# zhvng/open-musiclm

Measured on AMD Instinct MI355X. Metric: train steps/sec + AR tokens/sec, coarse-stage musiclm_small, higher is better.
Workload: dtype fp16ff; 1 GPU; musiclm_small coarse-stage train step (fwd+bwd+allreduce+clip+AdamW), N=1116 (3 start + 13 clap + 200 semantic + 900 coarse), forgetful mask 0.15, ff_dropout 0.1; global_batch=32, per_gpu_batch=32, grad_accum=1, seq_len=1116, parallelism=dp1, precision=fp16ff, hip_graph=True, exchange=none (single GPU)

## Files before the change

include/omlm.h:

```cpp
#ifndef OMLM_H
#define OMLM_H
#include <stdint.h>
#ifdef __cplusplus
extern "C" {
#endif

int         omlm_version(void);
const char* omlm_last_error(void);
void        omlm_set_error(const char* msg);

int omlm_gemm(const void* A, const void* B, void* C, const float* Cin,
              const int* a_map, const int* b_map, const int* c_map, long long a_rows, long long b_rows,
              int M, int N, int K, int lda, int ldb, int ldc, int ldcin,
              int a_kmajor, int b_kmajor, int in_dtype, int out_dtype, float alpha,
              void* workspace, long long workspace_bytes, void* stream);
long long omlm_gemm_tail_workspace_bytes(int M, int N);

int omlm_layernorm_fwd(const float* x, const float* gamma, void* y, void* xcast, float* mean, float* rstd,
                       int M, int D, int ldy, float eps, int out_dtype, void* stream);
int omlm_layernorm_fwd_planes(const float* x, const float* gamma, void* y, void* y_lo, float* mean, float* rstd,
                              int M, int D, int ldy, float eps, int out_dtype, void* stream);
int omlm_layernorm_fwd_seg(const float* x, const float* gamma, void* y, void* xcast, float* mean, float* rstd, float* xc,
                           int M, int D, int ldy, float eps, int out_dtype, int n_full, int p0, int n_live, void* stream);
int omlm_layernorm_fwd_planes_seg(const float* x, const float* gamma, void* y, void* y_lo, float* mean, float* rstd, float* xc,
                                  int M, int D, int ldy, float eps, int out_dtype, int n_full, int p0, int n_live, void* stream);
int omlm_layernorm_bwd2_seg(const void* dy, const float* x, const float* gamma, const float* mean, const float* rstd,
                            const float* dres, const void* dres2, float* dx, void* dxcast, float* dgamma, float* workspace, int M, int D,
                            float dx_scale, int cast_dtype, int dy_dtype, int n_full, int p0, int n_live, void* stream);
long long omlm_layernorm_bwd_workspace_bytes(int D);
int omlm_layernorm_bwd2(const void* dy, const float* x, const float* gamma, const float* mean, const float* rstd,
                        const float* dres, const void* dres2, float* dx, void* dxcast, float* dgamma, float* workspace, int M, int D,
                        float dx_scale, int cast_dtype, int dy_dtype, void* stream);

int omlm_qk_norm_fwd(const float* q_raw, const float* kv_raw, const float* q_scale, const float* k_scale,
                     void* q, void* k, void* v, int M, int H, int out_dtype, void* stream);
int omlm_qk_norm_bwd(const float* dq, const float* dk, const float* dv, const float* q_raw, const float* kv_raw,
                     const float* q_scale, const float* k_scale, void* dq_raw, void* dkv_raw,
                     float* dq_scale, float* dk_scale, int M, int H, int out_dtype, void* stream);

int omlm_gemm_qknorm(const void* A, const void* B, void* C, void* C2, int c2_col0, int ldc2, const float* scale, float* norm_out,
                     int ldnorm, int groups, long long a_rows, long long b_rows, int M, int N, int K, int lda, int ldb, int ldc,
                     int dtype, void* stream);
int omlm_qk_norm_bwd2(const float* dq, const float* dk, const float* dv, const void* q, const void* k, const float* qn, const float* kn,
                      const float* q_scale, const float* k_scale, void* dq_raw, void* dkv_raw, float* dq_scale, float* dk_scale,
                      int M, int H, int dtype, void* stream);

int omlm_mqa_attn_fwd(const void* q, const void* k, const void* v, const float* bias, const float* biasT, const unsigned char* keymask,
                      void* out, float* lse, int B, int N, int H, float scale, int bias_ld, int dtype, int P, float p,
                      unsigned long long seed, const unsigned long long* seed_dev, void* stream);
long long omlm_attn_bias_table_floats(int N, int H, int P);
int omlm_attn_bias_prepare(const float* bias, float* biasT, int N, int H, int bias_ld, const float* q_scale,
                           const float* k_scale, float qk_bound, float scale, int p_max_log2, void* stream);
int omlm_attn_bias_prepare_group(const float* bias, float* const* biasT, int layers, int N, int H, int bias_ld,
                                 const float* const* q_scale, const float* const* k_scale, float qk_bound, float scale,
                                 int p_max_log2, int P, void* stream);
int omlm_attn_max_positions(int dtype, int P);
long long omlm_mqa_attn_bwd_workspace_bytes(int B, int N, int H);
int omlm_mqa_attn_bwd(const void* q, const void* k, const void* v, const float* bias, const float* biasT, const unsigned char* keymask,
                      const void* out, const void* dout, const float* lse, float* delta, float* dq, float* dk, float* dv, float* dbias,
                      float* dbias_ws, int B, int N, int H, float scale, int bias_ld, int dtype, int P, float p, unsigned long long seed,
                      const unsigned long long* seed_dev, void* stream);
int omlm_attn_dropout_keep(unsigned char* keep, int B, int N, int H, float p, unsigned long long seed,
                           const unsigned long long* seed_dev, void* stream);
int omlm_dropout_residual_fwd(const float* x, const float* y, float* x1, long long M, int D, float p, unsigned long long seed,
                              const unsigned long long* seed_dev, void* stream);
int omlm_dropout_residual_bwd(const float* dx1, void* dy, long long M, int D, float p, unsigned long long seed,
                              const unsigned long long* seed_dev, int out_dtype, void* stream);

int omlm_ffmid_fwd(const void* h1, const void* convw, const void* gamma, void* h2, float* mean, float* rstd,
                   int M, int nseq, int F, int Fp, float eps, float p, unsigned long long seed,
                   const unsigned long long* seed_dev, unsigned char* drop_bits, void* gh, int dtype, void* stream);
int omlm_ffmid_fwd_planes(const void* h1, const void* h1_lo, const void* convw, const void* convw_lo, const void* gamma, const void* gamma_lo,
                          void* h2, void* h2_lo, float* mean, float* rstd, int M, int nseq, int F, int Fp, float eps, float p,
                          unsigned long long seed, const unsigned long long* seed_dev, unsigned char* drop_bits, void* gh, int dtype, void* stream);
int omlm_ffmid_fwd_seg(const void* h1, const void* convw, const void* gamma, void* h2, float* mean, float* rstd,
                       int M, int nseq, int F, int Fp, float eps, float p, unsigned long long seed,
                       const unsigned long long* seed_dev, unsigned char* drop_bits, void* gh, int dtype, int n_full, int p0, void* stream);
int omlm_ffmid_fwd_planes_seg(const void* h1, const void* h1_lo, const void* convw, const void* convw_lo, const void* gamma, const void* gamma_lo,
                              void* h2, void* h2_lo, float* mean, float* rstd, int M, int nseq, int F, int Fp, float eps, float p,
                              unsigned long long seed, const unsigned long long* seed_dev, unsigned char* drop_bits, void* gh, int dtype,
                              int n_full, int p0, void* stream);
long long omlm_ffmid_bwd_workspace_bytes(int F, int Fp);
int omlm_ffmid_bwd(const void* dh2, const void* h1, const void* convw, const void* gamma, const float* mean,
                   const float* rstd, void* du_tmp, void* dh1, float* dgamma, float* dconv, float* workspace,
                   int M, int nseq, int F, int Fp, float p, unsigned long long seed,
                   const unsigned long long* seed_dev, const unsigned char* drop_bits, const void* gh, int dtype, void* stream);
int omlm_colsum_accumulate(const float* part, float* out, int P, int C, int ldp, void* stream);
typedef struct omlm_colsum_desc { const float* part; float* out; int P, C, ldp; } omlm_colsum_desc;
int omlm_colsum_group(const omlm_colsum_desc* problems, int count, void* stream);
int omlm_ffmid_set_impl(int impl);

int omlm_embed_gather_fwd(const int* ids, const int* seg, const int* posidx,
                          const float* const* tables, const float* const* starts, const float* const* pos,
                          int nseq, float* out, int B, int N, int D,
                          const long long* table_rows, const long long* pos_rows, int* err_flag, void* stream);
int omlm_embed_gather_bwd(const int* ids, const int* seg, const int* posidx,
                          float* const* dtables, float* const* dstarts, float* const* dpos,
                          int nseq, const float* dx, int B, int N, int D, float alpha,
                          const long long* table_rows, const long long* pos_rows, int* err_flag, void* stream);

int omlm_prepare_train_batch(const long long* const* ids, int* const* labels, const int* len, const int* eos, const int* Q,
                             const int* codebook, int nseq, int B, int pad_id, const float* scores, int n_drop,
                             int* ids32, unsigned char* keymask, int N, const float* null_u, float null_p, void* stream);

int omlm_cross_entropy_fwd(const float* logits, const int* labels, float* row_lse, float* nll_sum,
                           int R, int V, int ld, int* err_flag, void* stream);
int omlm_cross_entropy_bwd(const float* logits, const int* labels, const float* row_lse, const float* gscale,
                           float coef, void* dlogits, int R, int V, int ld, int ldd, int out_dtype, void* stream);
int omlm_cross_entropy_fwd_reg(const float* logits, const int* labels, float* row_lse, float* sums,
                               int R, int V, int ld, int* err_flag, void* stream);
int omlm_cross_entropy_bwd_reg(const float* logits, const int* labels, const float* row_lse, const float* gscale,
                               float coef, void* dlogits, int R, int V, int ld, int ldd, int out_dtype,
                               float label_smoothing, float z_loss, void* stream);

int omlm_sumsq_accumulate(const float* g, long long n, float* out, float* partials, void* stream);
int omlm_adamw_clip_step(float* p, float* g, float* m, float* v, void* p16, long long n,
                         float lr, float beta1, float beta2, float eps, float wd, int step,
                         float gscale, const float* gnorm_sq, float max_norm, int decoupled, int zero_grad, int p16_dtype,
                         const float* ls_state, void* stream);
int omlm_adamw_clip_step_ema(float* p, float* g, float* m, float* v, void* p16, long long n,
                             float lr, float beta1, float beta2, float eps, float wd, int step,
                             float gscale, const float* gnorm_sq, float max_norm, int decoupled, int zero_grad, int p16_dtype,
                             const float* ls_state, float* e, float ema_decay, int ema_update_after_step, int ema_warmup, void* stream);
int omlm_loss_scale_update(float* ls_state, const float* gnorm_sq, float growth, float backoff, int interval,
                           float scale_min, float scale_max, void* stream);

int omlm_cast_pad(const float* src, void* dst, long long R, int C, int ld_src, int ld_dst, int out_dtype, void* stream);
typedef struct omlm_cast_pad_desc { const float* src; void* dst; int R, C, ld_src, ld_dst, transpose, lo; } omlm_cast_pad_desc;
int omlm_cast_pad_group(const omlm_cast_pad_desc* problems, int count, int out_dtype, void* stream);

int omlm_gemm_planes(const void* A, long long a_plane_bytes, const void* B, long long b_plane_bytes, void* C, const float* Cin,
                     const int* a_map, const int* b_map, const int* c_map, long long a_rows, long long b_rows,
                     int M, int N, int K, int lda, int ldb, int ldc, int ldcin,
                     int a_kmajor, int b_kmajor, int out_dtype, float alpha, void* workspace, long long workspace_bytes, void* stream);
int omlm_split_planes(const float* x, void* planes, long long n, long long plane_elems, void* stream);
int omlm_gemm_planes16(const void* A, const void* A_lo, const void* B, const void* B_lo, void* C, void* C_lo, const float* Cin,
                       const int* a_map, const int* c_map, long long a_rows, long long b_rows, int M, int N, int K,
                       int lda, int ldb, int ldc, int ldcin, int dtype, void* workspace, long long workspace_bytes, void* stream);
int omlm_gemm_mx16(const void* A, const void* A8, long long a8_stride, const unsigned char* a_scale,
                   const void* B, const void* B8, long long b8_stride, const unsigned char* b_scale,
                   void* C, void* C_lo, int c_lo_bf8, const float* Cin, long long a_rows, long long b_rows,
                   int M, int N, int K, int lda, int ldb, int ldc, int ldcin,
                   void* workspace, long long workspace_bytes, void* stream);
long long omlm_gemm_mx16_workspace_bytes(int M, int N, int K);
int omlm_layernorm_fwd_mx(const float* x, const float* gamma, void* y, void* y8, long long y8_stride, unsigned char* scale8,
                          float* mean, float* rstd, int M, int D, int ldy, float eps, void* stream);
int omlm_ffmid_fwd_mx(const void* h1, const void* h1_lo, const void* convw, const void* convw_lo, const void* gamma, const void* gamma_lo,
                      void* h2, void* h2_8, long long h2_8_stride, unsigned char* scale8, float* mean, float* rstd, int M, int nseq, int F, int Fp,
                      float eps, float p, unsigned long long seed, const unsigned long long* seed_dev, unsigned char* drop_bits, void* gh, void* stream);
int omlm_layernorm_fwd_mx_seg(const float* x, const float* gamma, void* y, void* y8, long long y8_stride, unsigned char* scale8,
                              float* mean, float* rstd, float* xc, int M, int D, int ldy, float eps, int n_full, int p0, int n_live, void* stream);
int omlm_ffmid_fwd_mx_seg(const void* h1, const void* h1_lo, const void* convw, const void* convw_lo, const void* gamma, const void* gamma_lo,
                          void* h2, void* h2_8, long long h2_8_stride, unsigned char* scale8, float* mean, float* rstd, int M, int nseq, int F, int Fp,
                          float eps, float p, unsigned long long seed, const unsigned long long* seed_dev, unsigned char* drop_bits, void* gh,
                          int n_full, int p0, void* stream);
typedef struct omlm_quant_rows_desc { const float* src; unsigned char* dst8; long long lo_stride; unsigned char* scale8; int R, C, ld_src, ld8; } omlm_quant_rows_desc;
int omlm_quant_rows_mx(const omlm_quant_rows_desc* problems, int count, void* stream);
typedef struct omlm_gemm_wgrad_desc {
    const void* A; const void* B; float* C; const int* c_map;
    int M, N, K, lda, ldb, ldc;
} omlm_gemm_wgrad_desc;
int omlm_gemm_wgrad_group(const omlm_gemm_wgrad_desc* problems, int count, int splits, int dtype, void* stream);

int omlm_relpos_first_fwd(const float* w0, const float* b0, float* pre, float* z, int n, int Hd, int x0, void* stream);
int omlm_relpos_first_bwd(const float* ds, float* dw0, int n, int Hd, int x0, void* stream);
int omlm_bias_silu_fwd(const float* a, const float* b, float* pre, float* z, long long R, int C, void* stream);
int omlm_silu_bwd(const float* dz, const float* pre, float* ds, long long total, void* stream);
int omlm_bias_add(const float* a, const float* b, float* out, int R, int C, int ld, void* stream);
int omlm_relpos_mlp_fwd(const float* w0, const float* b0, const float* W1, const float* b1, const float* W2, const float* b2,
                        const float* W3, const float* b3, float* pre0, float* z0, float* pre1, float* z1, float* pre2, float* z2,
                        float* table, int n, int Hd, int H, int ldb, int x0, void* stream);
int omlm_relpos_mlp_bwd(const float* dtable, const float* W1, const float* W2, const float* W3, const float* pre0, const float* z0,
                        const float* pre1, const float* z1, const float* pre2, const float* z2, float* scratch, float* gw0, float* gb0,
                        float* gW1, float* gb1, float* gW2, float* gb2, float* gW3, float* gb3, int n, int Hd, int H, int ldb, int x0,
                        void* stream);

int omlm_rvq_encode(const float* x, const float* codebooks_T, int* indices, float* residual_out,
                    int n, int D, int C, int nstage, int idx_stride, void* stream);
int omlm_nearest_centroid(const float* x, const float* centroids_T, int* indices, int n, int D, int C, void* stream);
int omlm_vq_accumulate(const float* x, const int* indices, int idx_stride, float* counts, float* sums, int n, int D, int K, void* stream);
int omlm_vq_kmeans_update(float* means, float* means_T, const float* counts, const float* sums, int K, int D, void* stream);
int omlm_vq_ema_update(float* cluster_size, float* embed_avg, float* embed, float* embed_T, const float* counts, const float* sums,
                       float* total_scratch, int K, int D, float decay, float eps, void* stream);

long long omlm_kmeans_pp_workspace_bytes(int m, int trials);
int omlm_kmeans_pp_pick(const float* rows, float* closest, const float* uniforms, int* pick_counter, float* centres, float* centres_T,
                        int* chosen, double* pots, void* workspace, long long workspace_bytes, int m, int D, int K, int trials,
                        void* stream);
int omlm_kmeans_pp_seed(const float* rows, float* closest, const float* uniforms, int* pick_counter, float* centres, float* centres_T,
                        int* chosen, double* pots, void* workspace, long long workspace_bytes, int m, int D, int K, int trials,
                        void* stream);
int omlm_kmeans_minibatch_step(const float* x, const int* idx, float* centres, float* centres_T, float* counts, float* bcounts,
                               float* sums, float* rowmin, double* move_partial, double* state, int n, int B, int D, int K,
                               double alpha, double tol_abs, int max_no_improvement, void* stream);
int omlm_kmeans_inertia(const float* x, const float* centres_T, double* out, int* labels, int n, int D, int K, void* stream);

int omlm_sample_topk_gumbel(const float* logits, const float* uniform, long long* out, int B, int V, int ld,
                            int k, float temperature, int forbid_last, void* stream);

int omlm_sample_topk_gumbel_at(const float* logits, const float* uniform_base, const int* step_dev, long long* out,
                               long long* hist, int B, int V, int ld, int k, float temperature, int forbid_last, void* stream);

int omlm_sample_embed_at(const float* logits, const float* uniform_base, const int* step_dev, long long* out, long long* hist,
                         int B, int V, int ld, int k, float temperature, int forbid_last,
                         const float* emb_table, long long emb_row_offset, long long emb_rows, float* x, int D, void* stream);

int omlm_sample_topk_gumbel_rng(const float* logits, unsigned seed_lo, unsigned seed_hi, int step, int row0, long long* out,
                                int B, int V, int ld, int k, float temperature, int forbid_last, void* stream);
int omlm_sample_topk_gumbel_at_rng(const float* logits, unsigned seed_lo, unsigned seed_hi, const int* step_dev, int row0,
                                   long long* out, long long* hist, int B, int V, int ld, int k, float temperature, int forbid_last,
                                   void* stream);
int omlm_sample_embed_at_rng(const float* logits, unsigned seed_lo, unsigned seed_hi, const int* step_dev, int row0, long long* out,
                             long long* hist, int B, int V, int ld, int k, float temperature, int forbid_last,
                             const float* emb_table, long long emb_row_offset, long long emb_rows, float* x, int D, void* stream);

typedef struct omlm_sample_args {
    const float* logits;
    int B, V, ld;
    const float* uniform;
    unsigned seed_lo, seed_hi;
    int step, row0;
    const int* step_dev;
    long long* out;
    long long* hist;
    int k;
    float temperature, top_p;
    int forbid_last;
    const float* emb_table;
    long long emb_row_offset, emb_rows;
    float* x;
    int D;
} omlm_sample_args;
int omlm_sample(const omlm_sample_args* args, void* stream);

int omlm_sample_lp(const omlm_sample_args* args, float* lp_model, float* lp_sampled, void* stream);

typedef struct omlm_sample_row_params {
    const int*   k;
    const float* temperature;
// ... 49 lines not shown
```

open_musiclm_amd/csrc/ffmid.hip:

```cpp
#include "common.h"
#include "ffmid_plan.h"
#include <initializer_list>
#include <stdlib.h>

namespace OMLM_NS {
using namespace omlm_plan;

template <typename T> struct vec8;
template <> struct vec8<float> {
    float v[8];
    __device__ __forceinline__ void load(const float* p) {
        const float4 a = ((const float4*)p)[0], b = ((const float4*)p)[1];
        v[0] = a.x; v[1] = a.y; v[2] = a.z; v[3] = a.w; v[4] = b.x; v[5] = b.y; v[6] = b.z; v[7] = b.w;
    }
    __device__ __forceinline__ void store(float* p) const {
        ((float4*)p)[0] = make_float4(v[0], v[1], v[2], v[3]);
        ((float4*)p)[1] = make_float4(v[4], v[5], v[6], v[7]);
    }
};
template <> struct vec8<h16_t> {
    float v[8];
    __device__ __forceinline__ void load(const h16_t* p) {
        const u32x4 a = *(const u32x4*)p;
#pragma unroll
// ... 421 lines not shown
        for (int i = 0; i < 8; ++i) {
            o.v[i] = w[i][2] * da.v[i] + w[i][1] * (m1 * db.v[i]) + w[i][0] * (m2 * dc.v[i]);
            dw[i][0] += da.v[i] * (p2 * xa.v[i]);
            dw[i][1] += da.v[i] * (p1 * xb.v[i]);
            dw[i][2] += da.v[i] * xc.v[i];
        }
        o.store(dh1 + (size_t)row * ld + col);
    }
#pragma unroll
    for (int i = 0; i < 8; ++i) {
        if (chreal + i < F) {
#pragma unroll
            for (int k = 0; k < 3; ++k)
                part_dconv[((size_t)blockIdx.y * 2 * F + wch + i) * 3 + k] = dw[i][k];
        }
    }
}

__global__ void colsum_kernel(const float* __restrict__ part, float* __restrict__ out, int P, int C, int ldp) {
    const int c = blockIdx.x * blockDim.x + threadIdx.x;
    if (c >= C) return;
    const int per = (P + gridDim.y - 1) / gridDim.y;
    const int p0 = blockIdx.y * per, p1 = min(P, p0 + per);
    float s = 0.f;
    for (int p = p0; p < p1; ++p) s += part[(size_t)p * ldp + c];
    if (p1 > p0) unsafeAtomicAdd(out + c, s);
}

struct omlm_colsum_desc { const float* part; float* out; int P, C, ldp; };
#define OMLM_COLSUM_MAX 32
struct ColsumGroupArgs { int n; omlm_colsum_desc p[OMLM_COLSUM_MAX]; };
__global__ void colsum_group_kernel(ColsumGroupArgs ga) {
    const omlm_colsum_desc& q = ga.p[blockIdx.z];
    const int c = blockIdx.x * blockDim.x + threadIdx.x;
    if (c >= q.C) return;
    const int per = (q.P + gridDim.y - 1) / gridDim.y;
    const int p0 = blockIdx.y * per, p1 = min(q.P, p0 + per);
    float s = 0.f;
    for (int p = p0; p < p1; ++p) s += q.part[(size_t)p * q.ldp + c];
    if (p1 > p0) unsafeAtomicAdd(q.out + c, s);
}

#if OMLM_FP16
extern "C" int omlm_colsum_accumulate(const float* part, float* out, int P, int C, int ldp, void* stream);
extern "C" int omlm_colsum_group(const omlm_colsum_desc* d, int count, void* stream);
#else
extern "C" int omlm_colsum_group(const omlm_colsum_desc* d, int count, void* stream) {
    if (count <= 0) return OMLM_OK;
    OMLM_CHECK_ARG(d, "colsum_group: null descriptor array");
    for (int base = 0; base < count; base += OMLM_COLSUM_MAX) {
        ColsumGroupArgs ga;
        memset(&ga, 0, sizeof(ga));
        ga.n = count - base < OMLM_COLSUM_MAX ? count - base : OMLM_COLSUM_MAX;
        int cmax = 0, pmax = 0;
        for (int i = 0; i < ga.n; ++i) {
            const omlm_colsum_desc& q = d[base + i];
            OMLM_CHECK_ARG(q.part && q.out && q.P > 0 && q.C > 0 && q.ldp >= q.C, "colsum_group: bad problem");
            ga.p[i] = q;
            if (q.C > cmax) cmax = q.C;
            if (q.P > pmax) pmax = q.P;
        }
        hipLaunchKernelGGL(colsum_group_kernel, dim3((cmax + 255) / 256, colsum_ysplit(pmax), ga.n), dim3(256), 0, as_stream(stream), ga);
    }
    return omlm_post_launch("omlm_colsum_group");
}

extern "C" int omlm_colsum_accumulate(const float* part, float* out, int P, int C, int ldp, void* stream) {
    if (P <= 0 || C <= 0) return OMLM_OK;
    OMLM_CHECK_ARG(part && out && ldp >= C, "colsum arguments");
    hipLaunchKernelGGL(colsum_kernel, dim3((C + 255) / 256, colsum_ysplit(P)), dim3(256), 0, as_stream(stream), part, out, P, C, ldp);
    return omlm_post_launch("omlm_colsum_accumulate");
}

#endif

static_assert(FF_ERR_ARG == OMLM_ERR_ARG && FF_LDS_CAP == 160 * 1024 && FF_LDS_OPT_IN == 48 * 1024, "ffmid_plan.h states the return code and launch_lds_optin's sizes");
int ffmid2_launch(const FfmidLaunch& l, const FfmidArgs& a);

template <typename T>
static int ffmid_launch_t(const FfmidLaunch& l, const FfmidArgs& a, float* part_g, float* part_c) {
    const hipStream_t st = as_stream(a.stream);
    const dim3 grid(l.gx, l.gy), block(l.threads);
    switch (l.kernel) {
    case FK_FWD1: {
#define FF_FWD(MC_) launch_lds_optin<ffmid_fwd_kernel<T, MC_>>(grid, block, (size_t)l.lds, st, (const T*)a.h1, (const T*)a.convw, (const T*)a.gamma, (T*)a.h2, a.mean, a.rstd, \
                                                               a.M, a.nseq, a.F, a.Fp, a.eps, a.p, a.seed, a.seed_dev, a.drop_bits, (T*)a.gh)
        switch (l.n) { case 2: FF_FWD(2); break; case 6: FF_FWD(6); break; case 8: FF_FWD(8); break; default: FF_FWD(16); break; }
#undef FF_FWD
        return omlm_post_launch("omlm_ffmid_fwd");
    }
    case FK_BWD1: {
#define FF_B1G(MC_, GH_) launch_lds_optin<ffmid_bwd1_kernel<T, MC_, GH_>>(grid, block, (size_t)l.lds, st, (const T*)a.dh2, (const T*)a.h1, (const T*)a.convw, (const T*)a.gamma, \
                             (const float*)a.mean, (const float*)a.rstd, (T*)a.du_tmp, part_g, a.M, a.nseq, a.F, a.Fp, a.p, a.seed, a.seed_dev, \
                             (const unsigned char*)a.drop_bits, (const T*)a.gh)
#define FF_B1(MC_) do { if (l.gh) FF_B1G(MC_, true); else FF_B1G(MC_, false); } while (0)
        switch (l.n) { case 2: FF_B1(2); break; case 6: FF_B1(6); break; case 8: FF_B1(8); break; default: FF_B1(16); break; }
#undef FF_B1
#undef FF_B1G
        return omlm_post_launch("omlm_ffmid_bwd (row pass)");
    }
    default:
        hipLaunchKernelGGL(ffmid_bwd2_kernel<T>, grid, block, 0, st, (const T*)a.du_tmp, (const T*)a.h1, (const T*)a.convw, (T*)a.dh1, part_c, a.M, a.nseq, a.F, a.Fp);
        return omlm_post_launch("omlm_ffmid_bwd");
    }
}

static int ffmid_launch(const FfmidLaunch& l, const FfmidArgs& a) {
    float* part_g = a.workspace;
    float* part_c = a.workspace ? a.workspace + ffmid_ws_dconv_at(a.Fp) : nullptr;
    switch (l.kernel) {
    case FK_FWD1: case FK_BWD1: case FK_BWD2:
#if !OMLM_FP16
        if (!l.t16) return ffmid_launch_t<float>(l, a, part_g, part_c);
#endif
        return ffmid_launch_t<h16_t>(l, a, part_g, part_c);
    case FK_COLSUM_GROUP: {
        const omlm_colsum_desc two[2] = {{part_g, a.dgamma, l.g_rows, a.F, a.Fp}, {part_c, a.dconv, l.c_rows, 2 * a.F * 3, 2 * a.F * 3}};
        return omlm_colsum_group(two, 2, a.stream);
    }
    case FK_COLSUM_G: return omlm_colsum_accumulate(part_g, a.dgamma, l.g_rows, a.F, a.Fp, a.stream);
    case FK_COLSUM_C: return omlm_colsum_accumulate(part_c, a.dconv, l.c_rows, 2 * a.F * 3, 2 * a.F * 3, a.stream);
    default: return ffmid2_launch(l, a);
    }
}

static int ffmid_run(const FfmidCall& c, const FfmidArgs& a) {
    const FfmidPlan plan = ffmid_plan(c);
    if (plan.rc != OMLM_OK) { omlm_set_error(plan.msg); return plan.rc; }
    for (int i = 0; i < plan.n; ++i) {
        const int rc = ffmid_launch(plan.l[i], a);
        if (rc) return rc;
    }
    return OMLM_OK;
}

#if !OMLM_FP16
extern "C" { __attribute__((visibility("hidden"))) int omlm_ffmid_impl_value = 1; }
extern "C" int omlm_ffmid_set_impl(int impl) {
    OMLM_CHECK_ARG(impl == 0 || impl == 1, "impl: 0 = wave-per-row, 1 = column strips");
    omlm_ffmid_impl_value = impl;
    return OMLM_OK;
}
extern "C" long long omlm_ffmid_bwd_workspace_bytes(int F, int Fp) { return ffmid_bwd_workspace_bytes(F, Fp); }
#else
extern "C" { extern __attribute__((visibility("hidden"))) int omlm_ffmid_impl_value; }
#endif

static FfmidCall ffmid_call(FfOp op, const FfmidArgs& a, int dtype, bool operands) {
    FfmidCall c;
    memset(&c, 0, sizeof(c));
    c.op = op; c.M = a.M; c.nseq = a.nseq; c.F = a.F; c.Fp = a.Fp; c.dtype = dtype; c.fp16_copy = OMLM_FP16 != 0; c.p = a.p; c.operands = operands;
    c.drop_bits = a.drop_bits != nullptr; c.gh = a.gh != nullptr; c.dgamma = a.dgamma != nullptr; c.dconv = a.dconv != nullptr;
    c.n_full = a.n_full; c.p0 = a.p0; c.h2_8_stride = a.h2_8_stride; c.impl = omlm_ffmid_impl_value;
    return c;
}
static bool ffmid_aligned16(std::initializer_list<const void*> ps) {
    uintptr_t all = 0;
    for (const void* q : ps) all |= (uintptr_t)q;
    return all % 16 == 0;
}

#if !OMLM_FP16
extern "C" int omlm_ffmid_fwd_seg_h(const void* h1, const void* convw, const void* gamma, void* h2, float* mean, float* rstd,
                                    int M, int nseq, int F, int Fp, float eps, float p, unsigned long long seed,
                                    const unsigned long long* seed_dev, unsigned char* drop_bits, void* gh, int dtype, int n_full, int p0, void* stream);
#endif
extern "C" int OMLM_API(omlm_ffmid_fwd_seg)(const void* h1, const void* convw, const void* gamma, void* h2, float* mean, float* rstd,
                              int M, int nseq, int F, int Fp, float eps, float p, unsigned long long seed,
                              const unsigned long long* seed_dev, unsigned char* drop_bits, void* gh, int dtype, int n_full, int p0, void* stream) {
#if !OMLM_FP16
    if (dtype == OMLM_DT_F16) return omlm_ffmid_fwd_seg_h(h1, convw, gamma, h2, mean, rstd, M, nseq, F, Fp, eps, p, seed, seed_dev, drop_bits, gh, 1, n_full, p0, stream);
#endif
    FfmidArgs a;
    memset(&a, 0, sizeof(a));
    a.h1 = h1; a.convw = convw; a.gamma = gamma; a.h2 = h2; a.mean = mean; a.rstd = rstd;
    a.M = M; a.nseq = nseq; a.F = F; a.Fp = Fp; a.eps = eps; a.p = p; a.seed = seed; a.seed_dev = seed_dev; a.drop_bits = drop_bits; a.gh = gh;
    a.n_full = n_full; a.p0 = p0; a.stream = stream;
    return ffmid_run(ffmid_call(FF_FWD, a, dtype, h1 && convw && gamma && h2 && mean && rstd), a);
}
#if !OMLM_FP16
extern "C" int omlm_ffmid_fwd(const void* h1, const void* convw, const void* gamma, void* h2, float* mean, float* rstd,
                              int M, int nseq, int F, int Fp, float eps, float p, unsigned long long seed,
                              const unsigned long long* seed_dev, unsigned char* drop_bits, void* gh, int dtype, void* stream) {
    return omlm_ffmid_fwd_seg(h1, convw, gamma, h2, mean, rstd, M, nseq, F, Fp, eps, p, seed, seed_dev, drop_bits, gh, dtype, 0, 0, stream);
}
#endif

#if !OMLM_FP16
extern "C" int omlm_ffmid_fwd_planes_seg_h(const void* h1, const void* h1_lo, const void* convw, const void* convw_lo, const void* gamma, const void* gamma_lo,
                                           void* h2, void* h2_lo, float* mean, float* rstd, int M, int nseq, int F, int Fp, float eps, float p,
                                           unsigned long long seed, const unsigned long long* seed_dev, unsigned char* drop_bits, void* gh, int dtype,
                                           int n_full, int p0, void* stream);
#endif
extern "C" int OMLM_API(omlm_ffmid_fwd_planes_seg)(const void* h1, const void* h1_lo, const void* convw, const void* convw_lo, const void* gamma,
                                               const void* gamma_lo, void* h2, void* h2_lo, float* mean, float* rstd, int M, int nseq, int F, int Fp,
                                               float eps, float p, unsigned long long seed, const unsigned long long* seed_dev,
                                               unsigned char* drop_bits, void* gh, int dtype, int n_full, int p0, void* stream) {
#if !OMLM_FP16
    if (dtype == OMLM_DT_F16)
        return omlm_ffmid_fwd_planes_seg_h(h1, h1_lo, convw, convw_lo, gamma, gamma_lo, h2, h2_lo, mean, rstd, M, nseq, F, Fp, eps, p, seed, seed_dev, drop_bits, gh, 1,
                                           n_full, p0, stream);
#endif
    FfmidArgs a;
    memset(&a, 0, sizeof(a));
    a.h1 = h1; a.h1_lo = h1_lo; a.convw = convw; a.convw_lo = convw_lo; a.gamma = gamma; a.gamma_lo = gamma_lo; a.h2 = h2; a.h2_lo = h2_lo;
    a.mean = mean; a.rstd = rstd; a.M = M; a.nseq = nseq; a.F = F; a.Fp = Fp; a.eps = eps; a.p = p; a.seed = seed; a.seed_dev = seed_dev;
    a.drop_bits = drop_bits; a.gh = gh; a.n_full = n_full; a.p0 = p0; a.stream = stream;
    FfmidCall c = ffmid_call(FF_FWD_PLANES, a, dtype, h1 && h1_lo && convw && convw_lo && gamma && gamma_lo && h2 && h2_lo && mean && rstd);
    c.planes_aligned = ffmid_aligned16({h1, h1_lo, convw, convw_lo, gamma, gamma_lo, h2, h2_lo});
    return ffmid_run(c, a);
}
#if !OMLM_FP16
extern "C" int omlm_ffmid_fwd_planes(const void* h1, const void* h1_lo, const void* convw, const void* convw_lo, const void* gamma,
                                     const void* gamma_lo, void* h2, void* h2_lo, float* mean, float* rstd, int M, int nseq, int F, int Fp,
                                     float eps, float p, unsigned long long seed, const unsigned long long* seed_dev,
                                     unsigned char* drop_bits, void* gh, int dtype, void* stream) {
    return omlm_ffmid_fwd_planes_seg(h1, h1_lo, convw, convw_lo, gamma, gamma_lo, h2, h2_lo, mean, rstd, M, nseq, F, Fp, eps, p, seed, seed_dev, drop_bits, gh,
                                     dtype, 0, 0, stream);
}
#endif

#if OMLM_FP16
}
extern "C" int omlm_ffmid_fwd_mx_seg(const void* h1, const void* h1_lo, const void* convw, const void* convw_lo, const void* gamma, const void* gamma_lo,
                                 void* h2, void* h2_8, long long h2_8_stride, unsigned char* scale8, float* mean, float* rstd, int M, int nseq, int F, int Fp,
                                 float eps, float p, unsigned long long seed, const unsigned long long* seed_dev, unsigned char* drop_bits, void* gh,
                                 int n_full, int p0, void* stream) {
    using namespace OMLM_NS;
    FfmidArgs a;
    memset(&a, 0, sizeof(a));
    a.h1 = h1; a.h1_lo = h1_lo; a.convw = convw; a.convw_lo = convw_lo; a.gamma = gamma; a.gamma_lo = gamma_lo; a.h2 = h2; a.h2_8 = h2_8;
    a.h2_8_stride = h2_8_stride; a.scale8 = scale8; a.mean = mean; a.rstd = rstd; a.M = M; a.nseq = nseq; a.F = F; a.Fp = Fp; a.eps = eps; a.p = p;
    a.seed = seed; a.seed_dev = seed_dev; a.drop_bits = drop_bits; a.gh = gh; a.n_full = n_full; a.p0 = p0; a.stream = stream;
    FfmidCall c = ffmid_call(FF_FWD_MX, a, 1, h1 && h1_lo && convw && convw_lo && gamma && gamma_lo && h2 && h2_8 && scale8 && mean && rstd);
    c.planes_aligned = ffmid_aligned16({h1, h1_lo, convw, convw_lo, gamma, gamma_lo, h2, h2_8});
    return ffmid_run(c, a);
}
extern "C" int omlm_ffmid_fwd_mx(const void* h1, const void* h1_lo, const void* convw, const void* convw_lo, const void* gamma, const void* gamma_lo,
                                 void* h2, void* h2_8, long long h2_8_stride, unsigned char* scale8, float* mean, float* rstd, int M, int nseq, int F, int Fp,
                                 float eps, float p, unsigned long long seed, const unsigned long long* seed_dev, unsigned char* drop_bits, void* gh,
                                 void* stream) {
    return omlm_ffmid_fwd_mx_seg(h1, h1_lo, convw, convw_lo, gamma, gamma_lo, h2, h2_8, h2_8_stride, scale8, mean, rstd, M, nseq, F, Fp, eps, p, seed, seed_dev,
                                 drop_bits, gh, 0, 0, stream);
}
namespace OMLM_NS {
#endif

#if !OMLM_FP16
extern "C" int omlm_ffmid_bwd_h(const void* dh2, const void* h1, const void* convw, const void* gamma, const float* mean,
                                const float* rstd, void* du_tmp, void* dh1, float* dgamma, float* dconv, float* workspace,
                                int M, int nseq, int F, int Fp, float p, unsigned long long seed,
                                const unsigned long long* seed_dev, const unsigned char* drop_bits, const void* gh, int dtype,
                                void* stream);
#endif
extern "C" int OMLM_API(omlm_ffmid_bwd)(const void* dh2, const void* h1, const void* convw, const void* gamma, const float* mean,
                              const float* rstd, void* du_tmp, void* dh1, float* dgamma, float* dconv, float* workspace,
                              int M, int nseq, int F, int Fp, float p, unsigned long long seed,
                              const unsigned long long* seed_dev, const unsigned char* drop_bits, const void* gh, int dtype,
                              void* stream) {
#if !OMLM_FP16
    if (dtype == OMLM_DT_F16)
        return omlm_ffmid_bwd_h(dh2, h1, convw, gamma, mean, rstd, du_tmp, dh1, dgamma, dconv, workspace, M, nseq, F, Fp, p, seed, seed_dev,
                                drop_bits, gh, 1, stream);
#endif
    FfmidArgs a;
    memset(&a, 0, sizeof(a));
    a.dh2 = dh2; a.h1 = h1; a.convw = convw; a.gamma = gamma; a.mean = const_cast<float*>(mean); a.rstd = const_cast<float*>(rstd);
    a.du_tmp = du_tmp; a.dh1 = dh1; a.dgamma = dgamma; a.dconv = dconv; a.workspace = workspace; a.M = M; a.nseq = nseq; a.F = F; a.Fp = Fp; a.p = p;
    a.seed = seed; a.seed_dev = seed_dev; a.drop_bits = const_cast<unsigned char*>(drop_bits); a.gh = const_cast<void*>(gh); a.stream = stream;
    FfmidCall c = ffmid_call(FF_BWD, a, dtype, dh2 && h1 && convw && gamma && mean && rstd && du_tmp && dh1 && workspace);
    c.du_aligned = (uintptr_t)du_tmp % 8 == 0;
    return ffmid_run(c, a);
}

}
```

open_musiclm_amd/csrc/ffmid2.hip:

```cpp
#include "common.h"
#include "ffmid_plan.h"
#include <type_traits>

namespace OMLM_NS {
using namespace omlm_plan;

typedef f32x2 v2;

__device__ __forceinline__ v2 mk2(float a, float b) { v2 r; r[0] = a; r[1] = b; return r; }
__device__ __forceinline__ v2 splat2(float a) { return mk2(a, a); }
__device__ __forceinline__ v2 bf2_to_f2(unsigned w) { return mk2(h16_lo_to_f(w), h16_hi_to_f(w)); }
__device__ __forceinline__ unsigned f2_to_bf2(v2 v) { return pack_h16_rne(v[0], v[1]); }
__device__ __forceinline__ v2 fma2(v2 a, v2 b, v2 c) { return __builtin_elementwise_fma(a, b, c); }

template <typename T> struct Ch8;
template <> struct Ch8<h16_t> {
    u32x4 r;
    __device__ __forceinline__ void load(const h16_t* p) { r = *(const u32x4*)p; }
    __device__ __forceinline__ void zero() { r[0] = 0u; r[1] = 0u; r[2] = 0u; r[3] = 0u; }
    __device__ __forceinline__ v2 get(int i) const { return bf2_to_f2(r[i]); }
    static __device__ __forceinline__ void store(h16_t* p, const v2 (&y)[4]) {
        u32x4 o;
#pragma unroll
        for (int i = 0; i < 4; ++i) o[i] = f2_to_bf2(y[i]);
        *(u32x4*)p = o;
    }
};
template <> struct Ch8<float> {
    float4 a, b;
    __device__ __forceinline__ void load(const float* p) { a = ((const float4*)p)[0]; b = ((const float4*)p)[1]; }
    __device__ __forceinline__ void zero() { a = make_float4(0.f, 0.f, 0.f, 0.f); b = a; }
    __device__ __forceinline__ v2 get(int i) const {
        return i == 0 ? mk2(a.x, a.y) : (i == 1 ? mk2(a.z, a.w) : (i == 2 ? mk2(b.x, b.y) : mk2(b.z, b.w)));
    }
    static __device__ __forceinline__ void store(float* p, const v2 (&y)[4]) {
        ((float4*)p)[0] = make_float4(y[0][0], y[0][1], y[1][0], y[1][1]);
        ((float4*)p)[1] = make_float4(y[2][0], y[2][1], y[3][0], y[3][1]);
    }
};
template <typename T> struct Ch4;
template <> struct Ch4<h16_t> {
    u32x2 r;
    __device__ __forceinline__ void load(const h16_t* p) { r = *(const u32x2*)p; }
    __device__ __forceinline__ void zero() { r[0] = 0u; r[1] = 0u; }
    __device__ __forceinline__ v2 get(int i) const { return bf2_to_f2(r[i]); }
    static __device__ __forceinline__ void store(h16_t* p, const v2 (&y)[2]) {
        u32x2 o; o[0] = f2_to_bf2(y[0]); o[1] = f2_to_bf2(y[1]);
        *(u32x2*)p = o;
    }
};
template <> struct Ch4<float> {
    float4 a;
    __device__ __forceinline__ void load(const float* p) { a = *(const float4*)p; }
    __device__ __forceinline__ void zero() { a = make_float4(0.f, 0.f, 0.f, 0.f); }
    __device__ __forceinline__ v2 get(int i) const { return i == 0 ? mk2(a.x, a.y) : mk2(a.z, a.w); }
    static __device__ __forceinline__ void store(float* p, const v2 (&y)[2]) { *(float4*)p = make_float4(y[0][0], y[0][1], y[1][0], y[1][1]); }
};

template <typename T, bool PL> struct Row8 {
    Ch8<T> h;
    __device__ __forceinline__ void load(const T* p, long long) { h.load(p); }
    __device__ __forceinline__ void zero() { h.zero(); }
    __device__ __forceinline__ v2 get(int i) const { return h.get(i); }
};
template <typename T> struct Row8<T, true> {
    Ch8<T> h, l;
    __device__ __forceinline__ void load(const T* p, long long lo) { h.load(p); l.load(p + lo); }
    __device__ __forceinline__ void zero() { h.zero(); l.zero(); }
    __device__ __forceinline__ v2 get(int i) const { return h.get(i) + l.get(i); }
};
__device__ __forceinline__ void store_planes8(h16_t* hi, h16_t* lo, const v2 (&y)[4]) {
    u32x4 o, l;
#pragma unroll
    for (int i = 0; i < 4; ++i) { o[i] = f2_to_bf2(y[i]); l[i] = f2_to_bf2(y[i] - bf2_to_f2(o[i])); }
    *(u32x4*)hi = o;
    *(u32x4*)lo = l;
}
__device__ __forceinline__ void store_planes8(float*, float*, const v2 (&)[4]) {}
struct FfPlanes { long long h1_lo, convw_lo, gamma_lo; void* h2_lo;
                  unsigned char* h2_8; long long h2_8_stride; unsigned char* scale8;
                  const unsigned char* h1_8; };
__device__ __forceinline__ v2 bf8_pair(u32x2 l, int i) {
    switch (i) {
        case 0: return __builtin_amdgcn_cvt_pk_f32_bf8((int)l[0], false);
        case 1: return __builtin_amdgcn_cvt_pk_f32_bf8((int)l[0], true);
        case 2: return __builtin_amdgcn_cvt_pk_f32_bf8((int)l[1], false);
        default: return __builtin_amdgcn_cvt_pk_f32_bf8((int)l[1], true);
    }
}
template <typename T, bool PL, bool MX> struct H1Row {
    Row8<T, PL> r;
    __device__ __forceinline__ void load(const T* h1, size_t off, const FfPlanes& pl) { r.load(h1 + off, pl.h1_lo); }
    __device__ __forceinline__ void zero() { r.zero(); }
    __device__ __forceinline__ v2 get(int i) const { return r.get(i); }
};
template <typename T> struct H1Row<T, true, true> {
    Ch8<T> h; u32x2 l;
    __device__ __forceinline__ void load(const T* h1, size_t off, const FfPlanes& pl) { h.load(h1 + off); l = *(const u32x2*)(pl.h1_8 + off); }
    __device__ __forceinline__ void zero() { h.zero(); l[0] = 0u; l[1] = 0u; }
    __device__ __forceinline__ v2 get(int i) const { return h.get(i) + bf8_pair(l, i); }
};
__device__ __forceinline__ void store_mx8(h16_t* hi, unsigned char* p8h, unsigned char* p8l, const v2 (&y)[4], float sh, float sl) {
    u32x4 o;
    u32x2 h8, l8;
#pragma unroll
    for (int i = 0; i < 4; ++i) o[i] = f2_to_bf2(y[i]);
#pragma unroll
    for (int i = 0; i < 2; ++i) {
        const v2 ha = bf2_to_f2(o[2 * i]), hb = bf2_to_f2(o[2 * i + 1]);
        h8[i] = pack4_fp8(ha[0] * sh, ha[1] * sh, hb[0] * sh, hb[1] * sh);
        l8[i] = pack4_fp8((y[2 * i][0] - ha[0]) * sl, (y[2 * i][1] - ha[1]) * sl, (y[2 * i + 1][0] - hb[0]) * sl, (y[2 * i + 1][1] - hb[1]) * sl);
    }
    *(u32x4*)hi = o;
    *(u32x2*)p8h = h8;
    *(u32x2*)p8l = l8;
}
__device__ __forceinline__ void store_mx8(float*, unsigned char*, unsigned char*, const v2 (&)[4], float, float) {}


__device__ __forceinline__ void gelu_parts(v2 u, v2& h, v2& ex) {
    const v2 au = mk2(fabsf(u[0]), fabsf(u[1]));
    const v2 d = fma2(au, splat2(0.23164189f), splat2(1.0f));
    const v2 t = mk2(__builtin_amdgcn_rcpf(d[0]), __builtin_amdgcn_rcpf(d[1]));
    v2 poly = fma2(t, splat2(0.5f * 1.061405429f), splat2(0.5f * -1.453152027f));
    poly = fma2(poly, t, splat2(0.5f * 1.421413741f));
    poly = fma2(poly, t, splat2(0.5f * -0.284496736f));
    poly = fma2(poly, t, splat2(0.5f * 0.254829592f));
    poly = poly * t;
    const v2 q = u * u;
    ex = mk2(__builtin_amdgcn_exp2f(q[0] * -0.72134752f), __builtin_amdgcn_exp2f(q[1] * -0.72134752f));
    const v2 hp = fma2(-poly, ex, splat2(0.5f));
    h = mk2(0.5f + copysignf(hp[0], u[0]), 0.5f + copysignf(hp[1], u[1]));
}

__device__ __forceinline__ unsigned lowbias32(unsigned x) {
    x ^= x >> 16; x *= 0x7feb352du; x ^= x >> 15; x *= 0x846ca68bu; x ^= x >> 16;
    return x;
}
__device__ __forceinline__ void keep_words(unsigned long long seed, unsigned long long blk, unsigned w[4]) {
    const unsigned k0 = (unsigned)seed, k1 = (unsigned)(seed >> 32);
    unsigned x = lowbias32(((unsigned)blk ^ k0) + 0x9E3779B9u * ((unsigned)(blk >> 32) ^ k1));
    x = lowbias32(x ^ k1);
    w[0] = x;
    x = (x ^ (x >> 15)) * 0x2c1b3c6du; w[1] = x ^ (x >> 13);
    x = (x ^ (x >> 12)) * 0x297a2d39u; w[2] = x ^ (x >> 15);
    x = (x ^ (x >> 14)) * 0x85ebca6bu; w[3] = x ^ (x >> 16);
}

#define FS_R 4
#define FS_OCC 1

struct FfSeg { int n_full, p0; };
template <typename T, int NT, bool TRAIN, bool PL, bool MX, bool SEG>
__device__ __forceinline__ void ffmid2_fwd_body(const T* __restrict__ h1, const T* __restrict__ convw,
                                                        const T* __restrict__ gamma, T* __restrict__ h2,
                                                        float* __restrict__ mean, float* __restrict__ rstd,
                                                        int nseq, int F, int Fp, int RB, int strips, float eps, float p,
                                                        unsigned long long seed, const unsigned long long* __restrict__ seed_dev,
                                                        unsigned char* __restrict__ drop_bits, T* __restrict__ gh_out, const FfPlanes pl, const FfSeg seg) {
    constexpr int NW = NT / 64;
    constexpr int RB_ = (sizeof(T) == 2 && !PL) ? FS_R : (FS_R > 2 ? 2 : FS_R);
    __shared__ float st[2][FS_R][NW][2];
    __shared__ float gmx[MX ? NW : 1];
    if (seed_dev) seed += seed_dev[0] * 0x9E3779B97F4A7C15ull;
    const int b = blockIdx.x / strips, s = blockIdx.x - b * strips;
    const int t0 = s * RB, t1 = min(nseq, t0 + RB);
    if (t0 >= t1) return;
    const int lane = threadIdx.x & 63, wave = threadIdx.x >> 6;
    const int col = threadIdx.x * 8;
    const int ld = 2 * Fp;
    const size_t row0 = (size_t)b * nseq;
    const size_t hrow0 = SEG ? (size_t)b * seg.n_full + seg.p0 : row0;
    const float inv = p > 0.f ? 1.0f / (1.0f - p) : 1.0f;
    const unsigned thr = (unsigned)(p * 65536.0f + 0.5f);

    v2 wv[3][4], wg[3][4], gm[4];
    Row8<T, PL> tv[3], tg[3];
#pragma unroll
    for (int k = 0; k < 3; ++k) {
        tv[k].load(convw + (size_t)k * ld + col, pl.convw_lo);
        tg[k].load(convw + (size_t)k * ld + Fp + col, pl.convw_lo);
#pragma unroll
        for (int i = 0; i < 4; ++i) { wv[k][i] = tv[k].get(i); wg[k][i] = tg[k].get(i); }
    }
    {
        Row8<T, PL> a;
        a.load(gamma + col, pl.gamma_lo);
#pragma unroll
        for (int i = 0; i < 4; ++i) gm[i] = a.get(i) * inv;
    }
    float gmmax = 0.f;
    if constexpr (MX) {
#pragma unroll
        for (int i = 0; i < 4; ++i) gmmax = fmaxf(gmmax, fmaxf(fabsf(gm[i][0]), fabsf(gm[i][1])));
        gmmax = wave_max(gmmax);
        if (lane == 0) gmx[wave] = gmmax;
        __syncthreads();
        gmmax = gmx[0];
#pragma unroll
        for (int w = 1; w < NW; ++w) gmmax = fmaxf(gmmax, gmx[w]);
    }
    const int e_mx = MX ? mx_row_exp(sqrtf((float)F) * gmmax) : 0;
    const float sh_mx = ldexpf(1.0f, -e_mx), sl_mx = ldexpf(1.0f, 11 - e_mx);
    v2 x1v[4], x1g[4], x2v[4], x2g[4];
    {
        H1Row<T, PL, MX> a, c, d, e;
        a.zero(); c.zero(); d.zero(); e.zero();
        if (t0 >= 1) { a.load(h1, (row0 + t0 - 1) * ld + col, pl); c.load(h1, (row0 + t0 - 1) * ld + Fp + col, pl); }
        if (t0 >= 2) { d.load(h1, (row0 + t0 - 2) * ld + col, pl); e.load(h1, (row0 + t0 - 2) * ld + Fp + col, pl); }
#pragma unroll
        for (int i = 0; i < 4; ++i) { x1v[i] = a.get(i); x1g[i] = c.get(i); x2v[i] = d.get(i); x2g[i] = e.get(i); }
    }
    H1Row<T, PL, MX> rv[RB_], rg[RB_];
#pragma unroll
    for (int r = 0; r < RB_; ++r)
        if (t0 + r < t1) {
            rv[r].load(h1, (row0 + t0 + r) * ld + col, pl);
            rg[r].load(h1, (row0 + t0 + r) * ld + Fp + col, pl);
        }
    const float invF = 1.0f / (float)F;

    auto batch = [&](auto full_tag, const int tb, const int it) {
        constexpr bool FULL = decltype(full_tag)::value;
        v2 g[RB_][4];
        float ls[RB_], lq[RB_];
#pragma unroll
        for (int r = 0; r < RB_; ++r) {
            ls[r] = 0.f; lq[r] = 0.f;
            if (FULL || tb + r < t1) {
                v2 s2 = splat2(0.f), q2 = splat2(0.f);
#pragma unroll
                for (int i = 0; i < 4; ++i) {
                    const v2 xv = rv[r].get(i), xg = rg[r].get(i);
                    const v2 uv = fma2(wv[2][i], xv, fma2(wv[1][i], x1v[i], wv[0][i] * x2v[i]));
                    const v2 ug = fma2(wg[2][i], xg, fma2(wg[1][i], x1g[i], wg[0][i] * x2g[i]));
                    x2v[i] = x1v[i]; x1v[i] = xv; x2g[i] = x1g[i]; x1g[i] = xg;
                    v2 h, ex;
                    gelu_parts(ug, h, ex);
                    const v2 gv = (ug * h) * uv;
                    g[r][i] = gv;
                    s2 += gv;
                    q2 = fma2(gv, gv, q2);
                }
                ls[r] = s2[0] + s2[1];
                lq[r] = q2[0] + q2[1];
            } else {
#pragma unroll
                for (int i = 0; i < 4; ++i) g[r][i] = splat2(0.f);
            }
            if (FULL || tb + RB_ + r < t1) {
                if (FULL) __builtin_amdgcn_sched_barrier(0);
                rv[r].load(h1, (row0 + tb + RB_ + r) * ld + col, pl);
                rg[r].load(h1, (row0 + tb + RB_ + r) * ld + Fp + col, pl);
                if (FULL) __builtin_amdgcn_sched_barrier(0);
            }
        }
#pragma unroll
        for (int r = 0; r < RB_; ++r) { ls[r] = wave_sum(ls[r]); lq[r] = wave_sum(lq[r]); }
        if (lane == 0) {
#pragma unroll
            for (int r = 0; r < RB_; ++r) { st[it & 1][r][wave][0] = ls[r]; st[it & 1][r][wave][1] = lq[r]; }
        }
        __syncthreads();
        float mu_r[RB_], rs_r[RB_];
#pragma unroll
        for (int r = 0; r < RB_; ++r) {
            if (!FULL && tb + r >= t1) continue;
            float S = 0.f, Q = 0.f;
#pragma unroll
            for (int w = 0; w < NW; ++w) { S += st[it & 1][r][w][0]; Q += st[it & 1][r][w][1]; }
            const float mu = S * invF;
            const float var = fmaxf(Q * invF - mu * mu, 0.f);
            const float rs = rsqrtf(var + eps);
            const size_t row = row0 + tb + r;
            const float sh = sh_mx, sl = sl_mx;
            if (FULL) { mu_r[r] = mu; rs_r[r] = rs; }
            else if (threadIdx.x == 0) { mean[row] = mu; rstd[row] = rs; if constexpr (MX) pl.scale8[row] = (unsigned char)(e_mx + 127); }
            const v2 nmr = splat2(-mu * rs), rs2 = splat2(rs);
            v2 gh[4], y[4];
#pragma unroll
            for (int i = 0; i < 4; ++i) gh[i] = fma2(g[r][i], rs2, nmr);
            if (col + 8 > F) {
#pragma unroll
                for (int i = 0; i < 4; ++i) {
                    if (col + 2 * i >= F) gh[i][0] = 0.f;
                    if (col + 2 * i + 1 >= F) gh[i][1] = 0.f;
                }
            }
#pragma unroll
            for (int i = 0; i < 4; ++i) y[i] = gh[i] * gm[i];
            if (TRAIN || p > 0.f) {
                unsigned w[4], bits = 0;
                keep_words(seed, (SEG ? hrow0 + tb + r : row) * (unsigned long long)(Fp >> 3) + (unsigned)(col >> 3), w);
#pragma unroll
                for (int i = 0; i < 4; ++i) {
                    const bool k0 = (w[i] & 0xFFFFu) >= thr, k1 = (w[i] >> 16) >= thr;
                    y[i][0] = k0 ? y[i][0] : 0.f;
                    y[i][1] = k1 ? y[i][1] : 0.f;
                    bits |= (k0 ? 1u : 0u) << (2 * i);
                    bits |= (k1 ? 1u : 0u) << (2 * i + 1);
                }
                if (TRAIN || drop_bits) drop_bits[row * (size_t)(Fp >> 3) + (col >> 3)] = (unsigned char)bits;
            }
            if constexpr (MX) {
                store_mx8(h2 + row * Fp + col, pl.h2_8 + row * (2 * (size_t)Fp) + col, pl.h2_8 + pl.h2_8_stride + row * (2 * (size_t)Fp) + col, y, sh, sl);
                if ((int)threadIdx.x < ((((Fp + 127) & ~127) - Fp) >> 3)) {
                    unsigned char* z8 = pl.h2_8 + row * (2 * (size_t)Fp) + Fp + 8 * threadIdx.x;
                    u32x2 z; z[0] = 0u; z[1] = 0u;
                    *(u32x2*)z8 = z;
                    *(u32x2*)(z8 + pl.h2_8_stride) = z;
                }
            }
            else if constexpr (PL) store_planes8(h2 + row * Fp + col, (T*)pl.h2_lo + row * Fp + col, y);
            else Ch8<T>::store(h2 + row * Fp + col, y);
            if (TRAIN || gh_out) Ch8<T>::store(gh_out + row * Fp + col, gh);
        }
        if (FULL) {
            const int q = lane % RB_;
            float m = mu_r[0], s_ = rs_r[0];
#pragma unroll
            for (int r = 1; r < RB_; ++r) { m = q == r ? mu_r[r] : m; s_ = q == r ? rs_r[r] : s_; }
            mean[row0 + tb + q] = m;
            rstd[row0 + tb + q] = s_;
            if constexpr (MX) pl.scale8[row0 + tb + q] = (unsigned char)(e_mx + 127);
        }
    };
    int it = 0, tb = t0;
    __builtin_amdgcn_s_waitcnt(0x0F70);
#pragma unroll 1
    for (; tb + 2 * RB_ <= t1; tb += RB_, ++it) batch(std::true_type{}, tb, it);
#pragma unroll 1
    for (; tb < t1; tb += RB_, ++it) batch(std::false_type{}, tb, it);
}

template <typename T, int NT, bool TRAIN, bool PL = false, bool MX = false>
__global__ __launch_bounds__(NT, (FS_OCC * NT + 255) / 256) void ffmid2_fwd_kernel(const T* __restrict__ h1, const T* __restrict__ convw,
                                                        const T* __restrict__ gamma, T* __restrict__ h2,
                                                        float* __restrict__ mean, float* __restrict__ rstd,
                                                        int nseq, int F, int Fp, int RB, int strips, float eps, float p,
                                                        unsigned long long seed, const unsigned long long* __restrict__ seed_dev,
                                                        unsigned char* __restrict__ drop_bits, T* __restrict__ gh_out, const FfPlanes pl) {
    ffmid2_fwd_body<T, NT, TRAIN, PL, MX, false>(h1, convw, gamma, h2, mean, rstd, nseq, F, Fp, RB, strips, eps, p, seed, seed_dev, drop_bits, gh_out, pl, FfSeg{0, 0});
}
template <typename T, int NT, bool TRAIN, bool PL = false, bool MX = false>
__global__ __launch_bounds__(NT, (FS_OCC * NT + 255) / 256) void ffmid2_fwd_seg_kernel(const T* __restrict__ h1, const T* __restrict__ convw,
                                                        const T* __restrict__ gamma, T* __restrict__ h2,
                                                        float* __restrict__ mean, float* __restrict__ rstd,
                                                        int nseq, int F, int Fp, int RB, int strips, float eps, float p,
                                                        unsigned long long seed, const unsigned long long* __restrict__ seed_dev,
                                                        unsigned char* __restrict__ drop_bits, T* __restrict__ gh_out, const FfPlanes pl, const FfSeg seg) {
    ffmid2_fwd_body<T, NT, TRAIN, PL, MX, true>(h1, convw, gamma, h2, mean, rstd, nseq, F, Fp, RB, strips, eps, p, seed, seed_dev, drop_bits, gh_out, pl, seg);
}

template <typename T, int MAXC>
__global__ __launch_bounds__(256) void ffmid2_rowsum_kernel(const T* __restrict__ dh2, const T* __restrict__ gamma,
                                                            const T* __restrict__ ghs, const unsigned char* __restrict__ drop_bits,
                                                            const float* __restrict__ rstd, float* __restrict__ bc,
                                                            float* __restrict__ part_dgamma, int M, int F, int Fp, float p) {
    const int lane = threadIdx.x & 63, wave = threadIdx.x >> 6;
    const float inv = p > 0.f ? 1.0f / (1.0f - p) : 1.0f;
    const int nwaves = gridDim.x * 4;
    v2 dg[MAXC][4], gmv[MAXC][4];
#pragma unroll
    for (int k = 0; k < MAXC; ++k) {
        const int ch = (lane + 64 * k) * 8;
        Ch8<T> a;
        a.zero();
        if (ch < Fp) a.load(gamma + ch);
#pragma unroll
        for (int i = 0; i < 4; ++i) { dg[k][i] = splat2(0.f); gmv[k][i] = a.get(i); }
    }
    Ch8<T> d[MAXC], gq[MAXC];
    unsigned bits[MAXC];
    float rs_next = 0.f;
    auto request = [&](int row, int k) {
        const int ch = (lane + 64 * k) * 8;
        if (ch < Fp) {
            d[k].load(dh2 + (size_t)row * Fp + ch);
            gq[k].load(ghs + (size_t)row * Fp + ch);
            bits[k] = (p > 0.f) ? drop_bits[(size_t)row * (Fp >> 3) + (ch >> 3)] : 0xFFu;
        }
    };
    {
        const int row0 = blockIdx.x * 4 + wave;
        if (row0 < M) {
#pragma unroll
            for (int k = 0; k < MAXC; ++k) request(row0, k);
            rs_next = rstd[row0];
        }
    }
    for (int row = blockIdx.x * 4 + wave; row < M; row += nwaves) {
        v2 s1 = splat2(0.f), s2 = splat2(0.f);
        const int nxt = row + nwaves;
        const float rs_cur = rs_next;
#pragma unroll
        for (int k = 0; k < MAXC; ++k) {
            const int ch = (lane + 64 * k) * 8;
            if (ch < Fp) {
#pragma unroll
                for (int i = 0; i < 4; ++i) {
                    v2 dy = d[k].get(i) * inv;
                    if (!((bits[k] >> (2 * i)) & 1u)) dy[0] = 0.f;
                    if (!((bits[k] >> (2 * i + 1)) & 1u)) dy[1] = 0.f;
                    const v2 gh = gq[k].get(i);
                    dg[k][i] = fma2(dy, gh, dg[k][i]);
                    const v2 gy = dy * gmv[k][i];
                    s1 += gy;
                    s2 = fma2(gy, gh, s2);
                }
            }
            if (nxt < M) request(nxt, k);
        }
        if (nxt < M) rs_next = rstd[nxt];
        const float t1 = wave_sum(s1[0] + s1[1]), t2 = wave_sum(s2[0] + s2[1]);
        if (lane == 0) {
            const float rs = rs_cur / (float)F;
            bc[2 * (size_t)row] = rs * t1;
            bc[2 * (size_t)row + 1] = rs * t2;
        }
    }
    extern __shared__ __attribute__((aligned(16))) float red[];
#pragma unroll
    for (int k = 0; k < MAXC; ++k) {
        const int ch = (lane + 64 * k) * 8;
        if (ch < Fp) {
#pragma unroll
            for (int i = 0; i < 4; ++i) { red[(size_t)wave * Fp + ch + 2 * i] = dg[k][i][0]; red[(size_t)wave * Fp + ch + 2 * i + 1] = dg[k][i][1]; }
        }
    }
    __syncthreads();
    for (int c = threadIdx.x; c < Fp; c += 256)
        part_dgamma[(size_t)blockIdx.x * Fp + c] = red[c] + red[Fp + c] + red[2 * Fp + c] + red[3 * Fp + c];
}

template <typename T> struct Bwd2Row { Ch4<T> dy, gh, xv, xg; unsigned bits; float a, b, c; };

template <typename T>
__global__ __launch_bounds__(256) void ffmid2_bwd_kernel(const T* __restrict__ dh2, const T* __restrict__ h1,
                                                         const T* __restrict__ convw, const T* __restrict__ gamma,
                                                         const float* __restrict__ rstd, const float* __restrict__ bc,
                                                         const T* __restrict__ ghs, const unsigned char* __restrict__ drop_bits,
                                                         T* __restrict__ dh1, float* __restrict__ part_dconv,
                                                         int nseq, int F, int Fp, int RB, int strips, int total_strips, float p) {
    const int c4 = blockIdx.x * 256 + threadIdx.x;
    const int col = c4 * 4;
    const bool act = col < Fp;
    const int colc = act ? col : 0;
    const int ld = 2 * Fp;
    const float inv = p > 0.f ? 1.0f / (1.0f - p) : 1.0f;
    const int nib = (c4 & 1) * 4;

    v2 wv[3][2], wg[3][2], gm[2];
#pragma unroll
    for (int k = 0; k < 3; ++k) {
        Ch4<T> a, c;
        a.load(convw + (size_t)k * ld + colc);
        c.load(convw + (size_t)k * ld + Fp + colc);
#pragma unroll
        for (int i = 0; i < 2; ++i) { wv[k][i] = act ? a.get(i) : splat2(0.f); wg[k][i] = act ? c.get(i) : splat2(0.f); }
    }
    {
        Ch4<T> a;
        a.load(gamma + colc);
#pragma unroll
        for (int i = 0; i < 2; ++i) gm[i] = act ? a.get(i) * inv : splat2(0.f);
    }
    v2 dcv[3][2], dcg[3][2];
#pragma unroll
    for (int k = 0; k < 3; ++k)
#pragma unroll
        for (int i = 0; i < 2; ++i) { dcv[k][i] = splat2(0.f); dcg[k][i] = splat2(0.f); }

    auto load_row = [&](Bwd2Row<T>& R, size_t row) {
        R.dy.load(dh2 + row * Fp + colc);
        R.gh.load(ghs + row * Fp + colc);
        R.xv.load(h1 + row * ld + colc);
        R.xg.load(h1 + row * ld + Fp + colc);
        R.bits = (p > 0.f) ? (unsigned)drop_bits[row * (size_t)(Fp >> 3) + (colc >> 3)] : 0xFFu;
        R.a = rstd[row]; R.b = bc[2 * row]; R.c = bc[2 * row + 1];
    };

#pragma unroll 1
    for (int strip = blockIdx.y; strip < total_strips; strip += gridDim.y) {
        const int b = strip / strips, s = strip - b * strips;
        const int t0 = s * RB, t1 = min(nseq, t0 + RB);
        if (t0 >= t1) continue;
        const size_t row0 = (size_t)b * nseq;
        v2 x1v[2], x1g[2], x2v[2], x2g[2], p1v[2], p1g[2], p2v[2], p2g[2];
        {
            Ch4<T> a, c, d, e;
            a.zero(); c.zero(); d.zero(); e.zero();
            if (t0 >= 1) { a.load(h1 + (row0 + t0 - 1) * ld + colc); c.load(h1 + (row0 + t0 - 1) * ld + Fp + colc); }
            if (t0 >= 2) { d.load(h1 + (row0 + t0 - 2) * ld + colc); e.load(h1 + (row0 + t0 - 2) * ld + Fp + colc); }
#pragma unroll
            for (int i = 0; i < 2; ++i) {
                x1v[i] = a.get(i); x1g[i] = c.get(i); x2v[i] = d.get(i); x2g[i] = e.get(i);
                p1v[i] = splat2(0.f); p1g[i] = splat2(0.f); p2v[i] = splat2(0.f); p2g[i] = splat2(0.f);
            }
        }
        const int tend = t1 + 2;
        Bwd2Row<T> cur, nxt;
        load_row(cur, row0 + t0);
#pragma unroll 1
        for (int t = t0; t < tend; ++t) {
            if (t + 1 < min(tend, nseq)) load_row(nxt, row0 + t + 1);
            v2 duv[2], dug[2];
            if (t < nseq) {
                const float own = t < t1 ? 1.f : 0.f;
                const unsigned kb = cur.bits >> nib;
#pragma unroll
                for (int i = 0; i < 2; ++i) {
                    v2 gy = cur.dy.get(i) * gm[i];
                    if (!((kb >> (2 * i)) & 1u)) gy[0] = 0.f;
                    if (!((kb >> (2 * i + 1)) & 1u)) gy[1] = 0.f;
                    const v2 gh = cur.gh.get(i);
                    v2 dg = fma2(gy, splat2(cur.a), splat2(-cur.b));
                    dg = fma2(gh, splat2(-cur.c), dg);
                    const v2 xv = cur.xv.get(i), xg = cur.xg.get(i);
                    const v2 uv = fma2(wv[2][i], xv, fma2(wv[1][i], x1v[i], wv[0][i] * x2v[i]));
                    const v2 ug = fma2(wg[2][i], xg, fma2(wg[1][i], x1g[i], wg[0][i] * x2g[i]));
                    v2 h, ex;
                    gelu_parts(ug, h, ex);
                    const v2 gp = fma2(ug * 0.3989422804f, ex, h);
                    const v2 a_ = dg * (ug * h);
                    const v2 g_ = (dg * uv) * gp;
                    duv[i] = a_; dug[i] = g_;
                    const v2 ao = a_ * own, go = g_ * own;
                    dcv[0][i] = fma2(ao, x2v[i], dcv[0][i]); dcv[1][i] = fma2(ao, x1v[i], dcv[1][i]); dcv[2][i] = fma2(ao, xv, dcv[2][i]);
                    dcg[0][i] = fma2(go, x2g[i], dcg[0][i]); dcg[1][i] = fma2(go, x1g[i], dcg[1][i]); dcg[2][i] = fma2(go, xg, dcg[2][i]);
                    x2v[i] = x1v[i]; x1v[i] = xv; x2g[i] = x1g[i]; x1g[i] = xg;
                }
            } else {
#pragma unroll
                for (int i = 0; i < 2; ++i) { duv[i] = splat2(0.f); dug[i] = splat2(0.f); }
            }
            if (t - 2 >= t0 && act) {
                v2 ov[2], og[2];
#pragma unroll
                for (int i = 0; i < 2; ++i) {
                    ov[i] = fma2(wv[0][i], duv[i], p2v[i]);
                    og[i] = fma2(wg[0][i], dug[i], p2g[i]);
                }
                Ch4<T>::store(dh1 + (row0 + t - 2) * ld + col, ov);
                Ch4<T>::store(dh1 + (row0 + t - 2) * ld + Fp + col, og);
            }
#pragma unroll
            for (int i = 0; i < 2; ++i) {
                p2v[i] = fma2(wv[1][i], duv[i], p1v[i]); p1v[i] = wv[2][i] * duv[i];
                p2g[i] = fma2(wg[1][i], dug[i], p1g[i]); p1g[i] = wg[2][i] * dug[i];
            }
            cur = nxt;
        }
    }
    if (act) {
        float* pr = part_dconv + (size_t)blockIdx.y * 2 * F * 3;
#pragma unroll
        for (int i = 0; i < 2; ++i)
#pragma unroll
            for (int e = 0; e < 2; ++e) {
                const int ch = col + 2 * i + e;
                if (ch < F) {
#pragma unroll
                    for (int k = 0; k < 3; ++k) { pr[(size_t)ch * 3 + k] = dcv[k][i][e]; pr[(size_t)(F + ch) * 3 + k] = dcg[k][i][e]; }
                }
            }
    }
}

template <typename T> struct Bwd3Row { Ch4<T> dy, gh, xv, xg; unsigned bits; float a; };
__device__ __forceinline__ void opaque(Ch4<h16_t>& c) { asm volatile("" : "+v"(c.r[0]), "+v"(c.r[1])); }
__device__ __forceinline__ void opaque(Ch4<float>&) {}

template <typename T, int NT>
__global__ __launch_bounds__(NT) void ffmid3_bwd_kernel(const T* __restrict__ dh2, const T* __restrict__ h1,
                                                        const T* __restrict__ convw, const T* __restrict__ gamma,
                                                        const float* __restrict__ rstd, const T* __restrict__ ghs,
                                                        const unsigned char* __restrict__ drop_bits, T* __restrict__ dh1,
                                                        float* __restrict__ part_dconv, float* __restrict__ part_dgamma,
                                                        int nseq, int F, int Fp, int RB, int strips, int total_strips, float p) {
    constexpr int NW = NT / 64;
    __shared__ __attribute__((aligned(16))) float red[2][NW][2];
    const int lane = threadIdx.x & 63, wave = threadIdx.x >> 6;
    const int col = threadIdx.x * 4;
    const bool act = col < Fp;
    const int colc = act ? col : 0;
    const int ld = 2 * Fp;
    const float inv = p > 0.f ? 1.0f / (1.0f - p) : 1.0f, invF = 1.0f / (float)F;
    const int nib = (threadIdx.x & 1) * 4;

    Ch4<T> wvr[3], wgr[3];
    v2 gm[2];
#pragma unroll
    for (int k = 0; k < 3; ++k) {
        wvr[k].zero(); wgr[k].zero();
        if (act) { wvr[k].load(convw + (size_t)k * ld + colc); wgr[k].load(convw + (size_t)k * ld + Fp + colc); }
    }
    {
        Ch4<T> a;
        a.load(gamma + colc);
#pragma unroll
        for (int i = 0; i < 2; ++i) gm[i] = act ? a.get(i) : splat2(0.f);
    }
    v2 dcv[3][2], dcg[3][2], dgam[2];
#pragma unroll
    for (int i = 0; i < 2; ++i) {
        dgam[i] = splat2(0.f);
#pragma unroll
        for (int k = 0; k < 3; ++k) { dcv[k][i] = splat2(0.f); dcg[k][i] = splat2(0.f); }
    }

    auto load_row = [&](Bwd3Row<T>& R, size_t row) {
        R.dy.load(dh2 + row * Fp + colc);
        R.gh.load(ghs + row * Fp + colc);
        R.xv.load(h1 + row * ld + colc);
        R.xg.load(h1 + row * ld + Fp + colc);
        R.bits = (p > 0.f) ? (unsigned)drop_bits[row * (size_t)(Fp >> 3) + (colc >> 3)] : 0xFFu;
        R.a = rstd[row];
    };
    auto dy_kept = [&](const Bwd3Row<T>& R, v2 (&dy)[2]) {
        const unsigned kb = R.bits >> nib;
#pragma unroll
        for (int i = 0; i < 2; ++i) {
            dy[i] = R.dy.get(i) * inv;
            if (!((kb >> (2 * i)) & 1u)) dy[i][0] = 0.f;
            if (!((kb >> (2 * i + 1)) & 1u)) dy[i][1] = 0.f;
        }
    };
    auto publish_sums = [&](const Bwd3Row<T>& R, int buf) {
        v2 dy[2], s1 = splat2(0.f), s2 = splat2(0.f);
        dy_kept(R, dy);
#pragma unroll
        for (int i = 0; i < 2; ++i) {
            const v2 gy = dy[i] * gm[i];
            s1 += gy;
            s2 = fma2(gy, R.gh.get(i), s2);
        }
        const float t1 = wave_sum_dpp(s1[0] + s1[1]), t2 = wave_sum_dpp(s2[0] + s2[1]);
        if (lane == 0) { red[buf][wave][0] = t1; red[buf][wave][1] = t2; }
    };

#pragma unroll 1
    for (int strip = blockIdx.y; strip < total_strips; strip += gridDim.y) {
        const int b = strip / strips, s = strip - b * strips;
        const int t0 = s * RB, t1 = min(nseq, t0 + RB);
        if (t0 >= t1) continue;
        const size_t row0 = (size_t)b * nseq;
        const int tlast = min(t1 + 2, nseq);
        v2 x1v[2], x1g[2], x2v[2], x2g[2], p1v[2], p1g[2], p2v[2], p2g[2];
        {
            Ch4<T> a, c, d, e;
            a.zero(); c.zero(); d.zero(); e.zero();
            if (t0 >= 1) { a.load(h1 + (row0 + t0 - 1) * ld + colc); c.load(h1 + (row0 + t0 - 1) * ld + Fp + colc); }
            if (t0 >= 2) { d.load(h1 + (row0 + t0 - 2) * ld + colc); e.load(h1 + (row0 + t0 - 2) * ld + Fp + colc); }
#pragma unroll
            for (int i = 0; i < 2; ++i) {
                x1v[i] = a.get(i); x1g[i] = c.get(i); x2v[i] = d.get(i); x2g[i] = e.get(i);
                p1v[i] = splat2(0.f); p1g[i] = splat2(0.f); p2v[i] = splat2(0.f); p2g[i] = splat2(0.f);
            }
        }
        Bwd3Row<T> cur, nx1, nx2;
        load_row(cur, row0 + t0);
        nx1 = cur;
        if (t0 + 1 < tlast) load_row(nx1, row0 + t0 + 1);
        __syncthreads();
        publish_sums(cur, t0 & 1);
        __syncthreads();
        const int tend = t1 + 2;
#pragma unroll 1
        for (int t = t0; t < tend; ++t) {
            nx2 = nx1;
            if (t + 2 < tlast) load_row(nx2, row0 + t + 2);

            if (t + 1 < tlast) publish_sums(nx1, (t + 1) & 1);
            v2 duv[2], dug[2];
            if (t < nseq) {
                v2 S12 = splat2(0.f);
#pragma unroll
                for (int w = 0; w < NW; ++w) S12 += *(const v2*)&red[t & 1][w][0];
                const float S1 = S12[0], S2 = S12[1];
                const float rs = cur.a * invF;
                const float bsum = rs * S1, csum = rs * S2;
                const float own = t < t1 ? 1.f : 0.f;
                v2 dy[2];
                dy_kept(cur, dy);
#pragma unroll
                for (int i = 0; i < 2; ++i) {
                    const v2 gh = cur.gh.get(i);
                    const v2 gy = dy[i] * gm[i];
                    dgam[i] = fma2(dy[i] * own, gh, dgam[i]);
                    v2 dg = fma2(gy, splat2(cur.a), splat2(-bsum));
                    dg = fma2(gh, splat2(-csum), dg);
                    const v2 xv = cur.xv.get(i), xg = cur.xg.get(i);
                    const v2 uv = fma2(wvr[2].get(i), xv, fma2(wvr[1].get(i), x1v[i], wvr[0].get(i) * x2v[i]));
                    const v2 ug = fma2(wgr[2].get(i), xg, fma2(wgr[1].get(i), x1g[i], wgr[0].get(i) * x2g[i]));
                    v2 h, ex;
                    gelu_parts(ug, h, ex);
                    const v2 gp = fma2(ug * 0.3989422804f, ex, h);
                    const v2 a_ = dg * (ug * h);
                    const v2 g_ = (dg * uv) * gp;
                    duv[i] = a_; dug[i] = g_;
                    const v2 ao = a_ * own, go = g_ * own;
                    dcv[0][i] = fma2(ao, x2v[i], dcv[0][i]); dcv[1][i] = fma2(ao, x1v[i], dcv[1][i]); dcv[2][i] = fma2(ao, xv, dcv[2][i]);
                    dcg[0][i] = fma2(go, x2g[i], dcg[0][i]); dcg[1][i] = fma2(go, x1g[i], dcg[1][i]); dcg[2][i] = fma2(go, xg, dcg[2][i]);
                    x2v[i] = x1v[i]; x1v[i] = xv; x2g[i] = x1g[i]; x1g[i] = xg;
                }
            } else {
#pragma unroll
                for (int i = 0; i < 2; ++i) { duv[i] = splat2(0.f); dug[i] = splat2(0.f); }
            }
            if (t - 2 >= t0 && act) {
                v2 ov[2], og[2];
#pragma unroll
                for (int i = 0; i < 2; ++i) {
                    ov[i] = fma2(wvr[0].get(i), duv[i], p2v[i]);
                    og[i] = fma2(wgr[0].get(i), dug[i], p2g[i]);
                }
                Ch4<T>::store(dh1 + (row0 + t - 2) * ld + col, ov);
                Ch4<T>::store(dh1 + (row0 + t - 2) * ld + Fp + col, og);
            }
#pragma unroll
            for (int i = 0; i < 2; ++i) {
                p2v[i] = fma2(wvr[1].get(i), duv[i], p1v[i]); p1v[i] = wvr[2].get(i) * duv[i];
                p2g[i] = fma2(wgr[1].get(i), dug[i], p1g[i]); p1g[i] = wgr[2].get(i) * dug[i];
            }
            cur = nx1; nx1 = nx2;
            __syncthreads();
        }
    }
    if (act) {
        float* pr = part_dconv + (size_t)blockIdx.y * 2 * F * 3;
        float* pg = part_dgamma + (size_t)blockIdx.y * Fp;
#pragma unroll
        for (int i = 0; i < 2; ++i)
#pragma unroll
            for (int e = 0; e < 2; ++e) {
                const int ch = col + 2 * i + e;
                pg[ch] = dgam[i][e];
                if (ch < F) {
#pragma unroll
                    for (int k = 0; k < 3; ++k) { pr[(size_t)ch * 3 + k] = dcv[k][i][e]; pr[(size_t)(F + ch) * 3 + k] = dcg[k][i][e]; }
                }
            }
    }
}

template <typename T, bool PL, bool MX>
static void strip_fwd_go(const FfmidLaunch& l, const FfmidArgs& a, const FfPlanes& pl) {
    const hipStream_t st = as_stream(a.stream);
    const dim3 grid(l.gx, l.gy), block(l.threads);
    const FfSeg seg{a.n_full, a.p0};
#define FF2_FWD(K_, NT_, ...) do { \
        if (l.train) hipLaunchKernelGGL((K_<T, NT_, true, PL, MX>), grid, block, 0, st, (const T*)a.h1, (const T*)a.convw, (const T*)a.gamma, (T*)a.h2, a.mean, a.rstd, \
                                        a.nseq, a.F, a.Fp, l.RB, l.strips, a.eps, a.p, a.seed, a.seed_dev, a.drop_bits, (T*)a.gh, pl, ##__VA_ARGS__); \
        else hipLaunchKernelGGL((K_<T, NT_, false, PL, MX>), grid, block, 0, st, (const T*)a.h1, (const T*)a.convw, (const T*)a.gamma, (T*)a.h2, a.mean, a.rstd, \
                                a.nseq, a.F, a.Fp, l.RB, l.strips, a.eps, a.p, a.seed, a.seed_dev, a.drop_bits, (T*)a.gh, pl, ##__VA_ARGS__); } while (0)
#define FF2_FWD_NT(K_, ...) switch (l.n) { \
        case 64: FF2_FWD(K_, 64, ##__VA_ARGS__); break; case 128: FF2_FWD(K_, 128, ##__VA_ARGS__); break; case 192: FF2_FWD(K_, 192, ##__VA_ARGS__); break; \
        case 256: FF2_FWD(K_, 256, ##__VA_ARGS__); break; case 320: FF2_FWD(K_, 320, ##__VA_ARGS__); break; case 384: FF2_FWD(K_, 384, ##__VA_ARGS__); break; \
        case 448: FF2_FWD(K_, 448, ##__VA_ARGS__); break; default: FF2_FWD(K_, 512, ##__VA_ARGS__); break; }
    if (l.kernel == FK_STRIP_FWD_SEG) FF2_FWD_NT(ffmid2_fwd_seg_kernel, seg)
    else FF2_FWD_NT(ffmid2_fwd_kernel)
#undef FF2_FWD_NT
#undef FF2_FWD
}

template <typename T>
static int ffmid2_launch_t(const FfmidLaunch& l, const FfmidArgs& a) {
    const hipStream_t st = as_stream(a.stream);
    const dim3 grid(l.gx, l.gy), block(l.threads);
    float* part_g = a.workspace;
    float* part_c = a.workspace ? a.workspace + ffmid_ws_dconv_at(a.Fp) : nullptr;
    float* bc = (float*)a.du_tmp;
    switch (l.kernel) {
    case FK_STRIP_FWD: case FK_STRIP_FWD_SEG: {
        FfPlanes pl{0, 0, 0, nullptr, nullptr, 0, nullptr, nullptr};
        if (!l.pl) strip_fwd_go<T, false, false>(l, a, pl);
        else if constexpr (sizeof(T) == 2) {
            pl.convw_lo = (const T*)a.convw_lo - (const T*)a.convw;
            pl.gamma_lo = (const T*)a.gamma_lo - (const T*)a.gamma;
            if (!l.mx) {
                pl.h1_lo = (const T*)a.h1_lo - (const T*)a.h1; pl.h2_lo = a.h2_lo;
                strip_fwd_go<T, true, false>(l, a, pl);
            }
#if OMLM_FP16
            else {
                pl.h1_8 = (const unsigned char*)a.h1_lo; pl.h2_8 = (unsigned char*)a.h2_8; pl.h2_8_stride = a.h2_8_stride; pl.scale8 = a.scale8;
                strip_fwd_go<T, true, true>(l, a, pl);
            }
#endif
        }
        return omlm_post_launch("omlm_ffmid_fwd (strip)");
    }
    case FK_BWD3: {
#define FF3_BWD(NT_) hipLaunchKernelGGL((ffmid3_bwd_kernel<T, NT_>), grid, block, 0, st, (const T*)a.dh2, (const T*)a.h1, (const T*)a.convw, (const T*)a.gamma, \
                       (const float*)a.rstd, (const T*)a.gh, (const unsigned char*)a.drop_bits, (T*)a.dh1, part_c, part_g, a.nseq, a.F, a.Fp, l.RB, l.strips, l.total, a.p)
        switch (l.n) { case 128: FF3_BWD(128); break; case 256: FF3_BWD(256); break; case 512: FF3_BWD(512); break; default: FF3_BWD(768); break; }
#undef FF3_BWD
        return omlm_post_launch("omlm_ffmid_bwd (fused strip)");
    }
    case FK_ROWSUM:
        launch_lds_optin<ffmid2_rowsum_kernel<T, FF_ROWSUM_MC>>(grid, block, (size_t)l.lds, st, (const T*)a.dh2, (const T*)a.gamma, (const T*)a.gh,
                                                                 (const unsigned char*)a.drop_bits, (const float*)a.rstd, bc, part_g, a.M, a.F, a.Fp, a.p);
        return omlm_post_launch("omlm_ffmid_bwd (row sums)");
    case FK_STRIP_BWD:
        hipLaunchKernelGGL(ffmid2_bwd_kernel<T>, grid, block, 0, st, (const T*)a.dh2, (const T*)a.h1, (const T*)a.convw, (const T*)a.gamma, (const float*)a.rstd,
                           (const float*)bc, (const T*)a.gh, (const unsigned char*)a.drop_bits, (T*)a.dh1, part_c, a.nseq, a.F, a.Fp, l.RB, l.strips, l.total, a.p);
        return omlm_post_launch("omlm_ffmid_bwd (strip)");
    default:
        omlm_set_error("omlm_ffmid: the plan names a kernel that ffmid2.hip does not build");
        return OMLM_ERR_UNSUPPORTED;
    }
}

int ffmid2_launch(const FfmidLaunch& l, const FfmidArgs& a) {
#if !OMLM_FP16
    if (!l.t16) return ffmid2_launch_t<float>(l, a);
#endif
    return ffmid2_launch_t<h16_t>(l, a);
}

}
```

open_musiclm_amd/csrc/ffmid_plan.h:

```cpp
#pragma once
#include <stdio.h>
#include <string.h>

#define FF_THREADS 256
#define FF_MAXC_LIMIT 16
#define FF_BWD1_BLOCKS 1024
#define FF_BWD2_STRIPS 512

namespace omlm_plan __attribute__((visibility("hidden"))) {

constexpr int FF_ERR_ARG = -1;
constexpr long long FF_LDS_CAP = 160 * 1024;
constexpr long long FF_LDS_OPT_IN = 48 * 1024;

constexpr int FF_MAX_FP = 8 * 64 * FF_MAXC_LIMIT;
constexpr int FF_STRIP_MAX_FP = 8 * 512;
constexpr int FF_ONE_PASS_MAX_FP = 4 * 768;
constexpr int FF_ROWSUM_MC = 8;
static inline bool ffmid_fp_ok(int F, int Fp) { return Fp % 8 == 0 && Fp >= F && Fp >= 0 && Fp <= FF_MAX_FP; }
static inline bool ffmid_strip_ok(int Fp) { return Fp % 8 == 0 && Fp / 8 <= FF_STRIP_MAX_FP / 8; }
static inline bool ffmid_one_pass(int Fp) { return Fp / 4 <= FF_ONE_PASS_MAX_FP / 4; }

static inline long long ffmid_ws_dconv_at(int Fp) { return (long long)FF_BWD1_BLOCKS * Fp; }
static inline long long ffmid_bwd_workspace_bytes(int F, int Fp) { return 4 * (ffmid_ws_dconv_at(Fp) + (long long)FF_BWD2_STRIPS * 2 * F * 3); }

static inline int ffmid_strip_rows(int nseq, int target) {
    const int n = (nseq + target - 1) / target;
    return (nseq + n - 1) / n;
}
static inline int ffmid_chunks_per_lane(int Fp) { return (Fp / 8 + 63) / 64; }
static inline int ffmid_maxc(int Fp) { const int mc = ffmid_chunks_per_lane(Fp); return mc <= 2 ? 2 : mc <= 6 ? 6 : mc <= 8 ? 8 : 16; }
static inline long long ffmid_row_lds(int Fp) { return 4ll * Fp * 4; }
static inline int colsum_ysplit(int P) { return P >= 1024 ? 128 : (P >= 64 ? 16 : 1); }

enum FfOp { FF_FWD, FF_FWD_PLANES, FF_FWD_MX, FF_BWD };
struct FfmidCall {
    FfOp op;
    int M, nseq, F, Fp;
    int dtype;
    bool fp16_copy;
    float p;
    bool operands;
    bool drop_bits, gh, dgamma, dconv;
    int n_full, p0;
    long long h2_8_stride;
    bool planes_aligned;
    bool du_aligned;
    int impl;
};
enum FfKernel {
    FK_FWD1, FK_BWD1, FK_BWD2,
    FK_STRIP_FWD, FK_STRIP_FWD_SEG, FK_ROWSUM, FK_STRIP_BWD, FK_BWD3,
    FK_COLSUM_G, FK_COLSUM_C, FK_COLSUM_GROUP
};
struct FfmidLaunch {
    FfKernel kernel;
    bool t16;
    int n;
    bool train, pl, mx, gh;
    int gx, gy, threads;
    long long lds;
    int RB, strips, total;
    int g_rows, c_rows;
};
struct FfmidPlan {
    int rc;
    char msg[384];
    bool strips;
    int n;
    FfmidLaunch l[4];
};

static inline FfmidPlan& ffmid_refuse(FfmidPlan& p, const char* text) {
    p.rc = FF_ERR_ARG; p.n = 0;
    snprintf(p.msg, sizeof(p.msg), "bad argument: %s", text);
    return p;
}
static inline FfmidLaunch& ffmid_push(FfmidPlan& p, FfKernel k, const FfmidCall& c, int n, int gx, int gy, int threads, long long lds) {
    FfmidLaunch& l = p.l[p.n++];
    memset(&l, 0, sizeof(l));
    l.kernel = k; l.t16 = c.dtype != 0; l.n = n; l.gx = gx; l.gy = gy; l.threads = threads; l.lds = lds;
    return l;
}
static inline void ffmid_push_colsums(FfmidPlan& p, const FfmidCall& c, int g_rows, int c_rows) {
    const int cg = c.F, cc = 2 * c.F * 3;
    if (c.dgamma && c.dconv) {
        FfmidLaunch& l = ffmid_push(p, FK_COLSUM_GROUP, c, 0, (cc + 255) / 256, colsum_ysplit(g_rows > c_rows ? g_rows : c_rows), 256, 0);
        l.g_rows = g_rows; l.c_rows = c_rows;
        return;
    }
    if (c.dgamma) ffmid_push(p, FK_COLSUM_G, c, 0, (cg + 255) / 256, colsum_ysplit(g_rows), 256, 0).g_rows = g_rows;
    if (c.dconv) ffmid_push(p, FK_COLSUM_C, c, 0, (cc + 255) / 256, colsum_ysplit(c_rows), 256, 0).c_rows = c_rows;
}

#define FF_REFUSE_UNLESS(cond, text) do { if (!(cond)) return ffmid_refuse(p, text); } while (0)

static inline FfmidPlan ffmid_plan(const FfmidCall& c) {
    FfmidPlan p;
    memset(&p, 0, sizeof(p));
    const int M = c.M, nseq = c.nseq, F = c.F, Fp = c.Fp;
    const bool fwd = c.op != FF_BWD, planes = c.op == FF_FWD_PLANES || c.op == FF_FWD_MX;
    const bool keep_ok = c.p == 0.f || c.drop_bits;
    if (c.op == FF_FWD_PLANES) FF_REFUSE_UNLESS(c.dtype == 1, "ffmid_fwd_planes: dtype 1 (bf16) or 2 (fp16) [dtype == 1]");
    else if (c.op != FF_FWD_MX) FF_REFUSE_UNLESS(!c.fp16_copy || c.dtype == 1, "the fp16 copy serves fp16 operands only [dtype == 1]");
    if (M <= 0) return p;
    if (fwd) FF_REFUSE_UNLESS(c.n_full == 0 || (c.p0 > 0 && c.p0 + nseq == c.n_full),
                              "row segment: nseq must be n_full - p0, p0 > 0 [(n_full) == 0 || ((p0) > 0 && (p0) + (nseq) == (n_full))]");
    FF_REFUSE_UNLESS(c.operands, c.op == FF_FWD ? "null pointer [h1 && convw && gamma && h2 && mean && rstd]" :
                                 c.op == FF_FWD_PLANES ? "null pointer [h1 && h1_lo && convw && convw_lo && gamma && gamma_lo && h2 && h2_lo && mean && rstd]" :
                                 c.op == FF_FWD_MX ? "null pointer [h1 && h1_lo && convw && convw_lo && gamma && gamma_lo && h2 && h2_8 && scale8 && mean && rstd]" :
                                                     "null pointer [dh2 && h1 && convw && gamma && mean && rstd && du_tmp && dh1 && workspace]");
    if (c.op == FF_FWD_PLANES)
        FF_REFUSE_UNLESS(Fp >= F && ffmid_strip_ok(Fp), "ffmid_fwd_planes: Fp must be F rounded up to 8 and <= 4096 [Fp % 8 == 0 && Fp >= F && ffmid2_supported(Fp)]");
    else if (c.op == FF_FWD_MX)
        FF_REFUSE_UNLESS(Fp >= F && ffmid_strip_ok(Fp), "ffmid_fwd_mx: Fp must be F rounded up to 8 and <= 4096 [Fp % 8 == 0 && Fp >= F && ffmid2_supported(Fp)]");
    else
        FF_REFUSE_UNLESS(ffmid_fp_ok(F, Fp), "Fp must be F rounded up to 8 and <= 8192 [Fp % 8 == 0 && Fp >= F && Fp <= 8192 && (size_t)5 * Fp * sizeof(float) <= 160 * 1024]");
    FF_REFUSE_UNLESS(nseq > 0 && M % nseq == 0, "M must be batch * nseq [nseq > 0 && M % nseq == 0]");
    if (planes) FF_REFUSE_UNLESS(c.p >= 0.f && c.p < 1.f && keep_ok, "dropout p (keep bits required when p > 0) [p >= 0.f && p < 1.f && (p == 0.f || drop_bits)]");
    else if (fwd) FF_REFUSE_UNLESS(c.p >= 0.f && c.p < 1.f, "dropout p [p >= 0.f && p < 1.f]");
    if (c.op == FF_FWD_MX) {
        FF_REFUSE_UNLESS(c.h2_8_stride >= (long long)M * 2 * Fp && c.h2_8_stride % 16 == 0,
                         "ffmid_fwd_mx: fp8 plane stride [h2_8_stride >= (long long)M * 2 * Fp && h2_8_stride % 16 == 0]");
        FF_REFUSE_UNLESS(2 * Fp >= (Fp + 127) / 128 * 128,
                         "ffmid_fwd_mx: an fp8 plane row (pitch 2 * Fp bytes) must hold Fp rounded up to 128 bytes [2 * Fp >= (Fp + 127) / 128 * 128]");
        FF_REFUSE_UNLESS(c.planes_aligned, "ffmid_fwd_mx: 16-byte aligned planes [(((uintptr_t)h1 | (uintptr_t)h1_lo | (uintptr_t)convw | (uintptr_t)convw_lo | "
                                           "(uintptr_t)gamma | (uintptr_t)gamma_lo | (uintptr_t)h2 | (uintptr_t)h2_8) % 16) == 0]");
    } else if (c.op == FF_FWD_PLANES) {
        FF_REFUSE_UNLESS(c.planes_aligned, "ffmid_fwd_planes: 16-byte aligned planes [(((uintptr_t)h1 | (uintptr_t)h1_lo | (uintptr_t)convw | (uintptr_t)convw_lo | "
                                           "(uintptr_t)gamma | (uintptr_t)gamma_lo | (uintptr_t)h2 | (uintptr_t)h2_lo) % 16) == 0]");
    }
    p.strips = planes || (c.impl == 1 && ffmid_strip_ok(Fp) && keep_ok && (fwd || c.gh));
    const int B = M / nseq, rows4 = (M + 3) / 4;
    if (fwd && p.strips) {
        const int RB = ffmid_strip_rows(nseq, 36), strips = (nseq + RB - 1) / RB, nt = ffmid_chunks_per_lane(Fp) * 64;
        const bool segd = c.n_full > 0 && c.p > 0.f;
        FfmidLaunch& l = ffmid_push(p, segd ? FK_STRIP_FWD_SEG : FK_STRIP_FWD, c, nt >= 64 && nt < 512 ? nt : 512, B * strips, 1, Fp / 8, 0);
        l.train = c.p > 0.f && c.drop_bits && c.gh;
        l.pl = planes; l.mx = c.op == FF_FWD_MX; l.RB = RB; l.strips = strips;
        return p;
    }
    if (fwd) {
        ffmid_push(p, FK_FWD1, c, ffmid_maxc(Fp), rows4 < 4096 ? rows4 : 4096, 1, FF_THREADS, ffmid_row_lds(Fp));
        return p;
    }
    if (!p.strips) {
        const int b1 = rows4 < FF_BWD1_BLOCKS ? rows4 : FF_BWD1_BLOCKS, strips = M < FF_BWD2_STRIPS ? M : FF_BWD2_STRIPS;
        ffmid_push(p, FK_BWD1, c, ffmid_maxc(Fp), b1, 1, FF_THREADS, ffmid_row_lds(Fp)).gh = c.gh;
        ffmid_push(p, FK_BWD2, c, 0, (2 * Fp / 8 + FF_THREADS - 1) / FF_THREADS, strips, FF_THREADS, 0);
        ffmid_push_colsums(p, c, b1, strips);
        return p;
    }
    FF_REFUSE_UNLESS(c.du_aligned, "du_tmp must be 8-byte aligned [((uintptr_t)du_tmp % 8) == 0]");
    const int RB = ffmid_strip_rows(nseq, 35), strips = (nseq + RB - 1) / RB, total = B * strips;
    const int per = (total + 255) / 256;
    int ny = (total + per - 1) / per, g_rows;
    if (ny > FF_BWD2_STRIPS) ny = FF_BWD2_STRIPS;
    if (ffmid_one_pass(Fp)) {
        const int nthr = (Fp / 4 + 63) / 64 * 64, nt = nthr <= 128 ? 128 : nthr <= 256 ? 256 : nthr <= 512 ? 512 : 768;
        FfmidLaunch& l = ffmid_push(p, FK_BWD3, c, nt, 1, ny, nt, 0);
        l.RB = RB; l.strips = strips; l.total = total;
        g_rows = ny;
    } else {
        g_rows = rows4 < FF_BWD1_BLOCKS ? rows4 : FF_BWD1_BLOCKS;
        ffmid_push(p, FK_ROWSUM, c, FF_ROWSUM_MC, g_rows, 1, 256, ffmid_row_lds(Fp));
        FfmidLaunch& l = ffmid_push(p, FK_STRIP_BWD, c, 0, (Fp / 4 + 255) / 256, ny, 256, 0);
        l.RB = RB; l.strips = strips; l.total = total;
    }
    ffmid_push_colsums(p, c, g_rows, ny);
    return p;
}
#undef FF_REFUSE_UNLESS

struct FfmidArgs {
    const void *h1, *convw, *gamma, *h1_lo, *convw_lo, *gamma_lo;
    void *h2, *h2_lo, *h2_8;
    unsigned char* scale8;
    float *mean, *rstd;
    const void* dh2;
    void *du_tmp, *dh1;
    float *dgamma, *dconv, *workspace;
    int M, nseq, F, Fp;
    float eps, p;
    unsigned long long seed;
    const unsigned long long* seed_dev;
    unsigned char* drop_bits;
    void* gh;
    int n_full, p0;
    long long h2_8_stride;
    void* stream;
};

}

#ifdef OMLM_PLAN_TEST_ABI
extern "C" void omlm_plan_ffmid(const int* v, double p, long long h2_8_stride, long long* out, char* msg) {
    const omlm_plan::FfmidCall c = {(omlm_plan::FfOp)v[0], v[1], v[2], v[3], v[4], v[5], v[6] != 0, (float)p, v[7] != 0, v[8] != 0, v[9] != 0, v[10] != 0,
                                    v[11] != 0, v[12], v[13], h2_8_stride, v[14] != 0, v[15] != 0, v[16]};
    const omlm_plan::FfmidPlan q = omlm_plan::ffmid_plan(c);
    out[0] = q.rc; out[1] = q.strips; out[2] = q.n;
    for (int i = 0; i < q.n; ++i) {
        const omlm_plan::FfmidLaunch& l = q.l[i];
        const long long w[16] = {l.kernel, l.t16, l.n, l.train, l.pl, l.mx, l.gh, l.gx, l.gy, l.threads, l.lds, l.RB, l.strips, l.total, l.g_rows, l.c_rows};
        memcpy(out + 3 + 16 * i, w, sizeof(w));
    }
    memcpy(msg, q.msg, sizeof(q.msg));
}
extern "C" void omlm_plan_ffmid_limits(int* out) {
    const int v[5] = {omlm_plan::FF_MAX_FP, omlm_plan::FF_STRIP_MAX_FP, omlm_plan::FF_ONE_PASS_MAX_FP, FF_BWD1_BLOCKS, FF_BWD2_STRIPS};
    memcpy(out, v, sizeof(v));
}
extern "C" int omlm_plan_ffmid_fp_ok(int F, int Fp) { return omlm_plan::ffmid_fp_ok(F, Fp); }
extern "C" int omlm_plan_ffmid_strip_ok(int Fp) { return omlm_plan::ffmid_strip_ok(Fp); }
extern "C" int omlm_plan_ffmid_one_pass(int Fp) { return omlm_plan::ffmid_one_pass(Fp); }
extern "C" long long omlm_plan_ffmid_bwd_workspace_bytes(int F, int Fp) { return omlm_plan::ffmid_bwd_workspace_bytes(F, Fp); }
extern "C" long long omlm_plan_ffmid_ws_dconv_at(int Fp) { return omlm_plan::ffmid_ws_dconv_at(Fp); }
#endif
```

open_musiclm_amd/engine.py:

```python
from __future__ import annotations

import math
import os
from dataclasses import dataclass, field
from typing import Dict, List, Optional, Sequence, Tuple

import torch

from . import ops
from .hip import require_gpu

ATTN_SCALE = 8.0
DIM_HEAD = 64

_PRECISIONS = {"bf16": torch.bfloat16, "bf16x3": torch.float32, "fp16": torch.float16, "fp16ff": torch.float16}


def is_half(precision: str) -> bool:
    return precision in ("fp16", "fp16ff")
_H16 = (torch.bfloat16, torch.float16)



FF_PLANES_MAX_FP = 4096


def ff_planes_ok(Fp: int) -> bool:
    return Fp <= FF_PLANES_MAX_FP


def ff_mx_ok(D: int, Fp: int) -> bool:
    return D % 64 == 0 and D <= 4096 and Fp % 64 == 0 and ff_planes_ok(Fp)


def default_precision() -> str:
    p = os.environ.get("OMLM_PRECISION", "bf16")
    if p not in _PRECISIONS:
        raise ValueError(f"OMLM_PRECISION must be one of {list(_PRECISIONS)}, got {p}")
    return p


def loss_scale_initial() -> float:
    return float(os.environ.get("OMLM_FP16_LOSS_SCALE", "4096"))


def loss_scale_state(model) -> torch.Tensor:
    dev = model.start_tokens[0].device
    st = model.__dict__.get("_omlm_ls_state")
    if st is None or st.device != dev:
        st = torch.tensor([loss_scale_initial(), 0.0, 0.0, 0.0, loss_scale_initial()], device=dev, dtype=torch.float32)
        model.__dict__["_omlm_ls_state"] = st
    return st


def loss_scale(precision: str, model=None) -> float:
    if not is_half(precision):
        return 1.0
    if model is None or "_omlm_ls_state" not in model.__dict__:
        return loss_scale_initial()
    return float(model.__dict__["_omlm_ls_state"][0].item())


_MODEL_OF: Dict[int, tuple] = {}


def tag_parameters(model, precision: Optional[str]):
    import weakref
    ref = weakref.ref(model)
    for p in model.parameters():
        p._omlm_precision = precision
        key = id(p)
        _MODEL_OF[key] = (weakref.ref(p, lambda _r, k=key: _MODEL_OF.pop(k, None)), ref)


def model_of(p) -> Optional[torch.nn.Module]:
    ent = _MODEL_OF.get(id(p))
    if ent is None or ent[0]() is not p:
        return None
    return ent[1]()


@torch.no_grad()
def unscale_grads_(model, precision: Optional[str] = None):
    s = loss_scale(precision or getattr(model, "precision", None) or default_precision(), model)
    if s != 1.0:
        for p in model.parameters():
            if p.grad is not None:
                p.grad.mul_(1.0 / s)


def ceil_to(x: int, m: int) -> int:
    return (x + m - 1) // m * m


def grad_of(p: torch.Tensor) -> torch.Tensor:
    if p.grad is None:
        p.grad = torch.zeros_like(p, memory_format=torch.contiguous_format)
    return p.grad


@dataclass
class SeqLayout:
    B: int
    N: int
    lens: Tuple[int, ...]
    starts: Tuple[int, ...]
    n_out: Tuple[int, ...]
    seg: torch.Tensor
    posidx: torch.Tensor
    start_col: torch.Tensor
    final_only: bool = False
    head_maps: Dict[Tuple[int, int], Tuple[torch.Tensor, torch.Tensor, int]] = field(default_factory=dict)
    live_maps: Dict[Tuple[int, int, int], torch.Tensor] = field(default_factory=dict)


def build_layout(B: int, lens: Sequence[int], quantizers: Sequence[int], device, final_rows_only: bool = False) -> SeqLayout:
    starts, pos = [], 0
    for l in lens:
        starts.append(pos)
        pos += l + 1
    N = pos
    seg = torch.empty(N, dtype=torch.int32)
    posidx = torch.zeros(N, dtype=torch.int32)
    start_col = torch.zeros(N, dtype=torch.bool)
    for s, (st, l) in enumerate(zip(starts, lens)):
        seg[st: st + l + 1] = s
        start_col[st] = True
        posidx[st + 1: st + l + 1] = torch.arange(l, dtype=torch.int32)
    n_out = [l for l in lens[:-1]] + [lens[-1] + 1]
    lay = SeqLayout(B, N, tuple(lens), tuple(starts), tuple(n_out), seg.to(device), posidx.to(device),
                    start_col.to(device), final_rows_only)
    if final_rows_only:
        s, st, n_s, Q = len(lens) - 1, starts[-1], n_out[-1], quantizers[-1]
        b = torch.arange(B)
        a_map = (b * N + st + n_s - 1).to(torch.int32)
        lay.head_maps[(s, (n_s - 1) % Q)] = (a_map.to(device), b.to(torch.int32).to(device), B)
        return lay
    for s, (st, n_s, Q) in enumerate(zip(starts, n_out, quantizers)):
        for qq in range(Q):
            js = torch.arange(qq, n_s, Q)
            if js.numel() == 0:
                continue
            b = torch.arange(B)[:, None]
            a_map = (b * N + st + js[None, :]).reshape(-1).to(torch.int32)
            c_map = (b * n_s + js[None, :]).reshape(-1).to(torch.int32)
            lay.head_maps[(s, qq)] = (a_map.to(device), c_map.to(device), int(a_map.numel()))
    return lay


CONV_HALO = 2
LIVE_K_MULTIPLE = 64
FF_ONE_PASS_MAX_FP = 3072


def first_live_row(lay: SeqLayout, want: Sequence[bool]) -> Optional[int]:
    firsts = [st for st, n_s, w in zip(lay.starts, lay.n_out, want) if w and n_s > 0]
    return min(firsts) if firsts else None


def live_rows(lay: SeqLayout, want: Sequence[bool], B: int, T: torch.dtype, Fp: int, halo: int = CONV_HALO) -> Optional[Tuple[int, int, int]]:
    if os.environ.get("OMLM_LIVE_ROWS", "1") == "0":
        return None
    if lay.final_only or T == torch.float32 or Fp > FF_ONE_PASS_MAX_FP:
        return None
    first = first_live_row(lay, want)
    if first is None:
        return None
    N = lay.N
    g = LIVE_K_MULTIPLE // math.gcd(B, LIVE_K_MULTIPLE)
    top = first - halo
    if top < 0:
        return None
    p0 = top - (top - N) % g
    if p0 <= 0 or 16 * p0 < N:
        return None
    return N, p0, N - p0


def live_to_full(r, seg: Tuple[int, int, int]):
    n_full, p0, n_live = seg
    return (r // n_live) * n_full + p0 + r % n_live


def full_to_live(r, seg: Tuple[int, int, int]):
    n_full, p0, n_live = seg
    return (r // n_full) * n_live + r % n_full - p0


def head_map(lay: SeqLayout, s: int, qq: int, live: Optional[Tuple[int, int, int]]):
    ent = lay.head_maps.get((s, qq))
    if ent is None or live is None:
        return ent
    a_map, c_map, rows = ent
    key = (s, qq, live[1])
    if key not in lay.live_maps:
        lay.live_maps[key] = full_to_live(a_map, live).to(torch.int32)
    return lay.live_maps[key], c_map, rows


def h16_operand(w: torch.Tensor, T: torch.dtype) -> torch.Tensor:
    sh = getattr(w, "_omlm_bf16", None)
    if (sh is not None and sh.dtype == T and getattr(w, "_omlm_bf16_version", -1) == w._version and sh.device == w.device):
        return sh
    c = torch.empty(w.shape, dtype=T, device=w.device)
    ops.cast_pad(w.detach(), c, w.numel() // w.shape[-1], w.shape[-1], w.shape[-1], w.shape[-1])
    return c


class PreparedWeights:
    def __init__(self, model, precision: str, persistent: bool = True):
        tr = model.transformer
        self.precision = precision
        self.T = _PRECISIONS[precision]
        self.ff3 = precision == "fp16ff"
        T = self.T
        dev = model.start_tokens[0].device
        D = tr.dim
        Fp_all = {ceil_to(ff.inner_dim, 64) for _, _, ff in tr.layers}
        self.ff_planes = self.ff3 and all(ff_planes_ok(f) for f in Fp_all)
        self.mx = self.ff_planes and all(ff_mx_ok(D, f) for f in Fp_all)
        quants = ops.QuantRowsGroup()
        self.layers = []
        wbuf = model.__dict__.setdefault("_omlm_wbuf", {})
        packs = ops.CastPadGroup()
        for li, (attn, _, ff) in enumerate(tr.layers):
            F = ff.inner_dim
            Fp = ceil_to(F, 64)
            w1 = ff.w_in.weight
            w2 = ff.w_out.weight
            ent = {}
            if T == torch.float32:
                ent["Wq"], ent["Wkv"], ent["Wo"] = attn.to_q.weight, attn.to_kv.weight, attn.to_out[0].weight
            else:
                for name, w in (("Wq", attn.to_q.weight), ("Wkv", attn.to_kv.weight), ("Wo", attn.to_out[0].weight)):
                    ent[name] = h16_operand(w, T)
            bkey = (li, T, str(dev), F, D)
            if not persistent:
                W1p, W2p, convp, gammap = (torch.zeros(2 * Fp, D, dtype=T, device=dev), torch.zeros(D, Fp, dtype=T, device=dev),
                                           torch.zeros(3, 2 * Fp, dtype=T, device=dev), torch.zeros(Fp, dtype=T, device=dev))
            else:
                if bkey not in wbuf:
                    wbuf[bkey] = (torch.zeros(2 * Fp, D, dtype=T, device=dev), torch.zeros(D, Fp, dtype=T, device=dev),
                                  torch.zeros(3, 2 * Fp, dtype=T, device=dev), torch.zeros(Fp, dtype=T, device=dev))
                W1p, W2p, convp, gammap = wbuf[bkey]
            packs.add(w1.detach(), W1p, F, D, D, D)
            packs.add(w1.detach()[F:], W1p[Fp:], F, D, D, D)
            packs.add(w2.detach(), W2p, D, F, F, Fp)
            ent["W1p"], ent["W2p"], ent["F"], ent["Fp"] = W1p, W2p, F, Fp
            if self.ff_planes:
                lkey = bkey + ("lo",)
                if not persistent or lkey not in wbuf:
                    lo = (torch.zeros(2 * Fp, D, dtype=T, device=dev), torch.zeros(D, Fp, dtype=T, device=dev),
                          torch.zeros(3, 2 * Fp, dtype=T, device=dev), torch.zeros(Fp, dtype=T, device=dev))
                    if persistent:
                        wbuf[lkey] = lo
                else:
                    lo = wbuf[lkey]
                W1l, W2l, convl, gammal = lo
                if not (self.mx and persistent):
                    packs.add(w1.detach(), W1l, F, D, D, D, lo=True)
                    packs.add(w1.detach()[F:], W1l[Fp:], F, D, D, D, lo=True)
                    packs.add(w2.detach(), W2l, D, F, F, Fp, lo=True)
                ent["W1p_lo"], ent["W2p_lo"], ent["convw_lo"], ent["gamma_mid_lo"] = W1l, W2l, convl, gammal
            if self.mx:
                mkey = bkey + ("mx",)
                if not persistent or mkey not in wbuf:
                    m8 = (ops.Fp8Planes(2 * Fp, D, dev), ops.Fp8Planes(D, Fp, dev))
                    if persistent:
                        wbuf[mkey] = m8
                else:
                    m8 = wbuf[mkey]
                quants.add(w1.detach(), m8[0], 0, F, D, D)
                quants.add(w1.detach()[F:], m8[0], Fp, F, D, D)
                quants.add(w2.detach(), m8[1], 0, D, F, F)
                ent["W1p8"], ent["W2p8"] = m8
            cw = ff.conv_weight().detach().reshape(2 * F, 3)
            packs.add(cw, convp, F, 3, 3, 2 * Fp, transpose=True)
            packs.add(cw[F:], convp[:, Fp:], F, 3, 3, 2 * Fp, transpose=True)
            packs.add(ff.norm_mid.gamma.detach(), gammap, 1, F, F, Fp)
            ent["convw"], ent["gamma_mid"] = convp, gammap
            if self.ff_planes:
                packs.add(cw, ent["convw_lo"], F, 3, 3, 2 * Fp, transpose=True, lo=True)
                packs.add(cw[F:], ent["convw_lo"][:, Fp:], F, 3, 3, 2 * Fp, transpose=True, lo=True)
                packs.add(ff.norm_mid.gamma.detach(), ent["gamma_mid_lo"], 1, F, F, Fp, lo=True)
            cache = ff.__dict__.setdefault("_omlm_cmap", {})
            if (F, Fp, str(dev)) not in cache:
                cm = torch.full((2 * Fp,), -1, dtype=torch.int32)
                cm[:F] = torch.arange(F, dtype=torch.int32)
                cm[Fp:Fp + F] = torch.arange(F, 2 * F, dtype=torch.int32)
                cache[(F, Fp, str(dev))] = cm.to(dev)
            ent["dW1_cmap"] = cache[(F, Fp, str(dev))]
            self.layers.append(ent)
        self.heads_lo = []
        if self.ff3:
            for w in model.logit_weights:
                lo = torch.empty(w.shape, dtype=T, device=dev)
                packs.add(w.detach().reshape(-1, D), lo.view(-1, D), w.numel() // D, D, D, D, lo=True)
                self.heads_lo.append(lo)
        packs.flush()
        quants.flush()
        self.heads = [w if T == torch.float32 else h16_operand(w, T) for w in model.logit_weights]


def prepared_weights(model, precision: str) -> PreparedWeights:
    key = (precision, sum(p._version for p in model.parameters()), tuple(p.data_ptr() for p in model.parameters()))
# ... 124 lines not shown
    ops.colsum_accumulate(dtable, grad_of(lin[3].bias), n, H, ldb)
    gw = grad_of(lin[3].weight)
    ops.gemm(dtable, zs[2], gw, M=H, N=Hd, K=n, a_kmajor=True, b_kmajor=True, Cin=gw, lda=ldb)
    dz = torch.empty(n, Hd, device=dev)
    ops.gemm(dtable, lin[3].weight.detach(), dz, M=n, N=Hd, K=ldb, b_kmajor=True, lda=ldb, b_rows=H)
    for k in (2, 1):
        ds = torch.empty(n, Hd, device=dev)
        ops.silu_bwd(dz, pres[k], ds, n * Hd)
        ops.colsum_accumulate(ds, grad_of(lin[k].bias), n, Hd, Hd)
        gw = grad_of(lin[k].weight)
        ops.gemm(ds, zs[k - 1], gw, M=Hd, N=Hd, K=n, a_kmajor=True, b_kmajor=True, Cin=gw, planes=False)
        dz = torch.zeros(n, Hd, device=dev)
        ops.gemm(ds, lin[k].weight.detach(), dz, M=n, N=Hd, K=Hd, b_kmajor=True, Cin=dz, planes=False)
    ds = torch.empty(n, Hd, device=dev)
    ops.silu_bwd(dz, pres[0], ds, n * Hd)
    ops.colsum_accumulate(ds, grad_of(lin[0].bias), n, Hd, Hd)
    ops.relpos_first_bwd(ds, grad_of(lin[0].weight).view(-1), n, Hd, x0=x0)


class LayerSaved:
    __slots__ = ("x", "m1", "r1", "xn", "xc", "q_raw", "kv_raw", "q", "k", "v", "o", "lse", "abias",
                 "x1", "m2", "r2", "xn2", "h1", "h2", "m3", "r3", "seed", "p", "drop_bits", "gh", "h1_lo_tail",
                 "pa", "sa", "po", "so")


def _dropout_state(tr, dev):
    st = tr.__dict__.get("_omlm_dropout")
    if st is None or st["counter"].device != dev:
        rank = int(os.environ.get("RANK", "0"))
        g = torch.Generator().manual_seed((int(torch.initial_seed()) + 0x9E3779B1 * rank) & 0x7FFFFFFF)
        L = len(tr.layers)
        st = dict(counter=torch.zeros(1, dtype=torch.int64, device=dev),
                  seeds=[int(v) for v in torch.randint(1, 2 ** 62, (L,), generator=g)])
        a = [int(v) for v in torch.randint(1, 2 ** 62, (2 * L,), generator=g)]
        st["attn_seeds"], st["out_seeds"] = a[:L], a[L:]
        st["last"] = None
        tr.__dict__["_omlm_dropout"] = st
    return st


def dropout_salt(tr, dev) -> torch.Tensor:
    st = _dropout_state(tr, dev)
    st["counter"].add_(1)
    st["last"] = st["counter"].clone()
    return st["last"], st["seeds"]


def dropout_state(tr, dev=None) -> dict:
    st = tr.__dict__.get("_omlm_dropout")
    if st is None:
        st = _dropout_state(tr, dev if dev is not None else torch.device("cpu"))
    last = st["last"]
    return dict(ff=list(st["seeds"]), attn=list(st["attn_seeds"]), out=list(st["out_seeds"]),
                salt=int(last.item()) if last is not None else None)


def trunk_forward(tr, pw: PreparedWeights, x: torch.Tensor, keymask: Optional[torch.Tensor], B: int, N: int,
                  save: bool, training: bool, keep_h1_lo_tail: bool = False, live: Optional[Tuple[int, int, int]] = None):
    T = pw.T
    dev = x.device
    M, D = x.shape
    H = tr.heads
    P = prefix_rows(tr)
    rc = tr.__dict__.get("_omlm_relpos_cache")
    if rc is not None and save and training and rc.usable(N):
        table, rp_saved = rc.table, ("cached", rc)
    else:
        table, rp_saved = relpos_forward(tr, N, save, P)
        if (rc is not None and rc.enabled and rc.n is None and save and training and rp_saved is not None and rp_saved[0] != "t5"
                and not torch.cuda.is_current_stream_capturing()):
            rc.adopt(N, table, rp_saved)
            rp_saved = ("cached", rc)
    saved_layers: List[LayerSaved] = []
    abiases = None
    assert live is None or (len(tr.layers) > 0 and not keep_h1_lo_tail and live[0] == N)
    salt, seeds, aseeds, oseeds = (None, None, None, None)
    aps = [(float(a_.attn_dropout.p), float(a_.to_out[1].p)) if training else (0.0, 0.0) for a_, _, _ in tr.layers]
    if training and (any(float(ff.dropout_p) > 0 for _, _, ff in tr.layers) or any(pa > 0 or po > 0 for pa, po in aps)):
        salt, seeds = dropout_salt(tr, dev)
        st_ = tr.__dict__["_omlm_dropout"]
        aseeds, oseeds = st_["attn_seeds"], st_["out_seeds"]
    for li, ((attn, _, ff), w) in enumerate(zip(tr.layers, pw.layers)):
        sv = LayerSaved()
        F, Fp = w["F"], w["Fp"]
        m1 = torch.empty(M, device=dev); r1 = torch.empty(M, device=dev)
        xn = torch.empty(M, D, dtype=T, device=dev)
        xc = x if T == torch.float32 else torch.empty(M, D, dtype=T, device=dev)
        ops.layernorm_fwd(x, attn.norm.gamma.detach(), xn, None if T == torch.float32 else xc, m1, r1)
        q = torch.empty(M, H * DIM_HEAD, dtype=T, device=dev)
        k = torch.empty(M, DIM_HEAD, dtype=T, device=dev)
        v = torch.empty(M, DIM_HEAD, dtype=T, device=dev)
        fused_qk = T in _H16
        if fused_qk:
            qn = torch.empty(M, H, device=dev)
            kn = torch.empty(M, device=dev)
            q_raw, kv_raw = qn, kn
            ops.gemm_qknorm(xn, w["Wq"], q, attn.q_scale.detach(), qn, H, M=M, N=H * DIM_HEAD, K=D)
            ops.gemm_qknorm(xc, w["Wkv"], k, attn.k_scale.detach(), kn, 1, M=M, N=2 * DIM_HEAD, K=D, C2=v, c2_col0=DIM_HEAD)
        else:
            q_raw = torch.empty(M, H * DIM_HEAD, device=dev)
            kv_raw = torch.empty(M, 2 * DIM_HEAD, device=dev)
            ops.gemm(xn, w["Wq"], q_raw, M=M, N=H * DIM_HEAD, K=D)
            ops.gemm(xc, w["Wkv"], kv_raw, M=M, N=2 * DIM_HEAD, K=D)
            ops.qk_norm_fwd(q_raw, kv_raw, attn.q_scale.detach(), attn.k_scale.detach(), q, k, v, H)
        o = torch.empty(M, H * DIM_HEAD, dtype=T, device=dev)
        lse = torch.empty(B, H, N, device=dev)
        if abiases is None:
            abiases = ops.AttnBias.group(table, N, H, dev, [a_.q_scale.detach() for a_, _, _ in tr.layers],
                                         [a_.k_scale.detach() for a_, _, _ in tr.layers], scale=ATTN_SCALE, half=T == torch.float16, P=P)
        abias = abiases[li]
        pa, po = aps[li]
        sa = aseeds[li] if pa > 0 else 0
        so = oseeds[li] if po > 0 else 0
        ops.attn_fwd(q, k, v, abias, keymask, o, lse, B, N, H, ATTN_SCALE, P=P, p=pa, seed=sa, seed_dev=salt if pa > 0 else None)
        x1 = torch.empty(M, D, device=dev)
        if po > 0:
            yo = torch.empty(M, D, device=dev)
            ops.gemm(o, w["Wo"], yo, M=M, N=D, K=H * DIM_HEAD)
            ops.dropout_residual_fwd(x, yo, x1, po, so, seed_dev=salt)
            del yo
        else:
            ops.gemm(o, w["Wo"], x1, M=M, N=D, K=H * DIM_HEAD, Cin=x)
        seg = live if li == len(tr.layers) - 1 else None
        x1c = None
        if seg is not None:
            M = B * seg[2]
            nff = seg[2]
            x1c = torch.empty(M, D, device=dev)
        else:
            nff = N
        m2 = torch.empty(M, device=dev); r2 = torch.empty(M, device=dev)
        xn2 = torch.empty(M, D, dtype=T, device=dev)
        h1 = torch.empty(M, 2 * Fp, dtype=T, device=dev)
        if pw.mx:
            P1 = ops.Fp8Planes(M, D, dev, zero=False)
            ops.layernorm_fwd_mx(x1, ff.norm_in.gamma.detach(), xn2, P1, m2, r2, seg=seg, xc=x1c)
            h1_lo = torch.empty(M, 2 * Fp, dtype=torch.uint8, device=dev)
            ops.gemm_mx16(xn2, P1, w["W1p"], w["W1p8"], h1, h1_lo, M=M, N=2 * Fp, K=D)
        elif pw.ff_planes:
            xn2_lo = torch.empty(M, D, dtype=T, device=dev)
            ops.layernorm_fwd_planes(x1, ff.norm_in.gamma.detach(), xn2, xn2_lo, m2, r2, seg=seg, xc=x1c)
            h1_lo = torch.empty(M, 2 * Fp, dtype=T, device=dev)
            ops.gemm_planes16(xn2, xn2_lo, w["W1p"], w["W1p_lo"], h1, h1_lo, M=M, N=2 * Fp, K=D)
        else:
            ops.layernorm_fwd(x1, ff.norm_in.gamma.detach(), xn2, None, m2, r2, seg=seg, xc=x1c)
            ops.gemm(xn2, w["W1p"], h1, M=M, N=2 * Fp, K=D)
        if seg is not None:
            x1 = x1c
        h2 = torch.empty(M, Fp, dtype=T, device=dev)
        m3 = torch.empty(M, device=dev); r3 = torch.empty(M, device=dev)
        p = float(ff.dropout_p) if training else 0.0
        seed = seeds[li] if (p > 0 and seeds is not None) else 0
        drop_bits = torch.empty(M, Fp // 8, dtype=torch.uint8, device=dev) if (p > 0 and (save or pw.ff_planes)) else None
        gh = torch.empty(M, Fp, dtype=T, device=dev) if save else None
        x2 = torch.empty(M, D, device=dev)
        if pw.ff_planes:
            if pw.mx:
                P2 = ops.Fp8Planes(M, Fp, dev, zero=False)
                ops.ffmid_fwd_mx(h1, h1_lo, w["convw"], w["convw_lo"], w["gamma_mid"], w["gamma_mid_lo"], h2, P2, m3, r3, nff, F, Fp, p, seed,
                                 seed_dev=salt if p > 0 else None, drop_bits=drop_bits, gh=gh, seg=seg)
                ops.gemm_mx16(h2, P2, w["W2p"], w["W2p8"], x2, M=M, N=D, K=Fp, Cin=x1)
            else:
                h2_lo = torch.empty(M, Fp, dtype=T, device=dev)
                ops.ffmid_fwd_planes(h1, h1_lo, w["convw"], w["convw_lo"], w["gamma_mid"], w["gamma_mid_lo"], h2, h2_lo, m3, r3, nff, F, Fp, p, seed,
                                     seed_dev=salt if p > 0 else None, drop_bits=drop_bits, gh=gh, seg=seg)
                ops.gemm_planes16(h2, h2_lo, w["W2p"], w["W2p_lo"], x2, M=M, N=D, K=Fp, Cin=x1)
                del xn2_lo, h2_lo
            if keep_h1_lo_tail and save:
                take = min(2, N)
                sv.h1_lo_tail = torch.zeros(B, 2, 2 * Fp, device=dev)
                tail = h1_lo.view(B, N, -1)[:, N - take:]
                if tail.dtype == torch.uint8:
                    tail = (tail.contiguous().to(torch.int16) << 8).view(torch.float16)
                sv.h1_lo_tail[:, 2 - take:].copy_(tail)
            del h1_lo
        else:
            ops.ffmid_fwd(h1, w["convw"], w["gamma_mid"], h2, m3, r3, nff, F, Fp, p, seed, seed_dev=salt if p > 0 else None,
                          drop_bits=drop_bits, gh=gh, seg=seg)
            ops.gemm(h2, w["W2p"], x2, M=M, N=D, K=Fp, Cin=x1)
        if save:
            sv.x, sv.m1, sv.r1, sv.xn, sv.xc = x, m1, r1, xn, xc
            sv.q_raw, sv.kv_raw, sv.q, sv.k, sv.v, sv.o, sv.lse, sv.abias = q_raw, kv_raw, q, k, v, o, lse, abias
            sv.x1, sv.m2, sv.r2, sv.xn2, sv.h1, sv.h2, sv.m3, sv.r3, sv.seed, sv.p = x1, m2, r2, xn2, h1, h2, m3, r3, seed, p
            sv.drop_bits = drop_bits
            sv.gh = gh
            sv.pa, sv.sa, sv.po, sv.so = pa, sa, po, so
            saved_layers.append(sv)
        x = x2
    mf = torch.empty(M, device=dev); rf = torch.empty(M, device=dev)
    y, y_lo = torch.empty(M, D, dtype=T, device=dev), None
    if pw.ff3:
        y_lo = torch.empty(M, D, dtype=T, device=dev)
        ops.layernorm_fwd_planes(x, tr.norm.gamma.detach(), y, y_lo, mf, rf)
    else:
        ops.layernorm_fwd(x, tr.norm.gamma.detach(), y, None, mf, rf)
    saved = dict(layers=saved_layers, xL=x, mf=mf, rf=rf, table=table, rp=rp_saved, keymask=keymask, salt=salt, live=live) if save else None
    return y, y_lo, saved


def trunk_backward(tr, pw: PreparedWeights, saved, dy: torch.Tensor, B: int, N: int, out_scale: float, head_wgrads=None):
    T = pw.T
    dev = dy.device
    D = dy.shape[1]
    M_all = B * N
    live = saved.get("live")
    M = B * live[2] if live is not None else M_all
    assert dy.shape[0] == M
    H = tr.heads
    table, keymask = saved["table"], saved["keymask"]
    rp_cached = saved["rp"] is not None and saved["rp"][0] == "cached"
    dtable = (saved["rp"][1].dtable if rp_cached else torch.zeros_like(table)) if table is not None else None
    nl = len(saved["layers"])
    dres = torch.empty(M, D, device=dev)
    dres_c = dres if T == torch.float32 else torch.empty(M, D, dtype=T, device=dev)
    cg = ops.ColsumGroup()
    ops.layernorm_bwd(dy, saved["xL"], tr.norm.gamma.detach(), saved["mf"], saved["rf"], None, dres,
                      None if T == torch.float32 else dres_c, grad_of(tr.norm.gamma),
                      dx_scale=out_scale if nl == 0 else 1.0, defer=cg)
    ws = None
    wg = ops.WgradGroup() if T in _H16 else None
    for dYh, Xh, dWh, Mo, No in (head_wgrads or []):
        if wg is not None:
            wg.add(dYh, Xh, dWh, M=Mo, N=No, K=dYh.shape[0])
        else:
            ops.gemm(dYh, Xh, dWh, M=Mo, N=No, K=dYh.shape[0], a_kmajor=True, b_kmajor=True, Cin=dWh)

    def wgrad(dY, X, dW, Mo, No, c_map=None):
        K = dY.shape[0]
        if wg is not None:
            wg.add(dY, X, dW, M=Mo, N=No, K=K, c_map=c_map)
            if len(wg.items) >= 40:
                wg.flush()
        else:
            ops.gemm(dY, X, dW, M=Mo, N=No, K=K, a_kmajor=True, b_kmajor=True, Cin=dW, c_map=c_map)

    for li in range(nl - 1, -1, -1):
        attn, _, ff = tr.layers[li]
        w, sv = pw.layers[li], saved["layers"][li]
        F, Fp = w["F"], w["Fp"]
        seg = live if li == nl - 1 else None
        nff = seg[2] if seg is not None else N
        dh2 = torch.empty(M, Fp, dtype=T, device=dev)
        ops.gemm(dres_c, w["W2p"], dh2, M=M, N=Fp, K=D, b_kmajor=True)
        gW2 = grad_of(ff.w_out.weight)
        wgrad(dres_c, sv.h2, gW2, D, F)
        if ws is None or ws.numel() < ops.ffmid_bwd_workspace_floats(F, Fp):
            ws = torch.empty(ops.ffmid_bwd_workspace_floats(F, Fp), device=dev)
        du = torch.empty(M, 2 * Fp, dtype=T, device=dev)
        dh1 = torch.empty(M, 2 * Fp, dtype=T, device=dev)
        gconv = grad_of(ff.conv_param()).view(-1) if ff.conv_param() is not None else None
        ops.ffmid_bwd(dh2, sv.h1, w["convw"], w["gamma_mid"], sv.m3, sv.r3, du, dh1,
                      grad_of(ff.norm_mid.gamma), gconv, ws, nff, F, Fp, sv.p, sv.seed,
                      seed_dev=saved["salt"] if sv.p > 0 else None, drop_bits=sv.drop_bits, gh=sv.gh)
        del du, dh2
        dxn2 = torch.empty(M, D, dtype=T, device=dev)
        ops.gemm(dh1, w["W1p"], dxn2, M=M, N=D, K=2 * Fp, b_kmajor=True)
        gW1 = grad_of(ff.w_in.weight)
        wgrad(dh1, sv.xn2, gW1, 2 * Fp, D, c_map=w["dW1_cmap"])
        del dh1
        M = M_all
        dx1 = torch.empty(M, D, device=dev)
        dx1_c = dx1 if T == torch.float32 else torch.empty(M, D, dtype=T, device=dev)
        ops.layernorm_bwd(dxn2, sv.x1, ff.norm_in.gamma.detach(), sv.m2, sv.r2, dres, dx1,
                          None if T == torch.float32 else dx1_c, grad_of(ff.norm_in.gamma), defer=cg, seg=seg)
        dyo = dx1_c
        if sv.po > 0:
            dyo = torch.empty(M, D, dtype=T, device=dev)
            ops.dropout_residual_bwd(dx1, dyo, sv.po, sv.so, seed_dev=saved["salt"])
        do = torch.empty(M, H * DIM_HEAD, dtype=T, device=dev)
        ops.gemm(dyo, w["Wo"], do, M=M, N=H * DIM_HEAD, K=D, b_kmajor=True)
        gWo = grad_of(attn.to_out[0].weight)
        wgrad(dyo, sv.o, gWo, D, H * DIM_HEAD)
        dq = torch.empty(M, H * DIM_HEAD, device=dev)
        dkv = torch.empty(2, M, DIM_HEAD, device=dev)
        dk, dv = dkv[0], dkv[1]
        delta = torch.empty(B, H, N, device=dev)
        ops.attn_bwd(sv.q, sv.k, sv.v, sv.abias, keymask, sv.o, do, sv.lse, delta, dq, dk, dv, dtable, B, N, H, ATTN_SCALE, P=prefix_rows(tr),
                     p=sv.pa, seed=sv.sa, seed_dev=saved["salt"] if sv.pa > 0 else None)
        dq_raw = torch.empty(M, H * DIM_HEAD, dtype=T, device=dev)
        dkv_raw = torch.empty(M, 2 * DIM_HEAD, dtype=T, device=dev)
        if T in _H16:
            ops.qk_norm_bwd2(dq, dk, dv, sv.q, sv.k, sv.q_raw, sv.kv_raw, attn.q_scale.detach(), attn.k_scale.detach(),
                             dq_raw, dkv_raw, grad_of(attn.q_scale), grad_of(attn.k_scale), H)
        else:
            ops.qk_norm_bwd(dq, dk, dv, sv.q_raw, sv.kv_raw, attn.q_scale.detach(), attn.k_scale.detach(),
                            dq_raw, dkv_raw, grad_of(attn.q_scale), grad_of(attn.k_scale), H)
        dxn = torch.empty(M, D, dtype=T, device=dev)
        kv16 = T in _H16
        tmp = torch.empty(M, D, dtype=T if kv16 else torch.float32, device=dev)
        ops.gemm(dq_raw, w["Wq"], dxn, M=M, N=D, K=H * DIM_HEAD, b_kmajor=True)
        ops.gemm(dkv_raw, w["Wkv"], tmp, M=M, N=D, K=2 * DIM_HEAD, b_kmajor=True, Cin=None if kv16 else dx1)
        gWq = grad_of(attn.to_q.weight)
        wgrad(dq_raw, sv.xn, gWq, H * DIM_HEAD, D)
        gWkv = grad_of(attn.to_kv.weight)
        wgrad(dkv_raw, sv.xc, gWkv, 2 * DIM_HEAD, D)
        dres = torch.empty(M, D, device=dev)
        dres_c = dres if T == torch.float32 else torch.empty(M, D, dtype=T, device=dev)
        last = li == 0
        ops.layernorm_bwd(dxn, sv.x, attn.norm.gamma.detach(), sv.m1, sv.r1, dx1 if kv16 else tmp, dres,
                          None if (T == torch.float32 or last) else dres_c, grad_of(attn.norm.gamma),
                          dx_scale=out_scale if last else 1.0, dres2=tmp if kv16 else None, defer=cg)
    cg.flush()
    if wg is not None:
        wg.flush()
    if dtable is not None and saved["rp"] is not None and not rp_cached:
        relpos_backward(tr, N, saved["rp"], dtable)
    return dres


def build_ids(model, all_token_ids: Sequence[torch.Tensor]) -> Tuple[torch.Tensor, List[int]]:
    parts, lens = [], []
    for seq, ids in zip(model.token_sequences, all_token_ids):
        ids = ids.reshape(ids.shape[0], -1)
        if seq.num_quantizers > 1:
            off = seq.codebook_size * (torch.arange(ids.shape[-1], device=ids.device) % seq.num_quantizers)
            ids = ids + off
        lens.append(ids.shape[-1])
        parts += [torch.full((ids.shape[0], 1), -2, device=ids.device, dtype=torch.int32), ids.to(torch.int32)]
    return torch.cat(parts, dim=1).contiguous(), lens


class PreparedIds:
    __slots__ = ("ids32", "lens")

    def __init__(self, ids32: torch.Tensor, lens: Sequence[int]):
        self.ids32, self.lens = ids32, list(lens)


def get_layout(model, B: int, lens: Sequence[int], device, final_rows_only: bool) -> SeqLayout:
    cache = model.__dict__.setdefault("_omlm_layouts", {})
    key = (B, tuple(lens), str(device), final_rows_only)
    if key not in cache:
        if len(cache) > 64:
            cache.clear()
        cache[key] = build_layout(B, lens, [s.num_quantizers for s in model.token_sequences], device, final_rows_only)
    return cache[key]


def embed_forward(model, ids32: torch.Tensor, lay: SeqLayout) -> torch.Tensor:
    B, N = ids32.shape
    D = model.dim
    x = torch.empty(B * N, D, device=ids32.device)
    pos = [e.weight.detach() for e in model.absolute_position_embeddings] if model.use_absolute_position_embeddings else None
    ops.embed_fwd(ids32, lay.seg, lay.posidx, [e.weight.detach() for e in model.embeddings],
                  [s.detach() for s in model.start_tokens], pos, x.view(B, N, D))
    return x


def embed_backward(model, ids32: torch.Tensor, lay: SeqLayout, dx: torch.Tensor, alpha: float):
    B, N = ids32.shape
    dpos = [grad_of(e.weight) for e in model.absolute_position_embeddings] if model.use_absolute_position_embeddings else None
    ops.embed_bwd(ids32, lay.seg, lay.posidx, [grad_of(e.weight) for e in model.embeddings],
                  [grad_of(s) for s in model.start_tokens], dpos, dx.view(B, N, -1), alpha)


def heads_forward(model, pw: PreparedWeights, y: torch.Tensor, y_lo: Optional[torch.Tensor], lay: SeqLayout, want: Sequence[bool],
                  live: Optional[Tuple[int, int, int]] = None):
    D = model.dim
    out = []
    for s, seq in enumerate(model.token_sequences):
        if not want[s]:
            out.append(None)
            continue
        V1 = seq.codebook_size + 1
        ldV = ceil_to(V1, 8)
        n_s = lay.n_out[s]
        buf = torch.empty(lay.B if lay.final_only else lay.B * n_s, ldV, device=y.device)
        for qq in range(seq.num_quantizers):
            ent = head_map(lay, s, qq, live)
            if ent is None:
                continue
            a_map, c_map, rows = ent
            if y_lo is not None:
                ops.gemm_planes16(y, y_lo, pw.heads[s][qq], pw.heads_lo[s][qq], buf, M=rows, N=V1, K=D, a_map=a_map, c_map=c_map, ldc=ldV,
                                  a_rows=y.shape[0], b_rows=V1)
                continue
            ops.gemm(y, pw.heads[s][qq], buf, M=rows, N=V1, K=D, a_map=a_map, c_map=c_map, ldc=ldV,
                     a_rows=y.shape[0], b_rows=V1)
        out.append(buf)
    return out


def heads_backward(model, pw: PreparedWeights, y: torch.Tensor, lay: SeqLayout, dlogits: Sequence[Optional[torch.Tensor]],
                   deferred: Optional[list] = None, live: Optional[Tuple[int, int, int]] = None):
    D = model.dim
    dy = torch.zeros(y.shape[0], D, device=y.device)
    for s, seq in enumerate(model.token_sequences):
        dl = dlogits[s]
        if dl is None:
            continue
        V1 = seq.codebook_size + 1
        ldV = dl.shape[-1]
        gW = grad_of(model.logit_weights[s])
        for qq in range(seq.num_quantizers):
            ent = head_map(lay, s, qq, live)
            if ent is None:
                continue
            a_map, c_map, rows = ent
            ops.gemm(dl, pw.heads[s][qq], dy, M=rows, N=D, K=ldV, b_kmajor=True, a_map=c_map, c_map=a_map,
                     a_rows=dl.shape[0], b_rows=V1)
            if deferred is not None and rows >= 1024:
                rp = ceil_to(rows, 64)
                gd = torch.empty(rp, dl.shape[-1], dtype=dl.dtype, device=dl.device)
                gy = torch.empty(rp, y.shape[-1], dtype=y.dtype, device=y.device)
                torch.index_select(dl, 0, c_map, out=gd[:rows])
                torch.index_select(y, 0, a_map, out=gy[:rows])
# ... 181 lines not shown
```

open_musiclm_amd/hip.py:

```python
from __future__ import annotations

import ctypes as C
import os
from typing import Optional

import torch

_HERE = os.path.dirname(os.path.abspath(__file__))
LIB_PATH = os.environ.get("OMLM_LIB_PATH") or os.path.join(_HERE, "libomlm_hip.so")

_lib: Optional[C.CDLL] = None

vp, i32, i64, f32, u64, f64, u32 = C.c_void_p, C.c_int, C.c_longlong, C.c_float, C.c_ulonglong, C.c_double, C.c_uint

SIGNATURES = {
    "omlm_version": [],
    "omlm_last_error": [],
    "omlm_set_error": [C.c_char_p],
    "omlm_gemm": [vp, vp, vp, vp, vp, vp, vp, i64, i64, i32, i32, i32, i32, i32, i32, i32, i32, i32, i32, i32, f32, vp, i64, vp],
    "omlm_gemm_tail_workspace_bytes": [i32, i32],
    "omlm_gemm_wgrad_group": [vp, i32, i32, i32, vp],
    "omlm_gemm_planes": [vp, i64, vp, i64, vp, vp, vp, vp, vp, i64, i64, i32, i32, i32, i32, i32, i32, i32, i32, i32, i32, f32, vp, i64, vp],
    "omlm_split_planes": [vp, vp, i64, i64, vp],
    "omlm_gemm_planes16": [vp, vp, vp, vp, vp, vp, vp, vp, vp, i64, i64, i32, i32, i32, i32, i32, i32, i32, i32, vp, i64, vp],
    "omlm_gemm_mx16": [vp, vp, i64, vp, vp, vp, i64, vp, vp, vp, i32, vp, i64, i64, i32, i32, i32, i32, i32, i32, i32, vp, i64, vp],
    "omlm_gemm_mx16_workspace_bytes": [i32, i32, i32],
    "omlm_layernorm_fwd_mx": [vp, vp, vp, vp, i64, vp, vp, vp, i32, i32, i32, f32, vp],
    "omlm_ffmid_fwd_mx": [vp, vp, vp, vp, vp, vp, vp, vp, i64, vp, vp, vp, i32, i32, i32, i32, f32, f32, u64, vp, vp, vp, vp],
    "omlm_layernorm_fwd_mx_seg": [vp, vp, vp, vp, i64, vp, vp, vp, vp, i32, i32, i32, f32, i32, i32, i32, vp],
    "omlm_ffmid_fwd_mx_seg": [vp, vp, vp, vp, vp, vp, vp, vp, i64, vp, vp, vp, i32, i32, i32, i32, f32, f32, u64, vp, vp, vp, i32, i32, vp],
    "omlm_quant_rows_mx": [vp, i32, vp],
    "omlm_layernorm_fwd_planes": [vp, vp, vp, vp, vp, vp, i32, i32, i32, f32, i32, vp],
    "omlm_ffmid_fwd_planes": [vp, vp, vp, vp, vp, vp, vp, vp, vp, vp, i32, i32, i32, i32, f32, f32, u64, vp, vp, vp, i32, vp],
    "omlm_layernorm_fwd": [vp, vp, vp, vp, vp, vp, i32, i32, i32, f32, i32, vp],
    "omlm_layernorm_fwd_seg": [vp, vp, vp, vp, vp, vp, vp, i32, i32, i32, f32, i32, i32, i32, i32, vp],
    "omlm_layernorm_fwd_planes_seg": [vp, vp, vp, vp, vp, vp, vp, i32, i32, i32, f32, i32, i32, i32, i32, vp],
    "omlm_layernorm_bwd2_seg": [vp, vp, vp, vp, vp, vp, vp, vp, vp, vp, vp, i32, i32, f32, i32, i32, i32, i32, i32, vp],
    "omlm_layernorm_bwd_workspace_bytes": [i32],
    "omlm_layernorm_bwd2": [vp, vp, vp, vp, vp, vp, vp, vp, vp, vp, vp, i32, i32, f32, i32, i32, vp],
    "omlm_qk_norm_fwd": [vp, vp, vp, vp, vp, vp, vp, i32, i32, i32, vp],
    "omlm_qk_norm_bwd": [vp, vp, vp, vp, vp, vp, vp, vp, vp, vp, vp, i32, i32, i32, vp],
    "omlm_gemm_qknorm": [vp, vp, vp, vp, i32, i32, vp, vp, i32, i32, i64, i64, i32, i32, i32, i32, i32, i32, i32, vp],
    "omlm_qk_norm_bwd2": [vp, vp, vp, vp, vp, vp, vp, vp, vp, vp, vp, vp, vp, i32, i32, i32, vp],
    "omlm_attn_bias_table_floats": [i32, i32, i32],
    "omlm_attn_bias_prepare": [vp, vp, i32, i32, i32, vp, vp, f32, f32, i32, vp],
    "omlm_attn_bias_prepare_group": [vp, vp, i32, i32, i32, i32, vp, vp, f32, f32, i32, i32, vp],
    "omlm_mqa_attn_fwd": [vp] * 8 + [i32, i32, i32, f32, i32, i32, i32, f32, u64, vp, vp],
    "omlm_mqa_attn_bwd": [vp] * 15 + [i32, i32, i32, f32, i32, i32, i32, f32, u64, vp, vp],
    "omlm_mqa_attn_bwd_workspace_bytes": [i32, i32, i32],
    "omlm_attn_max_positions": [i32, i32],
    "omlm_attn_dropout_keep": [vp, i32, i32, i32, f32, u64, vp, vp],
    "omlm_dropout_residual_fwd": [vp, vp, vp, i64, i32, f32, u64, vp, vp],
    "omlm_dropout_residual_bwd": [vp, vp, i64, i32, f32, u64, vp, i32, vp],
    "omlm_ffmid_fwd": [vp, vp, vp, vp, vp, vp, i32, i32, i32, i32, f32, f32, u64, vp, vp, vp, i32, vp],
    "omlm_ffmid_fwd_seg": [vp, vp, vp, vp, vp, vp, i32, i32, i32, i32, f32, f32, u64, vp, vp, vp, i32, i32, i32, vp],
    "omlm_ffmid_fwd_planes_seg": [vp, vp, vp, vp, vp, vp, vp, vp, vp, vp, i32, i32, i32, i32, f32, f32, u64, vp, vp, vp, i32, i32, i32, vp],
    "omlm_ffmid_bwd_workspace_bytes": [i32, i32],
    "omlm_ffmid_bwd": [vp, vp, vp, vp, vp, vp, vp, vp, vp, vp, vp, i32, i32, i32, i32, f32, u64, vp, vp, vp, i32, vp],
    "omlm_colsum_accumulate": [vp, vp, i32, i32, i32, vp],
    "omlm_colsum_group": [vp, i32, vp],
    "omlm_ffmid_set_impl": [i32],
    "omlm_embed_gather_fwd": [vp, vp, vp, vp, vp, vp, i32, vp, i32, i32, i32, vp, vp, vp, vp],
    "omlm_embed_gather_bwd": [vp, vp, vp, vp, vp, vp, i32, vp, i32, i32, i32, f32, vp, vp, vp, vp],
    "omlm_prepare_train_batch": [vp, vp, vp, vp, vp, vp, i32, i32, i32, vp, i32, vp, vp, i32, vp, f32, vp],
    "omlm_cross_entropy_fwd": [vp, vp, vp, vp, i32, i32, i32, vp, vp],
    "omlm_cross_entropy_bwd": [vp, vp, vp, vp, f32, vp, i32, i32, i32, i32, i32, vp],
    "omlm_cross_entropy_fwd_reg": [vp, vp, vp, vp, i32, i32, i32, vp, vp],
    "omlm_cross_entropy_bwd_reg": [vp, vp, vp, vp, f32, vp, i32, i32, i32, i32, i32, f32, f32, vp],
    "omlm_sumsq_accumulate": [vp, i64, vp, vp, vp],
    "omlm_adamw_clip_step": [vp, vp, vp, vp, vp, i64, f32, f32, f32, f32, f32, i32, f32, vp, f32, i32, i32, i32, vp, vp],
    "omlm_adamw_clip_step_ema": [vp, vp, vp, vp, vp, i64, f32, f32, f32, f32, f32, i32, f32, vp, f32, i32, i32, i32, vp, vp, f32, i32, i32, vp],
    "omlm_loss_scale_update": [vp, vp, f32, f32, i32, f32, f32, vp],
    "omlm_cast_pad": [vp, vp, i64, i32, i32, i32, i32, vp],
    "omlm_cast_pad_group": [vp, i32, i32, vp],
    "omlm_sample_topk_gumbel_at": [vp, vp, vp, vp, vp, i32, i32, i32, i32, f32, i32, vp],
    "omlm_sample_embed_at": [vp, vp, vp, vp, vp, i32, i32, i32, i32, f32, i32, vp, i64, i64, vp, i32, vp],
    "omlm_decode_step": [vp, vp, vp],
    "omlm_decode_advance": [vp, vp, vp],
    "omlm_relpos_first_fwd": [vp, vp, vp, vp, i32, i32, i32, vp],
    "omlm_relpos_first_bwd": [vp, vp, i32, i32, i32, vp],
    "omlm_bias_silu_fwd": [vp, vp, vp, vp, i64, i32, vp],
    "omlm_silu_bwd": [vp, vp, vp, i64, vp],
    "omlm_bias_add": [vp, vp, vp, i32, i32, i32, vp],
    "omlm_relpos_mlp_fwd": [vp] * 15 + [i32, i32, i32, i32, i32, vp],
    "omlm_relpos_mlp_bwd": [vp] * 19 + [i32, i32, i32, i32, i32, vp],
    "omlm_rvq_encode": [vp, vp, vp, vp, i32, i32, i32, i32, i32, vp],
    "omlm_nearest_centroid": [vp, vp, vp, i32, i32, i32, vp],
    "omlm_vq_accumulate": [vp, vp, i32, vp, vp, i32, i32, i32, vp],
    "omlm_vq_kmeans_update": [vp, vp, vp, vp, i32, i32, vp],
    "omlm_vq_ema_update": [vp, vp, vp, vp, vp, vp, vp, i32, i32, f32, f32, vp],
    "omlm_kmeans_pp_workspace_bytes": [i32, i32],
    "omlm_kmeans_pp_pick": [vp] * 9 + [i64, i32, i32, i32, i32, vp],
    "omlm_kmeans_pp_seed": [vp] * 9 + [i64, i32, i32, i32, i32, vp],
    "omlm_kmeans_minibatch_step": [vp] * 10 + [i32, i32, i32, i32, f64, f64, i32, vp],
    "omlm_kmeans_inertia": [vp, vp, vp, vp, i32, i32, i32, vp],
    "omlm_sample_topk_gumbel": [vp, vp, vp, i32, i32, i32, i32, f32, i32, vp],
    "omlm_sample_topk_gumbel_rng": [vp, u32, u32, i32, i32, vp, i32, i32, i32, i32, f32, i32, vp],
    "omlm_sample_topk_gumbel_at_rng": [vp, u32, u32, vp, i32, vp, vp, i32, i32, i32, i32, f32, i32, vp],
    "omlm_sample_embed_at_rng": [vp, u32, u32, vp, i32, vp, vp, i32, i32, i32, i32, f32, i32, vp, i64, i64, vp, i32, vp],
    "omlm_sample": [vp, vp],
    "omlm_sample_lp": [vp, vp, vp, vp],
    "omlm_sample_rows": [vp, vp, vp, vp, vp],
    "omlm_guide_logits": [vp, vp, vp, i32, i32, i32, f32, vp],
    "omlm_guide_logits_rows": [vp, vp, vp, i32, i32, i32, vp, vp],
    "omlm_decode_twin": [vp, vp, vp, vp, i32, i32, vp],
    "omlm_probe_tr16": [vp, vp],
}
_RESTYPES = {"omlm_last_error": C.c_char_p, "omlm_gemm_tail_workspace_bytes": C.c_longlong, "omlm_gemm_mx16_workspace_bytes": C.c_longlong, "omlm_ffmid_bwd_workspace_bytes": C.c_longlong,
             "omlm_attn_bias_table_floats": C.c_longlong, "omlm_mqa_attn_bwd_workspace_bytes": C.c_longlong,
             "omlm_layernorm_bwd_workspace_bytes": C.c_longlong, "omlm_kmeans_pp_workspace_bytes": C.c_longlong,
             "omlm_set_error": None}


class HipLibraryMissing(RuntimeError):
    pass


def lib() -> C.CDLL:
    global _lib
    if _lib is None:
        if not os.path.exists(LIB_PATH):
            raise HipLibraryMissing(
                f"{LIB_PATH} not found: build it with `python -c 'import __graft_entry__ as g; g.build()'` "
                "(or `make -C open_musiclm_amd/csrc`). There is no CPU fallback for the MI355X hot path.")
        l = C.CDLL(LIB_PATH)
        for name, args in SIGNATURES.items():
            fn = getattr(l, name)
            fn.argtypes = args
            fn.restype = _RESTYPES.get(name, C.c_int)
        _lib = l
    return _lib


def stream_ptr() -> int:
    return torch.cuda.current_stream().cuda_stream


def ptr(t: Optional[torch.Tensor]):
    if t is None:
        return None
    return t.data_ptr()


def call(name: str, *args):
    rc = getattr(lib(), name)(*args)
    if rc != 0:
        msg = lib().omlm_last_error()
        raise RuntimeError(f"{name} failed (rc={rc}): {msg.decode() if msg else '?'}")


def require_gpu(t: torch.Tensor, what: str = "tensor"):
    if not t.is_cuda:
        raise RuntimeError(
            f"open_musiclm_amd: {what} is on {t.device}; the TokenConditionedTransformer path only runs on an "
            "MI355X through libomlm_hip.so (no CPU fallback). Move the model and inputs to 'cuda'.")
    cur = torch.cuda.current_device()
    if t.device.index != cur:
        raise RuntimeError(f"open_musiclm_amd: {what} lives on cuda:{t.device.index} but the current device is cuda:{cur}; "
                           "call torch.cuda.set_device(LOCAL_RANK) and keep the model and its inputs on that device")
```

open_musiclm_amd/ops.py:

```python
from __future__ import annotations

import ctypes as C
import os
import weakref
from typing import Optional, Sequence

import torch

from . import hip
from .ema import check_ema_settings
from .hip import call, ptr, stream_ptr

F32, BF16, F16 = 0, 1, 2
_CODES = {torch.float32: F32, torch.bfloat16: BF16, torch.float16: F16}
H16 = (torch.bfloat16, torch.float16)


def dcode(dtype: torch.dtype) -> int:
    try:
        return _CODES[dtype]
    except KeyError:
        raise TypeError(f"unsupported operand dtype {dtype}") from None


# ... 321 lines not shown
    call("omlm_qk_norm_bwd2", ptr(dq), ptr(dk), ptr(dv), ptr(q), ptr(k), ptr(qn), ptr(kn), ptr(q_scale), ptr(k_scale),
         ptr(dq_raw), ptr(dkv_raw), ptr(dq_scale), ptr(dk_scale), q.shape[0], H, dcode(dq_raw.dtype), stream_ptr())


class AttnBias:

    def __init__(self, table: Optional[torch.Tensor], N: int, H: int, device=None, q_scale=None, k_scale=None,
                 qk_bound: float = 0.0, scale: float = 8.0, half: bool = False, _tableT: Optional[torch.Tensor] = None, _P: int = 0):
        self.table, self.N, self.H, self.P = table, N, H, _P
        dev = table.device if table is not None else device
        if _tableT is not None:
            self.tableT = _tableT
            return
        self.tableT = torch.empty(int(hip.lib().omlm_attn_bias_table_floats(N, H, 0)), device=dev)
        call("omlm_attn_bias_prepare", ptr(table), ptr(self.tableT), N, H, table.shape[-1] if table is not None else 0,
             ptr(q_scale), ptr(k_scale), float(qk_bound), float(scale), 15 if half else 0, stream_ptr())

    @staticmethod
    def group(table: Optional[torch.Tensor], N: int, H: int, device, q_scales, k_scales, scale: float = 8.0, half: bool = False, P: int = 0):
        L = len(q_scales)
        dev = table.device if table is not None else device
        buf = torch.empty(L, int(hip.lib().omlm_attn_bias_table_floats(N, H, P)), device=dev)
        outs = (C.c_void_p * L)(*[buf[l].data_ptr() for l in range(L)])
        qs = (C.c_void_p * L)(*[t.data_ptr() for t in q_scales])
        ks = (C.c_void_p * L)(*[t.data_ptr() for t in k_scales])
        for t in list(q_scales) + list(k_scales):
            hip.require_gpu(t, "scale")
        call("omlm_attn_bias_prepare_group", ptr(table), C.cast(outs, C.c_void_p), L, N, H, table.shape[-1] if table is not None else 0,
             C.cast(qs, C.c_void_p), C.cast(ks, C.c_void_p), 0.0, float(scale), 15 if half else 0, int(P), stream_ptr())
        return [AttnBias(table, N, H, dev, _tableT=buf[l], _P=P) for l in range(L)]


def _attn_tables(bias, N, H, P, device):
    if isinstance(bias, AttnBias):
        if bias.P != P:
            raise ValueError(f"attention with P = {P} handed an AttnBias prepared for P = {bias.P}")
        return bias.table, bias.tableT
    return bias, (AttnBias(bias, N, H, device).tableT if P == 0 else None)


def _dbias_workspace(B: int, N: int, H: int, device) -> torch.Tensor:
    n = int(hip.lib().omlm_mqa_attn_bwd_workspace_bytes(B, N, H)) // 4
    key = str(device)
    ws = _DBIAS_WS.get(key)
    if ws is None or ws.numel() < n:
        if ws is not None:
            _DBIAS_RETIRED.append(ws)
        ws = _DBIAS_WS[key] = torch.empty(n, device=device, dtype=torch.float32)
    return ws


def attn_max_positions(dtype, P: int = 0) -> int:
    return int(hip.lib().omlm_attn_max_positions(dcode(dtype), int(P)))


def _check_positions(what, N, dtype, P):
    if P == 0 and dtype in H16 and N > attn_max_positions(dtype, 0):
        raise RuntimeError(f"{what}: N = {N} positions per sample is past the limit of {attn_max_positions(dtype, 0)} "
                           f"(omlm_attn_max_positions) of causal attention with {dtype} operands")


def attn_fwd(q, k, v, bias, keymask, out, lse, B, N, H, scale, P=0, p=0.0, seed=0, seed_dev=None):
    _check_positions("attn_fwd", N, q.dtype, P)
    table, tableT = _attn_tables(bias, N, H, P, q.device)
    call("omlm_mqa_attn_fwd", ptr(q), ptr(k), ptr(v), ptr(table), ptr(tableT), ptr(keymask), ptr(out), ptr(lse), B, N, H, float(scale),
         table.shape[-1] if table is not None else 0, dcode(q.dtype), int(P), float(p), int(seed), ptr(seed_dev), stream_ptr())


def attn_bwd(q, k, v, bias, keymask, out, dout, lse, delta, dq, dk, dv, dbias, B, N, H, scale, P=0, workspace=True, p=0.0, seed=0,
             seed_dev=None):
    _check_positions("attn_bwd", N, q.dtype, P)
    table, tableT = _attn_tables(bias, N, H, P, q.device)
    ws = _dbias_workspace(B, N, H, q.device) if dbias is not None and workspace else None
    ld = table.shape[-1] if table is not None else (dbias.shape[-1] if dbias is not None else 0)
    call("omlm_mqa_attn_bwd", ptr(q), ptr(k), ptr(v), ptr(table), ptr(tableT), ptr(keymask), ptr(out), ptr(dout), ptr(lse), ptr(delta), ptr(dq),
         ptr(dk), ptr(dv), ptr(dbias), ptr(ws), B, N, H, float(scale), ld, dcode(q.dtype), int(P), float(p), int(seed), ptr(seed_dev),
         stream_ptr())


def attn_dropout_keep(B, N, H, p, seed, seed_dev=None, device=None) -> torch.Tensor:
    keep = torch.empty(B, H, N, N, dtype=torch.uint8, device=device if device is not None else seed_dev.device)
    call("omlm_attn_dropout_keep", ptr(keep), B, N, H, float(p), int(seed), ptr(seed_dev), stream_ptr())
    return keep


def dropout_residual_fwd(x, y, x1, p, seed, seed_dev=None):
    call("omlm_dropout_residual_fwd", ptr(x), ptr(y), ptr(x1), x.shape[0], x.shape[1], float(p), int(seed), ptr(seed_dev), stream_ptr())


def dropout_residual_bwd(dx1, dy, p, seed, seed_dev=None):
    call("omlm_dropout_residual_bwd", ptr(dx1), ptr(dy), dx1.shape[0], dx1.shape[1], float(p), int(seed), ptr(seed_dev), dcode(dy.dtype),
         stream_ptr())


def pack_conv_taps(convw: torch.Tensor, F: int, Fp: int) -> torch.Tensor:
    out = torch.zeros(3, 2 * Fp, device=convw.device, dtype=torch.float32)
    out[:, :F] = convw[:F].t()
    out[:, Fp:Fp + F] = convw[F:].t()
    return out


def pad_vector(v: torch.Tensor, n: int) -> torch.Tensor:
    out = torch.zeros(n, device=v.device, dtype=torch.float32)
    out[: v.numel()] = v
    return out


def _ff_seg(seg, nseq):
    if seg is None:
        return 0, 0
    assert seg[2] == nseq and seg[1] + seg[2] == seg[0]
    return int(seg[0]), int(seg[1])


def ffmid_fwd(h1, convw, gamma, h2, mean, rstd, nseq, F, Fp, p, seed, eps=1e-5, seed_dev=None, drop_bits=None, gh=None, seg=None):
    assert convw.shape == (3, 2 * Fp) and gamma.numel() == Fp
    assert convw.dtype == h1.dtype and gamma.dtype == h1.dtype, "taps / gamma travel in the operand dtype of h1"
    call("omlm_ffmid_fwd_seg", ptr(h1), ptr(convw), ptr(gamma), ptr(h2), ptr(mean), ptr(rstd),
         h1.shape[0], nseq, F, Fp, float(eps), float(p), int(seed), ptr(seed_dev), ptr(drop_bits), ptr(gh), dcode(h1.dtype),
         *_ff_seg(seg, nseq), stream_ptr())


def ffmid_fwd_planes(h1, h1_lo, convw, convw_lo, gamma, gamma_lo, h2, h2_lo, mean, rstd, nseq, F, Fp, p, seed, eps=1e-5, seed_dev=None,
                     drop_bits=None, gh=None, seg=None):
    assert convw.shape == (3, 2 * Fp) and gamma.numel() == Fp and h1.dtype in H16
    for t in (h1_lo, convw, convw_lo, gamma, gamma_lo, h2, h2_lo):
        assert t.dtype == h1.dtype, "every plane travels in the operand dtype of h1"
    assert h1_lo.shape == h1.shape and h2_lo.shape == h2.shape and convw_lo.shape == convw.shape
    call("omlm_ffmid_fwd_planes_seg", ptr(h1), ptr(h1_lo), ptr(convw), ptr(convw_lo), ptr(gamma), ptr(gamma_lo), ptr(h2), ptr(h2_lo), ptr(mean),
         ptr(rstd), h1.shape[0], nseq, F, Fp, float(eps), float(p), int(seed), ptr(seed_dev), ptr(drop_bits), ptr(gh), dcode(h1.dtype),
         *_ff_seg(seg, nseq), stream_ptr())


def ffmid_fwd_mx(h1, h1_lo, convw, convw_lo, gamma, gamma_lo, h2, P: "Fp8Planes", mean, rstd, nseq, F, Fp, p, seed, eps=1e-5, seed_dev=None,
                 drop_bits=None, gh=None, seg=None):
    assert convw.shape == (3, 2 * Fp) and gamma.numel() == Fp and h1.dtype == torch.float16 and h1_lo.dtype == torch.uint8
    for t in (convw, convw_lo, gamma, gamma_lo, h2):
        assert t.dtype == h1.dtype, "every plane travels in the operand dtype of h1"
    assert h1_lo.shape == h1.shape and convw_lo.shape == convw.shape and P.ld == Fp and P.rows >= h1.shape[0]
    call("omlm_ffmid_fwd_mx_seg", ptr(h1), ptr(h1_lo), ptr(convw), ptr(convw_lo), ptr(gamma), ptr(gamma_lo), ptr(h2), ptr(P.planes), P.stride,
         ptr(P.scale), ptr(mean), ptr(rstd), h1.shape[0], nseq, F, Fp, float(eps), float(p), int(seed), ptr(seed_dev), ptr(drop_bits), ptr(gh),
         *_ff_seg(seg, nseq), stream_ptr())


def ffmid_set_impl(impl: int):
    call("omlm_ffmid_set_impl", int(impl))


def ffmid_bwd_workspace_floats(F, Fp) -> int:
    return int(hip.lib().omlm_ffmid_bwd_workspace_bytes(F, Fp)) // 4


def ffmid_bwd(dh2, h1, convw, gamma, mean, rstd, du_tmp, dh1, dgamma, dconv, workspace, nseq, F, Fp, p, seed, seed_dev=None,
              drop_bits=None, gh=None):
    assert convw.shape == (3, 2 * Fp) and gamma.numel() == Fp
    assert convw.dtype == h1.dtype and gamma.dtype == h1.dtype, "taps / gamma travel in the operand dtype of h1"
    call("omlm_ffmid_bwd", ptr(dh2), ptr(h1), ptr(convw), ptr(gamma), ptr(mean), ptr(rstd), ptr(du_tmp), ptr(dh1),
         ptr(dgamma), ptr(dconv), ptr(workspace), h1.shape[0], nseq, F, Fp, float(p), int(seed), ptr(seed_dev), ptr(drop_bits),
         ptr(gh), dcode(h1.dtype), stream_ptr())


def _ptr_array(tensors: Sequence[Optional[torch.Tensor]]):
    arr = (C.c_void_p * len(tensors))()
    for i, t in enumerate(tensors):
        arr[i] = ptr(t) if t is not None else None
    return arr


_INDEX_ERR = {}


def index_error_flag(device) -> torch.Tensor:
    key = str(device)
    if key not in _INDEX_ERR:
        _INDEX_ERR[key] = torch.zeros(1, dtype=torch.int32, device=device)
    return _INDEX_ERR[key]


def raise_on_index_error(device):
    flag = _INDEX_ERR.get(str(device))
    if flag is None:
        return
    v = int(flag.item())
    if v:
        flag.zero_()
        what = [n for b, n in ((1, "token id >= embedding rows"), (2, "position >= absolute position rows"), (4, "label >= vocabulary")) if v & b]
        raise IndexError("open_musiclm_amd: " + ", ".join(what) + " (rows were skipped; check codebook sizes / the token store)")


def _rows_array(tensors):
    if tensors is None:
        return None
    return (C.c_longlong * len(tensors))(*[int(t.shape[0]) if t is not None else 0 for t in tensors])


def embed_fwd(ids, seg, posidx, tables, starts, pos_tables, out):
    B, N = ids.shape
    D = out.shape[-1]
    pos_arr = _ptr_array(pos_tables) if pos_tables is not None else None
    call("omlm_embed_gather_fwd", ptr(ids), ptr(seg), ptr(posidx), _ptr_array(tables), _ptr_array(starts),
         pos_arr, len(tables), ptr(out), B, N, D, _rows_array(tables), _rows_array(pos_tables), ptr(index_error_flag(out.device)),
         stream_ptr())


def embed_bwd(ids, seg, posidx, dtables, dstarts, dpos_tables, dx, alpha):
    B, N = ids.shape
    D = dx.shape[-1]
    pos_arr = _ptr_array(dpos_tables) if dpos_tables is not None else None
    call("omlm_embed_gather_bwd", ptr(ids), ptr(seg), ptr(posidx), _ptr_array(dtables), _ptr_array(dstarts),
         pos_arr, len(dtables), ptr(dx), B, N, D, float(alpha), _rows_array(dtables), _rows_array(dpos_tables),
         ptr(index_error_flag(dx.device)), stream_ptr())


def check_null_cond_prob(p, name="null_cond_prob"):
    try:
        v = float("nan") if isinstance(p, (str, bytes, bool)) else float(p)
    except (TypeError, ValueError):
        v = float("nan")
    if not (0.0 <= v <= 1.0):
        raise ValueError(f"{name} must be a number in [0, 1], not {p!r}")
    return v


FP32_MAX = 3.4028234663852886e38


def check_cond_scale(cond_scale, name="cond_scale"):
    if cond_scale is None:
        return None
    try:
        s = float("nan") if isinstance(cond_scale, (str, bytes, bool)) else float(cond_scale)
    except (TypeError, ValueError):
        s = float("nan")
    if not (0.0 <= s <= FP32_MAX):
        raise ValueError(f"{name} must be None or a finite number >= 0 (as fp32), not {cond_scale!r}")
    return None if s == 1.0 else s


def guide_logits(cond, null, out, V, scale):
    by_row = isinstance(scale, torch.Tensor) and scale.dim() == 1
    s = None if by_row else check_cond_scale(scale, "scale")
    rows, ld = cond.shape
    if by_row:
        hip.require_gpu(scale, "scale")
        if scale.dtype != torch.float32 or scale.shape != (rows,) or not scale.is_contiguous():
            raise ValueError(f"guide_logits: a per-row scale must be a contiguous fp32 tensor [{rows}]; got {scale.dtype} {tuple(scale.shape)}")
    for t, name in ((cond, "cond"), (null, "null"), (out, "out")):
        hip.require_gpu(t, name)
        if t.dtype != torch.float32 or t.shape != (rows, ld) or t.stride() != (ld, 1):
            raise ValueError(f"guide_logits: {name} must be fp32 [{rows}, {ld}] with contiguous rows; got {t.dtype} {tuple(t.shape)} {t.stride()}")
    if not 0 < int(V) <= ld:
        raise ValueError(f"guide_logits: V must lie in [1, {ld}], not {V}")
    if by_row:
        call("omlm_guide_logits_rows", ptr(cond), ptr(null), ptr(out), rows, int(V), ld, ptr(scale), stream_ptr())
        return
    call("omlm_guide_logits", ptr(cond), ptr(null), ptr(out), rows, int(V), ld, 1.0 if s is None else s, stream_ptr())


def decode_twin(ids=None, ids_twin=None, x=None, x_twin=None):
    if (ids is None) != (ids_twin is None) or (x is None) != (x_twin is None):
        raise ValueError("decode_twin: give ids with ids_twin and x with x_twin")
    if ids is None and x is None:
        return
    rows = ids.shape[0] if ids is not None else x.shape[0]
    if ids is not None:
        for t in (ids, ids_twin):
            hip.require_gpu(t, "ids")
            assert t.dtype == torch.int64 and t.shape == (rows,) and t.is_contiguous()
    D = 0
    if x is not None:
        D = x.shape[1]
        for t in (x, x_twin):
            hip.require_gpu(t, "x")
            assert t.dtype == torch.float32 and t.shape == (rows, D) and t.is_contiguous()
    call("omlm_decode_twin", ptr(ids), ptr(ids_twin), ptr(x), ptr(x_twin), rows, D, stream_ptr())


def prepare_train_batch(raw_ids, eos_ids, quantizers, codebooks, pad_id, scores, n_drop, want_labels, *, null_u=None, null_p=0.):
    n = len(raw_ids)
    B, dev = raw_ids[0].shape[0], raw_ids[0].device
    if null_u is not None:
        null_p = check_null_cond_prob(null_p, "null_p")
        if n < 2:
            raise ValueError("prepare_train_batch: the condition drop needs a conditioning sequence (at least two token sequences)")
        hip.require_gpu(null_u, "null_u")
        assert null_u.dtype == torch.float32 and null_u.shape == (B,) and null_u.is_contiguous()
    for t in raw_ids:
        hip.require_gpu(t, "token ids")
        assert t.dtype == torch.int64 and t.dim() == 2 and t.is_contiguous() and t.shape[0] == B
    lens = [int(t.shape[1]) for t in raw_ids]
    N = sum(l + 1 for l in lens) + (n - 1)
    ids32 = torch.empty(B, N, dtype=torch.int32, device=dev)
    keymask = torch.empty(B, N, dtype=torch.uint8, device=dev)
    labels = [torch.empty(B, l + 1, dtype=torch.int32, device=dev) if w else None for l, w in zip(lens, want_labels)]
    arr_i = lambda v: (C.c_int * n)(*[int(x) for x in v])
    call("omlm_prepare_train_batch", _ptr_array(raw_ids), _ptr_array(labels), arr_i(lens), arr_i(eos_ids), arr_i(quantizers), arr_i(codebooks),
         n, B, int(pad_id), ptr(scores), int(n_drop), ptr(ids32), ptr(keymask), N, ptr(null_u), float(null_p) if null_u is not None else 0.,
         stream_ptr())
    return ids32, keymask, labels, [l + 1 for l in lens[:-1]] + [lens[-1]]


def _check_number(x):
    try:
        return float("nan") if isinstance(x, (str, bytes, bool)) else float(x)
    except (TypeError, ValueError):
        return float("nan")


def check_label_smoothing(eps, name="label_smoothing"):
# ... 356 lines not shown
```

Before: 1205 samples/s.

## Recompute FF mid gated pre-norm activation in backward instead of saving gh

The forward no longer writes the gated pre-norm activation gh when Fp fits the one-pass backward. The fused backward strip kernel instead recomputes it from h1, the conv taps, and the saved mean/rstd. This drops an M x Fp store in forward and the matching load in backward, saving bandwidth and activation memory, at the cost of reordered conv/GELU arithmetic in the backward. The s2 reduction is also rewritten to use dy times h2 directly.

```diff
diff --git a/include/omlm.h b/include/omlm.h
--- a/include/omlm.h
+++ b/include/omlm.h
@@ -85,6 +85,10 @@
                    const float* rstd, void* du_tmp, void* dh1, float* dgamma, float* dconv, float* workspace,
                    int M, int nseq, int F, int Fp, float p, unsigned long long seed,
                    const unsigned long long* seed_dev, const unsigned char* drop_bits, const void* gh, int dtype, void* stream);
+int omlm_ffmid_bwd_saved(const void* dh2, const void* h1, const void* convw, const void* gamma, const float* mean,
+                         const float* rstd, void* du_tmp, void* dh1, float* dgamma, float* dconv, float* workspace,
+                         int M, int nseq, int F, int Fp, float p, unsigned long long seed,
+                         const unsigned long long* seed_dev, const unsigned char* drop_bits, const void* gh, const void* h2, int dtype, void* stream);
 int omlm_colsum_accumulate(const float* part, float* out, int P, int C, int ldp, void* stream);
 typedef struct omlm_colsum_desc { const float* part; float* out; int P, C, ldp; } omlm_colsum_desc;
 int omlm_colsum_group(const omlm_colsum_desc* problems, int count, void* stream);
diff --git a/open_musiclm_amd/csrc/ffmid.hip b/open_musiclm_amd/csrc/ffmid.hip
--- a/open_musiclm_amd/csrc/ffmid.hip
+++ b/open_musiclm_amd/csrc/ffmid.hip
@@ -597,6 +597,7 @@
     c.op = op; c.M = a.M; c.nseq = a.nseq; c.F = a.F; c.Fp = a.Fp; c.dtype = dtype; c.fp16_copy = OMLM_FP16 != 0; c.p = a.p; c.operands = operands;
     c.drop_bits = a.drop_bits != nullptr; c.gh = a.gh != nullptr; c.dgamma = a.dgamma != nullptr; c.dconv = a.dconv != nullptr;
     c.n_full = a.n_full; c.p0 = a.p0; c.h2_8_stride = a.h2_8_stride; c.impl = omlm_ffmid_impl_value;
+    c.lean = true;
     return c;
 }
 static bool ffmid_aligned16(std::initializer_list<const void*> ps) {
@@ -718,4 +719,32 @@
     return ffmid_run(c, a);
 }
 
-}
+#if !OMLM_FP16
+extern "C" int omlm_ffmid_bwd_saved_h(const void* dh2, const void* h1, const void* convw, const void* gamma, const float* mean,
+                                      const float* rstd, void* du_tmp, void* dh1, float* dgamma, float* dconv, float* workspace,
+                                      int M, int nseq, int F, int Fp, float p, unsigned long long seed,
+                                      const unsigned long long* seed_dev, const unsigned char* drop_bits, const void* gh, const void* h2,
+                                      int dtype, void* stream);
+#endif
+extern "C" int OMLM_API(omlm_ffmid_bwd_saved)(const void* dh2, const void* h1, const void* convw, const void* gamma, const float* mean,
+                              const float* rstd, void* du_tmp, void* dh1, float* dgamma, float* dconv, float* workspace,
+                              int M, int nseq, int F, int Fp, float p, unsigned long long seed,
+                              const unsigned long long* seed_dev, const unsigned char* drop_bits, const void* gh, const void* h2,
+                              int dtype, void* stream) {
+#if !OMLM_FP16
+    if (dtype == OMLM_DT_F16)
+        return omlm_ffmid_bwd_saved_h(dh2, h1, convw, gamma, mean, rstd, du_tmp, dh1, dgamma, dconv, workspace, M, nseq, F, Fp, p, seed, seed_dev,
+                                      drop_bits, gh, h2, 1, stream);
+#endif
+    FfmidArgs a;
+    memset(&a, 0, sizeof(a));
+    a.dh2 = dh2; a.h1 = h1; a.convw = convw; a.gamma = gamma; a.mean = const_cast<float*>(mean); a.rstd = const_cast<float*>(rstd);
+    a.du_tmp = du_tmp; a.dh1 = dh1; a.dgamma = dgamma; a.dconv = dconv; a.workspace = workspace; a.M = M; a.nseq = nseq; a.F = F; a.Fp = Fp; a.p = p;
+    a.seed = seed; a.seed_dev = seed_dev; a.drop_bits = const_cast<unsigned char*>(drop_bits); a.gh = const_cast<void*>(gh); a.h2_saved = h2; a.stream = stream;
+    FfmidCall c = ffmid_call(FF_BWD, a, dtype, dh2 && h1 && convw && gamma && rstd && du_tmp && dh1 && workspace);
+    c.saved = true; c.h2 = h2 != nullptr; c.mean = mean != nullptr;
+    c.du_aligned = (uintptr_t)du_tmp % 8 == 0;
+    return ffmid_run(c, a);
+}
+
+}
diff --git a/open_musiclm_amd/csrc/ffmid2.hip b/open_musiclm_amd/csrc/ffmid2.hip
--- a/open_musiclm_amd/csrc/ffmid2.hip
+++ b/open_musiclm_amd/csrc/ffmid2.hip
@@ -151,7 +151,7 @@
 #define FS_OCC 1
 
 struct FfSeg { int n_full, p0; };
-template <typename T, int NT, bool TRAIN, bool PL, bool MX, bool SEG>
+template <typename T, int NT, bool TRAIN, bool PL, bool MX, bool SEG, bool GH>
 __device__ __forceinline__ void ffmid2_fwd_body(const T* __restrict__ h1, const T* __restrict__ convw,
                                                         const T* __restrict__ gamma, T* __restrict__ h2,
                                                         float* __restrict__ mean, float* __restrict__ rstd,
@@ -313,7 +313,7 @@
             }
             else if constexpr (PL) store_planes8(h2 + row * Fp + col, (T*)pl.h2_lo + row * Fp + col, y);
             else Ch8<T>::store(h2 + row * Fp + col, y);
-            if (TRAIN || gh_out) Ch8<T>::store(gh_out + row * Fp + col, gh);
+            if (TRAIN ? GH : gh_out != nullptr) Ch8<T>::store(gh_out + row * Fp + col, gh);
         }
         if (FULL) {
             const int q = lane % RB_;
@@ -333,23 +333,23 @@
     for (; tb < t1; tb += RB_, ++it) batch(std::false_type{}, tb, it);
 }
 
-template <typename T, int NT, bool TRAIN, bool PL = false, bool MX = false>
+template <typename T, int NT, bool TRAIN, bool PL = false, bool MX = false, bool GH = TRAIN>
 __global__ __launch_bounds__(NT, (FS_OCC * NT + 255) / 256) void ffmid2_fwd_kernel(const T* __restrict__ h1, const T* __restrict__ convw,
                                                         const T* __restrict__ gamma, T* __restrict__ h2,
                                                         float* __restrict__ mean, float* __restrict__ rstd,
                                                         int nseq, int F, int Fp, int RB, int strips, float eps, float p,
                                                         unsigned long long seed, const unsigned long long* __restrict__ seed_dev,
                                                         unsigned char* __restrict__ drop_bits, T* __restrict__ gh_out, const FfPlanes pl) {
-    ffmid2_fwd_body<T, NT, TRAIN, PL, MX, false>(h1, convw, gamma, h2, mean, rstd, nseq, F, Fp, RB, strips, eps, p, seed, seed_dev, drop_bits, gh_out, pl, FfSeg{0, 0});
-}
-template <typename T, int NT, bool TRAIN, bool PL = false, bool MX = false>
+    ffmid2_fwd_body<T, NT, TRAIN, PL, MX, false, GH>(h1, convw, gamma, h2, mean, rstd, nseq, F, Fp, RB, strips, eps, p, seed, seed_dev, drop_bits, gh_out, pl, FfSeg{0, 0});
+}
+template <typename T, int NT, bool TRAIN, bool PL = false, bool MX = false, bool GH = TRAIN>
 __global__ __launch_bounds__(NT, (FS_OCC * NT + 255) / 256) void ffmid2_fwd_seg_kernel(const T* __restrict__ h1, const T* __restrict__ convw,
                                                         const T* __restrict__ gamma, T* __restrict__ h2,
                                                         float* __restrict__ mean, float* __restrict__ rstd,
                                                         int nseq, int F, int Fp, int RB, int strips, float eps, float p,
                                                         unsigned long long seed, const unsigned long long* __restrict__ seed_dev,
                                                         unsigned char* __restrict__ drop_bits, T* __restrict__ gh_out, const FfPlanes pl, const FfSeg seg) {
-    ffmid2_fwd_body<T, NT, TRAIN, PL, MX, true>(h1, convw, gamma, h2, mean, rstd, nseq, F, Fp, RB, strips, eps, p, seed, seed_dev, drop_bits, gh_out, pl, seg);
+    ffmid2_fwd_body<T, NT, TRAIN, PL, MX, true, GH>(h1, convw, gamma, h2, mean, rstd, nseq, F, Fp, RB, strips, eps, p, seed, seed_dev, drop_bits, gh_out, pl, seg);
 }
 
 template <typename T, int MAXC>
@@ -567,14 +567,14 @@
     }
 }
 
-template <typename T> struct Bwd3Row { Ch4<T> dy, gh, xv, xg; unsigned bits; float a; };
+template <typename T> struct Bwd3Row { Ch4<T> dy, gh, xv, xg; unsigned bits; float a, mu; };
 __device__ __forceinline__ void opaque(Ch4<h16_t>& c) { asm volatile("" : "+v"(c.r[0]), "+v"(c.r[1])); }
 __device__ __forceinline__ void opaque(Ch4<float>&) {}
 
-template <typename T, int NT>
+template <typename T, int NT, bool H2 = false>
 __global__ __launch_bounds__(NT) void ffmid3_bwd_kernel(const T* __restrict__ dh2, const T* __restrict__ h1,
                                                         const T* __restrict__ convw, const T* __restrict__ gamma,
-                                                        const float* __restrict__ rstd, const T* __restrict__ ghs,
+                                                        const float* __restrict__ mean, const float* __restrict__ rstd, const T* __restrict__ ghs,
                                                         const unsigned char* __restrict__ drop_bits, T* __restrict__ dh1,
                                                         float* __restrict__ part_dconv, float* __restrict__ part_dgamma,
                                                         int nseq, int F, int Fp, int RB, int strips, int total_strips, float p) {
@@ -616,6 +616,7 @@
         R.xg.load(h1 + row * ld + Fp + colc);
         R.bits = (p > 0.f) ? (unsigned)drop_bits[row * (size_t)(Fp >> 3) + (colc >> 3)] : 0xFFu;
         R.a = rstd[row];
+        if constexpr (H2) R.mu = mean[row];
     };
     auto dy_kept = [&](const Bwd3Row<T>& R, v2 (&dy)[2]) {
         const unsigned kb = R.bits >> nib;
@@ -633,9 +634,10 @@
         for (int i = 0; i < 2; ++i) {
             const v2 gy = dy[i] * gm[i];
             s1 += gy;
-            s2 = fma2(gy, R.gh.get(i), s2);
-        }
-        const float t1 = wave_sum_dpp(s1[0] + s1[1]), t2 = wave_sum_dpp(s2[0] + s2[1]);
+            if constexpr (H2) s2 = fma2(R.dy.get(i), R.gh.get(i), s2);
+            else s2 = fma2(gy, R.gh.get(i), s2);
+        }
+        const float t1 = wave_sum_dpp(s1[0] + s1[1]), t2 = wave_sum_dpp((H2 && !act) ? 0.f : s2[0] + s2[1]);
         if (lane == 0) { red[buf][wave][0] = t1; red[buf][wave][1] = t2; }
     };
 
@@ -681,22 +683,36 @@
                 const float rs = cur.a * invF;
                 const float bsum = rs * S1, csum = rs * S2;
                 const float own = t < t1 ? 1.f : 0.f;
+                const float nmr = H2 ? -cur.mu * cur.a : 0.f;
                 v2 dy[2];
                 dy_kept(cur, dy);
 #pragma unroll
                 for (int i = 0; i < 2; ++i) {
-                    const v2 gh = cur.gh.get(i);
-                    const v2 gy = dy[i] * gm[i];
-                    dgam[i] = fma2(dy[i] * own, gh, dgam[i]);
-                    v2 dg = fma2(gy, splat2(cur.a), splat2(-bsum));
-                    dg = fma2(gh, splat2(-csum), dg);
+                    v2 dg, uv, ug, h, ex, ugh;
                     const v2 xv = cur.xv.get(i), xg = cur.xg.get(i);
-                    const v2 uv = fma2(wvr[2].get(i), xv, fma2(wvr[1].get(i), x1v[i], wvr[0].get(i) * x2v[i]));
-                    const v2 ug = fma2(wgr[2].get(i), xg, fma2(wgr[1].get(i), x1g[i], wgr[0].get(i) * x2g[i]));
-                    v2 h, ex;
-                    gelu_parts(ug, h, ex);
+                    if constexpr (H2) {
+                        uv = fma2(wvr[2].get(i), xv, fma2(wvr[1].get(i), x1v[i], wvr[0].get(i) * x2v[i]));
+                        ug = fma2(wgr[2].get(i), xg, fma2(wgr[1].get(i), x1g[i], wgr[0].get(i) * x2g[i]));
+                        gelu_parts(ug, h, ex);
+                        ugh = ug * h;
+                        const v2 gh = fma2(ugh * uv, splat2(cur.a), splat2(nmr));
+                        const v2 gy = dy[i] * gm[i];
+                        dgam[i] = fma2(dy[i] * own, gh, dgam[i]);
+                        dg = fma2(gy, splat2(cur.a), splat2(-bsum));
+                        dg = fma2(gh, splat2(-csum), dg);
+                    } else {
+                        const v2 gh = cur.gh.get(i);
+                        const v2 gy = dy[i] * gm[i];
+                        dgam[i] = fma2(dy[i] * own, gh, dgam[i]);
+                        dg = fma2(gy, splat2(cur.a), splat2(-bsum));
+                        dg = fma2(gh, splat2(-csum), dg);
+                        uv = fma2(wvr[2].get(i), xv, fma2(wvr[1].get(i), x1v[i], wvr[0].get(i) * x2v[i]));
+                        ug = fma2(wgr[2].get(i), xg, fma2(wgr[1].get(i), x1g[i], wgr[0].get(i) * x2g[i]));
+                        gelu_parts(ug, h, ex);
+                        ugh = ug * h;
+                    }
                     const v2 gp = fma2(ug * 0.3989422804f, ex, h);
-                    const v2 a_ = dg * (ug * h);
+                    const v2 a_ = dg * ugh;
                     const v2 g_ = (dg * uv) * gp;
                     duv[i] = a_; dug[i] = g_;
                     const v2 ao = a_ * own, go = g_ * own;
@@ -735,7 +751,7 @@
 #pragma unroll
             for (int e = 0; e < 2; ++e) {
                 const int ch = col + 2 * i + e;
-                pg[ch] = dgam[i][e];
+                pg[ch] = (H2 && ch >= F) ? 0.f : dgam[i][e];
                 if (ch < F) {
 #pragma unroll
                     for (int k = 0; k < 3; ++k) { pr[(size_t)ch * 3 + k] = dcv[k][i][e]; pr[(size_t)(F + ch) * 3 + k] = dcg[k][i][e]; }
@@ -752,6 +768,8 @@
 #define FF2_FWD(K_, NT_, ...) do { \
         if (l.train) hipLaunchKernelGGL((K_<T, NT_, true, PL, MX>), grid, block, 0, st, (const T*)a.h1, (const T*)a.convw, (const T*)a.gamma, (T*)a.h2, a.mean, a.rstd, \
                                         a.nseq, a.F, a.Fp, l.RB, l.strips, a.eps, a.p, a.seed, a.seed_dev, a.drop_bits, (T*)a.gh, pl, ##__VA_ARGS__); \
+        else if (l.lean) hipLaunchKernelGGL((K_<T, NT_, true, PL, MX, false>), grid, block, 0, st, (const T*)a.h1, (const T*)a.convw, (const T*)a.gamma, (T*)a.h2, a.mean, a.rstd, \
+                                a.nseq, a.F, a.Fp, l.RB, l.strips, a.eps, a.p, a.seed, a.seed_dev, a.drop_bits, (T*)nullptr, pl, ##__VA_ARGS__); \
         else hipLaunchKernelGGL((K_<T, NT_, false, PL, MX>), grid, block, 0, st, (const T*)a.h1, (const T*)a.convw, (const T*)a.gamma, (T*)a.h2, a.mean, a.rstd, \
                                 a.nseq, a.F, a.Fp, l.RB, l.strips, a.eps, a.p, a.seed, a.seed_dev, a.drop_bits, (T*)a.gh, pl, ##__VA_ARGS__); } while (0)
 #define FF2_FWD_NT(K_, ...) switch (l.n) { \
@@ -792,10 +810,12 @@
         return omlm_post_launch("omlm_ffmid_fwd (strip)");
     }
     case FK_BWD3: {
-#define FF3_BWD(NT_) hipLaunchKernelGGL((ffmid3_bwd_kernel<T, NT_>), grid, block, 0, st, (const T*)a.dh2, (const T*)a.h1, (const T*)a.convw, (const T*)a.gamma, \
-                       (const float*)a.rstd, (const T*)a.gh, (const unsigned char*)a.drop_bits, (T*)a.dh1, part_c, part_g, a.nseq, a.F, a.Fp, l.RB, l.strips, l.total, a.p)
+#define FF3_BWD_(NT_, H2_, SV_) hipLaunchKernelGGL((ffmid3_bwd_kernel<T, NT_, H2_>), grid, block, 0, st, (const T*)a.dh2, (const T*)a.h1, (const T*)a.convw, (const T*)a.gamma, \
+                       (const float*)a.mean, (const float*)a.rstd, (const T*)(SV_), (const unsigned char*)a.drop_bits, (T*)a.dh1, part_c, part_g, a.nseq, a.F, a.Fp, l.RB, l.strips, l.total, a.p)
+#define FF3_BWD(NT_) do { if (l.h2) FF3_BWD_(NT_, true, a.h2_saved); else FF3_BWD_(NT_, false, a.gh); } while (0)
         switch (l.n) { case 128: FF3_BWD(128); break; case 256: FF3_BWD(256); break; case 512: FF3_BWD(512); break; default: FF3_BWD(768); break; }
 #undef FF3_BWD
+#undef FF3_BWD_
         return omlm_post_launch("omlm_ffmid_bwd (fused strip)");
     }
     case FK_ROWSUM:
diff --git a/open_musiclm_amd/csrc/ffmid_plan.h b/open_musiclm_amd/csrc/ffmid_plan.h
--- a/open_musiclm_amd/csrc/ffmid_plan.h
+++ b/open_musiclm_amd/csrc/ffmid_plan.h
@@ -47,6 +47,9 @@
     bool planes_aligned;
     bool du_aligned;
     int impl;
+    bool saved;
+    bool h2, mean;
+    bool lean;
 };
 enum FfKernel {
     FK_FWD1, FK_BWD1, FK_BWD2,
@@ -62,6 +65,8 @@
     long long lds;
     int RB, strips, total;
     int g_rows, c_rows;
+    bool h2;
+    bool lean;
 };
 struct FfmidPlan {
     int rc;
@@ -109,7 +114,11 @@
     FF_REFUSE_UNLESS(c.operands, c.op == FF_FWD ? "null pointer [h1 && convw && gamma && h2 && mean && rstd]" :
                                  c.op == FF_FWD_PLANES ? "null pointer [h1 && h1_lo && convw && convw_lo && gamma && gamma_lo && h2 && h2_lo && mean && rstd]" :
                                  c.op == FF_FWD_MX ? "null pointer [h1 && h1_lo && convw && convw_lo && gamma && gamma_lo && h2 && h2_8 && scale8 && mean && rstd]" :
+                                 c.saved ?           "null pointer [dh2 && h1 && convw && gamma && rstd && du_tmp && dh1 && workspace]" :
                                                      "null pointer [dh2 && h1 && convw && gamma && mean && rstd && du_tmp && dh1 && workspace]");
+    const bool h2_given = c.saved && c.h2 && c.mean;
+    if (c.op == FF_BWD && c.saved)
+        FF_REFUSE_UNLESS(c.gh || h2_given, "ffmid_bwd_saved: the forward's gh, or its h2 and mean, must be given [gh || (h2 && mean)]");
     if (c.op == FF_FWD_PLANES)
         FF_REFUSE_UNLESS(Fp >= F && ffmid_strip_ok(Fp), "ffmid_fwd_planes: Fp must be F rounded up to 8 and <= 4096 [Fp % 8 == 0 && Fp >= F && ffmid2_supported(Fp)]");
     else if (c.op == FF_FWD_MX)
@@ -130,13 +139,17 @@
         FF_REFUSE_UNLESS(c.planes_aligned, "ffmid_fwd_planes: 16-byte aligned planes [(((uintptr_t)h1 | (uintptr_t)h1_lo | (uintptr_t)convw | (uintptr_t)convw_lo | "
                                            "(uintptr_t)gamma | (uintptr_t)gamma_lo | (uintptr_t)h2 | (uintptr_t)h2_lo) % 16) == 0]");
     }
-    p.strips = planes || (c.impl == 1 && ffmid_strip_ok(Fp) && keep_ok && (fwd || c.gh));
+    const bool strip_call = c.impl == 1 && ffmid_strip_ok(Fp) && keep_ok;
+    if (c.op == FF_BWD && c.saved && strip_call)
+        FF_REFUSE_UNLESS(c.gh || ffmid_one_pass(Fp), "ffmid_bwd_saved: Fp > 3072 runs the two-pass backward, which reads gh [gh || ffmid_one_pass(Fp)]");
+    p.strips = planes || (strip_call && (fwd || c.gh || h2_given));
     const int B = M / nseq, rows4 = (M + 3) / 4;
     if (fwd && p.strips) {
         const int RB = ffmid_strip_rows(nseq, 36), strips = (nseq + RB - 1) / RB, nt = ffmid_chunks_per_lane(Fp) * 64;
         const bool segd = c.n_full > 0 && c.p > 0.f;
         FfmidLaunch& l = ffmid_push(p, segd ? FK_STRIP_FWD_SEG : FK_STRIP_FWD, c, nt >= 64 && nt < 512 ? nt : 512, B * strips, 1, Fp / 8, 0);
         l.train = c.p > 0.f && c.drop_bits && c.gh;
+        l.lean = c.lean && c.p > 0.f && c.drop_bits && !c.gh;
         l.pl = planes; l.mx = c.op == FF_FWD_MX; l.RB = RB; l.strips = strips;
         return p;
     }
@@ -145,6 +158,7 @@
         return p;
     }
     if (!p.strips) {
+        FF_REFUSE_UNLESS(!c.saved || c.mean, "ffmid_bwd_saved: the wave-per-row backward reads mean [mean]");
         const int b1 = rows4 < FF_BWD1_BLOCKS ? rows4 : FF_BWD1_BLOCKS, strips = M < FF_BWD2_STRIPS ? M : FF_BWD2_STRIPS;
         ffmid_push(p, FK_BWD1, c, ffmid_maxc(Fp), b1, 1, FF_THREADS, ffmid_row_lds(Fp)).gh = c.gh;
         ffmid_push(p, FK_BWD2, c, 0, (2 * Fp / 8 + FF_THREADS - 1) / FF_THREADS, strips, FF_THREADS, 0);
@@ -160,6 +174,7 @@
         const int nthr = (Fp / 4 + 63) / 64 * 64, nt = nthr <= 128 ? 128 : nthr <= 256 ? 256 : nthr <= 512 ? 512 : 768;
         FfmidLaunch& l = ffmid_push(p, FK_BWD3, c, nt, 1, ny, nt, 0);
         l.RB = RB; l.strips = strips; l.total = total;
+        l.h2 = !c.gh;
         g_rows = ny;
     } else {
         g_rows = rows4 < FF_BWD1_BLOCKS ? rows4 : FF_BWD1_BLOCKS;
@@ -186,6 +201,7 @@
     const unsigned long long* seed_dev;
     unsigned char* drop_bits;
     void* gh;
+    const void* h2_saved;
     int n_full, p0;
     long long h2_8_stride;
     void* stream;
@@ -206,6 +222,19 @@
     }
     memcpy(msg, q.msg, sizeof(q.msg));
 }
+extern "C" void omlm_plan_ffmid_saved(const int* v, double p, long long h2_8_stride, long long* out, char* msg) {
+    omlm_plan::FfmidCall c = {(omlm_plan::FfOp)v[0], v[1], v[2], v[3], v[4], v[5], v[6] != 0, (float)p, v[7] != 0, v[8] != 0, v[9] != 0, v[10] != 0,
+                              v[11] != 0, v[12], v[13], h2_8_stride, v[14] != 0, v[15] != 0, v[16]};
+    c.saved = v[17] != 0; c.h2 = v[18] != 0; c.mean = v[19] != 0; c.lean = v[20] != 0;
+    const omlm_plan::FfmidPlan q = omlm_plan::ffmid_plan(c);
+    out[0] = q.rc; out[1] = q.strips; out[2] = q.n;
+    for (int i = 0; i < q.n; ++i) {
+        const omlm_plan::FfmidLaunch& l = q.l[i];
+        const long long w[18] = {l.kernel, l.t16, l.n, l.train, l.pl, l.mx, l.gh, l.gx, l.gy, l.threads, l.lds, l.RB, l.strips, l.total, l.g_rows, l.c_rows, l.h2, l.lean};
+        memcpy(out + 3 + 18 * i, w, sizeof(w));
+    }
+    memcpy(msg, q.msg, sizeof(q.msg));
+}
 extern "C" void omlm_plan_ffmid_limits(int* out) {
     const int v[5] = {omlm_plan::FF_MAX_FP, omlm_plan::FF_STRIP_MAX_FP, omlm_plan::FF_ONE_PASS_MAX_FP, FF_BWD1_BLOCKS, FF_BWD2_STRIPS};
     memcpy(out, v, sizeof(v));
diff --git a/open_musiclm_amd/engine.py b/open_musiclm_amd/engine.py
--- a/open_musiclm_amd/engine.py
+++ b/open_musiclm_amd/engine.py
@@ -151,6 +151,10 @@
 CONV_HALO = 2
 LIVE_K_MULTIPLE = 64
 FF_ONE_PASS_MAX_FP = 3072
+
+
+def ff_saves_gh(Fp: int) -> bool:
+    return Fp > FF_ONE_PASS_MAX_FP
 
 
 def first_live_row(lay: SeqLayout, want: Sequence[bool]) -> Optional[int]:
@@ -581,7 +585,7 @@
         p = float(ff.dropout_p) if training else 0.0
         seed = seeds[li] if (p > 0 and seeds is not None) else 0
         drop_bits = torch.empty(M, Fp // 8, dtype=torch.uint8, device=dev) if (p > 0 and (save or pw.ff_planes)) else None
-        gh = torch.empty(M, Fp, dtype=T, device=dev) if save else None
+        gh = torch.empty(M, Fp, dtype=T, device=dev) if save and ff_saves_gh(Fp) else None
         x2 = torch.empty(M, D, device=dev)
         if pw.ff_planes:
             if pw.mx:
@@ -680,7 +684,7 @@
         gconv = grad_of(ff.conv_param()).view(-1) if ff.conv_param() is not None else None
         ops.ffmid_bwd(dh2, sv.h1, w["convw"], w["gamma_mid"], sv.m3, sv.r3, du, dh1,
                       grad_of(ff.norm_mid.gamma), gconv, ws, nff, F, Fp, sv.p, sv.seed,
-                      seed_dev=saved["salt"] if sv.p > 0 else None, drop_bits=sv.drop_bits, gh=sv.gh)
+                      seed_dev=saved["salt"] if sv.p > 0 else None, drop_bits=sv.drop_bits, gh=sv.gh, h2=sv.h2)
         del du, dh2
         dxn2 = torch.empty(M, D, dtype=T, device=dev)
         ops.gemm(dh1, w["W1p"], dxn2, M=M, N=D, K=2 * Fp, b_kmajor=True)
diff --git a/open_musiclm_amd/hip.py b/open_musiclm_amd/hip.py
--- a/open_musiclm_amd/hip.py
+++ b/open_musiclm_amd/hip.py
@@ -57,6 +57,7 @@
     "omlm_ffmid_fwd_planes_seg": [vp, vp, vp, vp, vp, vp, vp, vp, vp, vp, i32, i32, i32, i32, f32, f32, u64, vp, vp, vp, i32, i32, i32, vp],
     "omlm_ffmid_bwd_workspace_bytes": [i32, i32],
     "omlm_ffmid_bwd": [vp, vp, vp, vp, vp, vp, vp, vp, vp, vp, vp, i32, i32, i32, i32, f32, u64, vp, vp, vp, i32, vp],
+    "omlm_ffmid_bwd_saved": [vp, vp, vp, vp, vp, vp, vp, vp, vp, vp, vp, i32, i32, i32, i32, f32, u64, vp, vp, vp, vp, i32, vp],
     "omlm_colsum_accumulate": [vp, vp, i32, i32, i32, vp],
     "omlm_colsum_group": [vp, i32, vp],
     "omlm_ffmid_set_impl": [i32],
diff --git a/open_musiclm_amd/ops.py b/open_musiclm_amd/ops.py
--- a/open_musiclm_amd/ops.py
+++ b/open_musiclm_amd/ops.py
@@ -497,9 +497,15 @@
 
 
 def ffmid_bwd(dh2, h1, convw, gamma, mean, rstd, du_tmp, dh1, dgamma, dconv, workspace, nseq, F, Fp, p, seed, seed_dev=None,
-              drop_bits=None, gh=None):
+              drop_bits=None, gh=None, h2=None):
     assert convw.shape == (3, 2 * Fp) and gamma.numel() == Fp
     assert convw.dtype == h1.dtype and gamma.dtype == h1.dtype, "taps / gamma travel in the operand dtype of h1"
+    if h2 is not None:
+        assert h2.dtype == h1.dtype and h2.shape == (h1.shape[0], Fp) and h2.is_contiguous()
+        call("omlm_ffmid_bwd_saved", ptr(dh2), ptr(h1), ptr(convw), ptr(gamma), ptr(mean), ptr(rstd), ptr(du_tmp), ptr(dh1),
+             ptr(dgamma), ptr(dconv), ptr(workspace), h1.shape[0], nseq, F, Fp, float(p), int(seed), ptr(seed_dev), ptr(drop_bits),
+             ptr(gh), ptr(h2), dcode(h1.dtype), stream_ptr())
+        return
     call("omlm_ffmid_bwd", ptr(dh2), ptr(h1), ptr(convw), ptr(gamma), ptr(mean), ptr(rstd), ptr(du_tmp), ptr(dh1),
          ptr(dgamma), ptr(dconv), ptr(workspace), h1.shape[0], nseq, F, Fp, float(p), int(seed), ptr(seed_dev), ptr(drop_bits),
          ptr(gh), dcode(h1.dtype), stream_ptr())
```

Result: no change. 1209 samples/s (median of 3 runs) (+0.3%).
